# QuentinFuxa/WhisperLiveKit

Hardware: AMD Instinct MI355X
Metric: audio seconds transcribed per second (1/RTF), Whisper-base EN simul_whisper AlignAtt, 0.5 s chunks (higher is better)
Workload: dtype f32; 1 GPU; base.en simul_whisper, 1 stream(s) over 1 GPU(s) (1 per GPU), 30 s 16 kHz speech-like stream, 0.5 s chunks, beam 1, frame_threshold 25, seeded random weights, synthetic vocabulary; model=base.en, streams_total=1

## Files before the change

include/wlk_hip.h:

```cpp
#ifndef WLK_HIP_H
#define WLK_HIP_H

#include <stdint.h>

#ifdef __cplusplus
extern "C" {
#endif

#define WLK_OK 0
#define WLK_ERR_ARG (-1)
#define WLK_ERR_HIP (-2)
#define WLK_ERR_STATE (-3)
#define WLK_ERR_CAPACITY (-4)

typedef struct wlk_model wlk_model;
typedef struct wlk_session wlk_session;

typedef struct wlk_dims {
    int32_t n_mels, n_audio_ctx, n_audio_state, n_audio_head, n_audio_layer;
    int32_t n_vocab, n_text_ctx, n_text_state, n_text_head, n_text_layer;
} wlk_dims;

const char* wlk_last_error(void);
int wlk_abi_version(void);
// ... 264 lines not shown
typedef struct wlk_vad_group wlk_vad_group;
int wlk_vad_group_create(wlk_vad* m, int max_streams , int max_windows_total , wlk_vad_group** out);
int wlk_vad_group_run(wlk_vad_group* g, wlk_vad_stream* const* streams, const int32_t* n_windows, int n_streams,
                      const void* pcm_host, int sample_format, float* probs_host);
int wlk_vad_group_destroy(wlk_vad_group* g);

const char* wlk_diag_last_error(void);
int wlk_diag_env_refresh(void);
int wlk_diag_linear(const float* a, int64_t lda, int64_t a_floats, const float* w, const float* bias,
                    const float* r, int64_t ldr, int m, int n, int k, int flags, float scale, int scale_cols,
                    int force_gemv, float* c);
typedef struct wlk_nllb_dims {
    int32_t vocab, d_model, heads, ffn, enc_layers, dec_layers;
    int32_t max_src, max_tgt;
    int32_t pad_id;
    int32_t n_positions;
    float embed_scale;
} wlk_nllb_dims;
typedef struct wlk_nllb wlk_nllb;
typedef struct wlk_nllb_session wlk_nllb_session;
int wlk_nllb_arena_floats(const wlk_nllb_dims* dims, uint64_t* n_floats);
int wlk_nllb_tensor_lookup(const wlk_nllb_dims* dims, const char* packed_name, uint64_t* offset_floats, uint64_t* numel);
int wlk_nllb_tensor_name(const wlk_nllb_dims* dims, int index, const char** name);
int wlk_nllb_create(const wlk_nllb_dims* dims, int device, wlk_nllb** out);
int wlk_nllb_upload(wlk_nllb* m, const char* packed_name, const float* host, uint64_t numel);
int wlk_nllb_finalize(wlk_nllb* m);
int wlk_nllb_destroy(wlk_nllb* m);
int wlk_nllb_session_create(wlk_nllb* m, int rows, wlk_nllb_session** out);
int wlk_nllb_session_destroy(wlk_nllb_session* s);
int wlk_nllb_encode(wlk_nllb_session* s, const int64_t* src_ids, int32_t n);
int wlk_nllb_decode(wlk_nllb_session* s, const int64_t* tokens, int32_t n_rows, int32_t n_tok, int32_t first);
int wlk_nllb_step(wlk_nllb_session* s, const int64_t* tokens, int32_t n_rows, int32_t k, float* logprobs, int32_t* ids);
int wlk_nllb_kv_reorder(wlk_nllb_session* s, const int32_t* source_rows, int32_t n_rows);
int wlk_nllb_topk(wlk_nllb_session* s, int32_t k, float* logprobs, int32_t* ids);
int wlk_nllb_step_beam(wlk_nllb_session* s, const int64_t* tokens , const int32_t* source_rows ,
                       int32_t n_rows, int32_t k , float* logprobs, int32_t* ids);
int wlk_nllb_session_beam_stats(wlk_nllb_session* s, uint64_t* ancestry_steps);
int wlk_nllb_session_set_align(wlk_nllb_session* s, const int32_t* layer_head_pairs, int32_t n);
int wlk_nllb_step_align(wlk_nllb_session* s, const int64_t* tokens, int32_t n_rows, int32_t k , int32_t lo, int32_t hi,
                        int32_t limit, float* logprobs, int32_t* ids, int32_t* align_pos , float* align_prob ,
                        float* tail_mass );
enum { WLK_ALIGN_STOP_ATTENTION = 0, WLK_ALIGN_STOP_EOS = 1, WLK_ALIGN_STOP_LENGTH = 2, WLK_ALIGN_STOP_CONTEXT = 3 };
int wlk_nllb_generate_alignatt(wlk_nllb_session* s, const int64_t* prompt, int32_t n_prompt, int32_t n_accessible,
                               int32_t threshold, int32_t final, int64_t eos_id, int32_t max_new, int64_t* out_ids,
                               int32_t* out_align, int32_t* n_out, int32_t* stop_reason);
int wlk_nllb_session_align_stats(wlk_nllb_session* s, uint64_t* align_steps, uint64_t* graph_captures);
int wlk_nllb_export(wlk_nllb_session* s, const char* what, float* host, uint64_t capacity, uint64_t* n_written);
int wlk_nllb_sync(wlk_nllb_session* s);

typedef struct wlk_nllb_batch wlk_nllb_batch;
int wlk_nllb_batch_create(wlk_nllb* m, int n_slots, wlk_nllb_batch** out);
int wlk_nllb_batch_destroy(wlk_nllb_batch* b);
int wlk_nllb_batch_encode(wlk_nllb_batch* b, const int32_t* slots, const int64_t* src_ids, const int32_t* src_offsets, int32_t n);
int wlk_nllb_batch_step(wlk_nllb_batch* b, const int32_t* slots, const int64_t* tokens, int32_t n_rows, int32_t k, float* logprobs,
                        int32_t* ids);
int wlk_nllb_batch_release(wlk_nllb_batch* b, int32_t slot);
int wlk_nllb_batch_export(wlk_nllb_batch* b, int32_t slot, const char* what, float* host, uint64_t capacity, uint64_t* n_written);
int wlk_nllb_batch_cross_attention(wlk_nllb_batch* b, const int32_t* slots, int32_t n_rows, int32_t layer, const float* q_host,
                                   float* out_host);
int wlk_nllb_batch_sync(wlk_nllb_batch* b);
int wlk_nllb_batch_set_align(wlk_nllb_batch* b, const int32_t* layer_head_pairs, int32_t n);
int wlk_nllb_batch_prefill(wlk_nllb_batch* b, const int32_t* slots, const int64_t* prompt_ids, const int32_t* prompt_offsets,
                           int32_t n);
int wlk_nllb_batch_step_align(wlk_nllb_batch* b, const int32_t* slots, const int64_t* tokens, int32_t n_rows, int32_t k ,
                              const int32_t* lo , const int32_t* hi , const int32_t* limit ,
                              float* logprobs, int32_t* ids, int32_t* align_pos , float* align_prob ,
                              float* tail_mass );
int wlk_nllb_batch_align_stats(wlk_nllb_batch* b, uint64_t* align_steps, uint64_t* graph_captures);
int wlk_nllb_batch_verify(wlk_nllb_batch* b, const int32_t* slots, const int64_t* ids, const int32_t* offsets, int32_t n,
                          int32_t* accepted, int64_t* next_token);
int wlk_nllb_batch_verify_stats(wlk_nllb_batch* b, uint64_t* passes, uint64_t* draft_tokens, uint64_t* accepted_tokens);

int wlk_dtw(int device, const float* x, int32_t n_rows, int32_t n_cols, int8_t* trace);
int wlk_log_mel(wlk_session* s, const float* pcm, int64_t n_samples, int32_t padding, float* mel, uint64_t capacity_floats,
                int32_t* n_frames);
int wlk_encode_mel(wlk_session* s, const float* mel, int32_t n_frames);
int wlk_find_alignment(wlk_session* s, const int64_t* tokens, int32_t n_tokens, int32_t n_sot, int32_t eot,
                       int32_t num_frames, float qk_scale, float* cost, int8_t* trace, float* token_probs);
int wlk_head_survey(wlk_session* s, const int64_t* tokens, int32_t n_tokens, int32_t num_frames, float* peak, int32_t* frame);

int wlk_diag_linear_time(int m, int n, int k, int flags, int force_gemv, int reps, float* us_per_launch);
int wlk_diag_linear_ln(const float* a, const float* w, const float* bias, const float* gamma, const float* beta,
                       int m, int n, int k, int force_gemv, float* c);
int wlk_diag_layernorm(const float* x, const float* gamma, const float* beta, int rows, int d, float* y);
int wlk_diag_prefill_stack(wlk_session** sessions, const int64_t* tokens, const int32_t* n_tok, const int32_t* sot_index, int32_t n,
                           int32_t* taken);
int wlk_engine_prefill_stats(wlk_model* m, uint64_t* batches, uint64_t* sessions);
int wlk_diag_encoder_attention_time(int t, int d, int n_head, int reps, float* us_per_launch);
int wlk_diag_encoder_attention(const float* qkv, int t, int d, int n_head, float* out);
typedef struct wlk_diag_select_args {
    int32_t route, n_rows, n_vocab, k;
    const float* logits;
    const int32_t* adj_row;
    const int32_t* adj_ids;
    const float* adj_deltas;
    int32_t n_adj;
    int32_t n_align, ring_rows, T, single_base;
    const float* ring;
    const int32_t* prefill_rows;
    const int32_t* n_single;
    const int32_t* newest_row;
    const int32_t* content_len;
    int32_t ns_token;
    const float* ns_logits;
    float* top_logprobs;
    int32_t* top_ids;
    int32_t* frames;
    float* attn_last;
    float* z;
    float* ns_probs;
    float* logits_out;
} wlk_diag_select_args;
int wlk_diag_select(const wlk_diag_select_args* args);
int wlk_diag_topk(const float* logits, int32_t n_rows, int32_t n_vocab, int32_t k, int32_t form ,
                  float* logprobs, int32_t* ids);
int wlk_diag_nllb_align(const float* probs, int32_t n_align, int32_t rows, int32_t S, int32_t lo, int32_t hi, int32_t limit,
                        float* p_out, int32_t* pos, float* prob, float* mass);
int wlk_diag_nllb_align_rows(const float* probs, int32_t n_align, int32_t rows, int32_t stride, const int32_t* S,
                             const int32_t* lo, const int32_t* hi, const int32_t* limit, float* p_out, int32_t* pos, float* prob,
                             float* mass);
int wlk_diag_nllb_verify_pick(const float* logits, int32_t n_rows, int32_t n_vocab, const int32_t* targets, int32_t* picks,
                              int32_t* match);
enum {
    WLK_DA_S0 = 0, WLK_DA_S1 = 1, WLK_DA_S2 = 2,
    WLK_DA_C0 = 10, WLK_DA_C1 = 11, WLK_DA_C2 = 12, WLK_DA_C3 = 13, WLK_DA_C4 = 14, WLK_DA_C5 = 15,
    WLK_DA_A0 = 20, WLK_DA_G0 = 21, WLK_DA_K0 = 22, WLK_DA_K1 = 23
};
typedef struct wlk_diag_dec_attention_args {
    int32_t route, n_rows, n_tok, d, n_head, ctx_len, T;
    int32_t anc_rows, n_updates, gather_len, n_layer, n_kv, k_splits, n_align, n_beam, ring_rows;
    float scale;
    int64_t cache_floats;
    int64_t layer_off;
    int64_t scores_floats, out_floats;
    const float* qkv;
    float* kcache;
    float* vcache;
    const int32_t* offsets;
    const int32_t* row_cache;
    uint8_t* anc;
    const int32_t* ctl;
    const int32_t* upd_offsets;
    const float* q;
    const float* k;
    const float* v;
    const int32_t* row_kv;
    const float* x;
    const float* wq;
    const float* bq;
    const float* gamma;
    const float* beta;
    const float* wo;
    const float* bo;
    const float* resid;
    const int32_t* head_rank;
    const int32_t* ring_row;
    const int32_t* beam_of_row;
    float* ring;
    float* scores;
    float* out;
} wlk_diag_dec_attention_args;
int wlk_diag_dec_attention(const wlk_diag_dec_attention_args* args);
enum {
    WLK_SFK_ATTENTION = 0, WLK_SFK_CONV0 = 1, WLK_SFK_DWCONV2D = 2, WLK_SFK_GLU_DWCONV = 3, WLK_SFK_HEAD = 4, WLK_SFK_ASSEMBLE = 5
};
typedef struct wlk_diag_sf_kernel_args {
// ... 125 lines not shown
```

whisperlivekit_amd/_lib.py:

```python
from __future__ import annotations

import ctypes as C
import os
import threading
from typing import Optional


_LIB_NAME = "libwlk_hip.so"
_lock = threading.Lock()
_lib: Optional[C.CDLL] = None


class WlkError(RuntimeError):
    """Raised for every non-zero status of the C ABI (message from wlk_last_error())."""


class Dims(C.Structure):
    _fields_ = [(n, C.c_int32) for n in (
        "n_mels", "n_audio_ctx", "n_audio_state", "n_audio_head", "n_audio_layer",
        "n_vocab", "n_text_ctx", "n_text_state", "n_text_head", "n_text_layer")]


class SfDims(C.Structure):
    _fields_ = [(n, C.c_int32) for n in (
# ... 246 lines not shown
        "wlk_prof_end": (cint, [p, cint, C.POINTER(C.c_char_p), p, p, p, p, C.POINTER(i32)]),
        "wlk_melspec_create": (cint, [cint, cint, cint, cint, cint, p, p, C.c_float, C.c_float, cint, C.POINTER(p)]),
        "wlk_melspec_run": (cint, [p, p, cint, p, cint, C.POINTER(cint)]),
        "wlk_melspec_destroy": (cint, [p]),
        "wlk_sf_arena_floats": (cint, [C.POINTER(SfDims), C.POINTER(u64)]),
        "wlk_sf_tensor_lookup": (cint, [C.POINTER(SfDims), C.c_char_p, C.POINTER(u64), C.POINTER(u64)]),
        "wlk_sf_tensor_name": (cint, [C.POINTER(SfDims), cint, C.POINTER(C.c_char_p)]),
        "wlk_sf_create": (cint, [C.POINTER(SfDims), cint, C.POINTER(p)]),
        "wlk_sf_upload": (cint, [p, C.c_char_p, p, u64]),
        "wlk_sf_finalize": (cint, [p]),
        "wlk_sf_step": (cint, [p, p, cint, p, cint, p, cint, C.POINTER(cint), p, cint]),
        "wlk_sf_step_pcm": (cint, [p, p, p, cint, cint, p, cint, p, cint, C.POINTER(cint), p, cint, p, cint, C.POINTER(cint), p, cint]),
        "wlk_sf_stats": (cint, [p, C.POINTER(u64), C.POINTER(u64), C.POINTER(u64)]),
        "wlk_sf_export": (cint, [p, C.c_char_p, p, u64, C.POINTER(u64)]),
        "wlk_sf_destroy": (cint, [p]),
        "wlk_sf_session_create": (cint, [p, C.POINTER(SfCacheParams), cint, C.POINTER(p)]),
        "wlk_sf_session_destroy": (cint, [p]),
        "wlk_sf_session_step_pcm": (cint, [p, p, p, cint, cint, cint, cint, p, cint, C.POINTER(cint)]),
        "wlk_sf_session_step": (cint, [p, p, cint, cint, cint, p, cint, C.POINTER(cint)]),
        "wlk_sf_session_update": (cint, [p, p, cint, p, cint, cint, cint, p, cint, C.POINTER(cint)]),
        "wlk_sf_session_get_state": (cint, [p, C.POINTER(SfState)]),
        "wlk_sf_session_set_state": (cint, [p, C.POINTER(SfState)]),
        "wlk_nllb_arena_floats": (cint, [C.POINTER(NllbDims), C.POINTER(u64)]),
        "wlk_nllb_tensor_lookup": (cint, [C.POINTER(NllbDims), C.c_char_p, C.POINTER(u64), C.POINTER(u64)]),
        "wlk_nllb_tensor_name": (cint, [C.POINTER(NllbDims), cint, C.POINTER(C.c_char_p)]),
        "wlk_nllb_create": (cint, [C.POINTER(NllbDims), cint, C.POINTER(p)]),
        "wlk_nllb_upload": (cint, [p, C.c_char_p, p, u64]),
        "wlk_nllb_finalize": (cint, [p]),
        "wlk_nllb_destroy": (cint, [p]),
        "wlk_nllb_session_create": (cint, [p, cint, C.POINTER(p)]),
        "wlk_nllb_session_destroy": (cint, [p]),
        "wlk_nllb_encode": (cint, [p, p, i32]),
        "wlk_nllb_decode": (cint, [p, p, i32, i32, i32]),
        "wlk_nllb_step": (cint, [p, p, i32, i32, p, p]),
        "wlk_nllb_kv_reorder": (cint, [p, p, i32]),
        "wlk_nllb_step_beam": (cint, [p, p, p, i32, i32, p, p]),
        "wlk_nllb_session_beam_stats": (cint, [p, C.POINTER(u64)]),
        "wlk_nllb_topk": (cint, [p, i32, p, p]),
        "wlk_nllb_session_set_align": (cint, [p, p, i32]),
        "wlk_nllb_step_align": (cint, [p, p, i32, i32, i32, i32, i32, p, p, p, p, p]),
        "wlk_nllb_generate_alignatt": (cint, [p, p, i32, i32, i32, i32, C.c_int64, i32, p, p, C.POINTER(i32), C.POINTER(i32)]),
        "wlk_nllb_session_align_stats": (cint, [p, C.POINTER(u64), C.POINTER(u64)]),
        "wlk_nllb_export": (cint, [p, C.c_char_p, p, u64, C.POINTER(u64)]),
        "wlk_nllb_sync": (cint, [p]),
        "wlk_nllb_batch_create": (cint, [p, cint, C.POINTER(p)]),
        "wlk_nllb_batch_destroy": (cint, [p]),
        "wlk_nllb_batch_encode": (cint, [p, p, p, p, i32]),
        "wlk_nllb_batch_step": (cint, [p, p, p, i32, i32, p, p]),
        "wlk_nllb_batch_release": (cint, [p, i32]),
        "wlk_nllb_batch_export": (cint, [p, i32, C.c_char_p, p, u64, C.POINTER(u64)]),
        "wlk_nllb_batch_cross_attention": (cint, [p, p, i32, i32, p, p]),
        "wlk_nllb_batch_sync": (cint, [p]),
        "wlk_nllb_batch_set_align": (cint, [p, p, i32]),
        "wlk_nllb_batch_prefill": (cint, [p, p, p, p, i32]),
        "wlk_nllb_batch_step_align": (cint, [p, p, p, i32, i32, p, p, p, p, p, p, p, p]),
        "wlk_nllb_batch_align_stats": (cint, [p, C.POINTER(u64), C.POINTER(u64)]),
        "wlk_nllb_batch_verify": (cint, [p, p, p, p, i32, p, p]),
        "wlk_nllb_batch_verify_stats": (cint, [p, C.POINTER(u64), C.POINTER(u64), C.POINTER(u64)]),
        "wlk_vad_weights_floats": (cint, [C.POINTER(u64)]),
        "wlk_vad_tensor_lookup": (cint, [C.c_char_p, C.POINTER(u64), C.POINTER(u64)]),
        "wlk_vad_tensor_name": (cint, [cint, C.POINTER(C.c_char_p)]),
        "wlk_vad_create": (cint, [cint, p, u64, C.POINTER(p)]),
        "wlk_vad_destroy": (cint, [p]),
        "wlk_vad_stream_create": (cint, [p, cint, C.POINTER(p)]),
        "wlk_vad_stream_reset": (cint, [p]),
        "wlk_vad_stream_run": (cint, [p, p, cint, p]),
        "wlk_vad_stream_state": (cint, [p, p, p]),
        "wlk_vad_stream_destroy": (cint, [p]),
        "wlk_vad_stream_run_pcm16": (cint, [p, p, cint, p]),
        "wlk_vad_group_create": (cint, [p, cint, cint, C.POINTER(p)]),
        "wlk_vad_group_run": (cint, [p, C.POINTER(p), i32p, cint, p, cint, p]),
        "wlk_vad_group_destroy": (cint, [p]),
        "wlk_diag_last_error": (C.c_char_p, []),
        "wlk_diag_linear": (cint, [p, C.c_int64, C.c_int64, p, p, p, C.c_int64, cint, cint, cint, cint, C.c_float,
                                   cint, cint, p]),
        "wlk_dtw": (cint, [cint, C.POINTER(C.c_float), C.c_int32, C.c_int32, C.POINTER(C.c_int8)]),
        "wlk_encode_mel": (cint, [C.c_void_p, C.POINTER(C.c_float), C.c_int32]),
        "wlk_log_mel": (cint, [C.c_void_p, C.POINTER(C.c_float), C.c_int64, C.c_int32, C.POINTER(C.c_float), C.c_uint64,
                               C.POINTER(C.c_int32)]),
        "wlk_find_alignment": (cint, [C.c_void_p, C.POINTER(C.c_int64), C.c_int32, C.c_int32, C.c_int32, C.c_int32, C.c_float,
                                      C.POINTER(C.c_float), C.POINTER(C.c_int8), C.POINTER(C.c_float)]),
        "wlk_diag_linear_time": (cint, [cint, cint, cint, cint, cint, cint, C.POINTER(C.c_float)]),
        "wlk_diag_linear_ln": (cint, [p, p, p, p, p, cint, cint, cint, cint, p]),
        "wlk_diag_layernorm": (cint, [p, p, p, cint, cint, p]),
        "wlk_diag_encoder_attention_time": (cint, [cint, cint, cint, cint, C.POINTER(C.c_float)]),
        "wlk_diag_encoder_attention": (cint, [p, cint, cint, cint, p]),
        "wlk_diag_wave_ops": (cint, [p, p, p]),
        "wlk_diag_env_refresh": (cint, []),
        "wlk_diag_linear_x3": (cint, [p, p, p, cint, cint, cint, cint, C.c_float, cint, p]),
        "wlk_diag_linear_x3_time": (cint, [cint, cint, cint, cint, cint, C.POINTER(C.c_float)]),
        "wlk_diag_layernorm_x3": (cint, [p, p, p, cint, cint, p]),
        "wlk_diag_encoder_attention_x3": (cint, [p, cint, cint, cint, p]),
        "wlk_diag_encoder_attention_x3_time": (cint, [cint, cint, cint, cint, C.POINTER(C.c_float)]),
        "wlk_diag_qkv_x3_attention": (cint, [p, p, p, cint, cint, cint, C.c_float, p, p]),
        "wlk_diag_select": (cint, [C.POINTER(DiagSelectArgs)]),
        "wlk_diag_dec_attention": (cint, [C.POINTER(DiagDecAttentionArgs)]),
        "wlk_diag_topk": (cint, [p, i32, i32, i32, i32, p, p]),
        "wlk_diag_nllb_align": (cint, [p, i32, i32, i32, i32, i32, i32, p, p, p, p]),
        "wlk_diag_nllb_align_rows": (cint, [p, i32, i32, i32, p, p, p, p, p, p, p, p]),
        "wlk_diag_nllb_verify_pick": (cint, [p, i32, i32, p, p, p]),
        "wlk_diag_sf_kernel": (cint, [C.POINTER(DiagSfKernelArgs)]),
        "wlk_diag_linear_ex": (cint, [C.POINTER(DiagLinearArgs)]),
        "wlk_diag_gemv_variant": (cint, [cint, cint, cint, cint, cint, C.c_char_p, cint]),
        "wlk_diag_gemm_plan": (cint, [cint, cint, cint, cint, cint, cint, C.c_char_p, cint]),
        "wlk_diag_enc_op": (cint, [C.POINTER(DiagEncOpArgs)]),
        "wlk_diag_x3_plan": (cint, [cint, cint, cint, cint, cint, C.c_char_p, cint]),
        "wlk_diag_word_align": (cint, [C.POINTER(DiagWordAlignArgs)]),
        "wlk_diag_head_survey": (cint, [C.POINTER(DiagHeadSurveyArgs)]),
        "wlk_head_survey": (cint, [C.c_void_p, C.POINTER(C.c_int64), C.c_int32, C.c_int32, C.POINTER(C.c_float), C.POINTER(C.c_int32)]),
        "wlk_diag_nllb_cross_ragged": (cint, [C.POINTER(DiagNllbCrossRaggedArgs)]),
        "wlk_model_set_cif": (cint, [p, p, cint, C.c_float]),
        "wlk_cif_result": (cint, [p, C.POINTER(CifOut)]),
        "wlk_diag_cif": (cint, [p, cint, cint, p, C.c_float, cint, cint, p, p, p]),
    }
    for name, (res, args) in sig.items():
        try:
            fn = getattr(lib, name)
        except AttributeError:
            if "WLK_HIP_LIB" in os.environ and name.startswith("wlk_diag_"):
                continue
            raise
        fn.restype = res
        fn.argtypes = args


EXPORTED_SYMBOLS = (
    "wlk_last_error", "wlk_abi_version", "wlk_device_count", "wlk_arena_floats", "wlk_tensor_lookup",
    "wlk_tensor_name", "wlk_model_create", "wlk_model_arena", "wlk_model_upload",
    "wlk_model_set_alignment_heads", "wlk_model_finalize", "wlk_model_destroy", "wlk_session_create",
    "wlk_session_destroy", "wlk_session_set_debug", "wlk_audio_append", "wlk_audio_append_pcm16", "wlk_audio_append_zeros",
    "wlk_audio_drop_front", "wlk_audio_clear", "wlk_audio_len", "wlk_encode", "wlk_decode",
    "wlk_no_speech_prob", "wlk_rules_set", "wlk_pick_greedy", "wlk_pick_topk", "wlk_decode_ancestry", "wlk_select", "wlk_kv_reorder", "wlk_sync", "wlk_decode_until_stop", "wlk_engine_attach", "wlk_engine_detach",
    "wlk_engine_stats", "wlk_engine_encode_stats", "wlk_engine_prefill_stats", "wlk_diag_prefill_stack", "wlk_job_create",
    "wlk_job_begin_step", "wlk_job_no_speech", "wlk_job_adjustments", "wlk_job_consume", "wlk_job_result",
    "wlk_job_destroy", "wlk_export", "wlk_session_step_stats", "wlk_prof_begin",
    "wlk_decode_beam_until_stop", "wlk_session_beam_stats", "wlk_diag_beam_step", "wlk_beam_job_create",
    "wlk_beam_job_begin_step", "wlk_beam_job_no_speech", "wlk_beam_job_adjustments", "wlk_beam_job_consume",
    "wlk_beam_job_state", "wlk_beam_job_result", "wlk_beam_job_destroy",
    "wlk_prof_end", "wlk_melspec_create", "wlk_melspec_run", "wlk_melspec_destroy",
    "wlk_sf_arena_floats", "wlk_sf_tensor_lookup", "wlk_sf_tensor_name", "wlk_sf_create", "wlk_sf_upload",
    "wlk_sf_finalize", "wlk_sf_step", "wlk_sf_step_pcm", "wlk_sf_stats", "wlk_sf_export", "wlk_sf_destroy",
    "wlk_sf_session_create", "wlk_sf_session_destroy", "wlk_sf_session_step_pcm", "wlk_sf_session_step",
    "wlk_sf_session_update", "wlk_sf_session_get_state", "wlk_sf_session_set_state",
    "wlk_vad_weights_floats", "wlk_vad_tensor_lookup", "wlk_vad_tensor_name", "wlk_vad_create", "wlk_vad_destroy",
    "wlk_vad_stream_create", "wlk_vad_stream_reset", "wlk_vad_stream_run", "wlk_vad_stream_state",
    "wlk_vad_stream_destroy", "wlk_vad_stream_run_pcm16", "wlk_vad_group_create", "wlk_vad_group_run",
    "wlk_vad_group_destroy",
    "wlk_dtw", "wlk_encode_mel", "wlk_log_mel", "wlk_find_alignment", "wlk_head_survey",
    "wlk_nllb_arena_floats", "wlk_nllb_tensor_lookup", "wlk_nllb_tensor_name", "wlk_nllb_create", "wlk_nllb_upload",
    "wlk_nllb_finalize", "wlk_nllb_destroy", "wlk_nllb_session_create", "wlk_nllb_session_destroy", "wlk_nllb_encode",
    "wlk_nllb_decode", "wlk_nllb_step", "wlk_nllb_kv_reorder", "wlk_nllb_topk", "wlk_nllb_export", "wlk_nllb_sync",
    "wlk_nllb_step_beam", "wlk_nllb_session_beam_stats",
    "wlk_nllb_session_set_align", "wlk_nllb_step_align", "wlk_nllb_generate_alignatt", "wlk_nllb_session_align_stats",
    "wlk_nllb_batch_create", "wlk_nllb_batch_destroy", "wlk_nllb_batch_encode", "wlk_nllb_batch_step", "wlk_nllb_batch_release",
    "wlk_nllb_batch_export", "wlk_nllb_batch_cross_attention", "wlk_nllb_batch_sync",
    "wlk_nllb_batch_set_align", "wlk_nllb_batch_prefill", "wlk_nllb_batch_step_align", "wlk_nllb_batch_align_stats",
    "wlk_diag_last_error", "wlk_diag_linear", "wlk_diag_linear_time", "wlk_diag_linear_ln", "wlk_diag_layernorm",
    "wlk_diag_encoder_attention", "wlk_diag_encoder_attention_time", "wlk_diag_wave_ops", "wlk_diag_env_refresh",
    "wlk_diag_linear_x3", "wlk_diag_linear_x3_time", "wlk_diag_layernorm_x3",
    "wlk_diag_encoder_attention_x3", "wlk_diag_encoder_attention_x3_time", "wlk_diag_qkv_x3_attention",
    "wlk_diag_select", "wlk_diag_dec_attention", "wlk_diag_topk", "wlk_diag_sf_kernel", "wlk_diag_nllb_align",
    "wlk_diag_nllb_align_rows", "wlk_diag_linear_ex", "wlk_diag_gemv_variant", "wlk_diag_gemm_plan", "wlk_diag_enc_op",
    "wlk_diag_x3_plan", "wlk_diag_word_align", "wlk_diag_head_survey", "wlk_diag_nllb_cross_ragged",
    "wlk_model_set_cif", "wlk_cif_result", "wlk_diag_cif",
    "wlk_group_create", "wlk_group_destroy", "wlk_group_step_pick", "wlk_group_stats", "wlk_group_export_logits",
    "wlk_diag_pick_rows",
    "wlk_group_find_alignment", "wlk_group_align_fits", "wlk_diag_dtw_starts",
    "wlk_group_run_pick", "wlk_diag_pick_advance",
    "wlk_group_verify", "wlk_group_verify_fits", "wlk_diag_draft_pick",
    "wlk_nllb_batch_verify", "wlk_nllb_batch_verify_stats", "wlk_diag_nllb_verify_pick",
)


def load() -> C.CDLL:
    global _lib
    if _lib is not None:
        return _lib
    with _lock:
        if _lib is None:
            path = lib_path()
            if not os.path.exists(path):
                raise WlkError(
                    f"{path} not found: build it with `python -m whisperlivekit_amd.build` "
                    "(hipcc, gfx950). There is no CPU fallback for the HIP backend.")
            try:
                import torch
            except Exception:
                pass
            try:
                lib = C.CDLL(path, mode=C.RTLD_GLOBAL)
            except OSError as e:
                raise WlkError(f"cannot load {path}: {e}") from e
            _declare(lib)
            _lib = lib
    return _lib


def check(rc: int) -> None:
    if rc != 0:
        msg = load().wlk_last_error()
        err = WlkError(f"wlk_hip error {rc}: {msg.decode('utf-8', 'replace') if msg else '?'}")
        err.code = int(rc)
        raise err


def device_count() -> int:
    return int(load().wlk_device_count())
```

whisperlivekit_amd/csrc/api.hip:

```cpp
#include <cmath>
#include <cstdio>
#include <cstdlib>
#include <atomic>
#include <chrono>
#include <cstring>
#include <map>
#include <memory>
#include <mutex>
#include <string>
#include <vector>

#include "../../include/wlk_hip.h"
#include "common.h"
#include "internal.h"

namespace wlk {

namespace {
struct UtilStream {
    std::mutex mu;
    hipStream_t stream = nullptr;
};
UtilStream g_util[64];
UtilStream& util_of_current_device() {
// ... 333 lines not shown
        m->finalized = true;
        return WLK_OK;
    });
}

int wlk_model_destroy(wlk_model* m) {
    if (!m) return WLK_OK;
    wlk_engine_destroy_for_model(m);
    (void)hipSetDevice(m->device);
    if (m->owns_arena) (void)hipFree(m->arena);
    if (m->xkv_all_w) (void)hipFree(m->xkv_all_w);
    if (m->xkv_all_b) (void)hipFree(m->xkv_all_b);
    for (unsigned short* p : m->x3_owned) (void)hipFree(p);
    (void)hipFree(m->twiddle);
    (void)hipFree(m->filt_lo);
    (void)hipFree(m->filt_hi);
    (void)hipFree(m->head_rank);
    (void)hipFree(m->layer_heads);
    (void)hipFree(m->layer_ranks);
    (void)hipFree(m->all_ranks);
    if (m->cif_w) (void)hipFree(m->cif_w);
    delete m;
    return WLK_OK;
}

int wlk_session_create(wlk_model* m, int beam, int max_audio_samples, wlk_session** out) {
    if (!m || !out) return fail(WLK_ERR_ARG, "NULL argument");
    if (!m->finalized) return fail(WLK_ERR_STATE, "model not finalized");
    if (beam < 1 || beam > 7) return fail(WLK_ERR_ARG, "beam must be in [1, 7]");
    if (max_audio_samples < kHop) return fail(WLK_ERR_ARG, "max_audio_samples too small");
    return guarded([&]() {
        WLK_HIP(hipSetDevice(m->device));
        auto s = std::make_unique<wlk_session>();
        s->m = m;
        s->beam = beam;
        s->audio_cap = max_audio_samples;
        WLK_HIP(hipStreamCreateWithFlags(&s->stream, hipStreamNonBlocking));
        if (const char* e = std::getenv("WLK_NO_GRAPH")) s->use_graph = !(e[0] == '1');
        hipStream_t st = s->stream;
        const wlk_dims& D = m->D;
        const size_t d = D.n_audio_state, T = D.n_audio_ctx, ctx = D.n_text_ctx, V = D.n_vocab;
        s->audio[0] = dev_alloc_zero<float>(s->audio_cap, st);
        s->audio[1] = dev_alloc_zero<float>(s->audio_cap, st);
        s->frame_cap = s->audio_cap / kHop + 4;
        s->logmel = dev_alloc<float>((size_t)s->frame_cap * D.n_mels);
        s->frame_max = dev_alloc<float>(s->frame_cap);
        s->logmel_alt = dev_alloc<float>((size_t)s->frame_cap * D.n_mels);
        s->frame_max_alt = dev_alloc<float>(s->frame_cap);
        if (const char* e = std::getenv("WLK_MEL_INCREMENTAL")) s->mel_incremental = !(e[0] == '0');
        s->mel_t = dev_alloc_zero<float>((size_t)(kMelFrames + 2) * D.n_mels, st);
        s->x1p = dev_alloc_zero<float>((size_t)(kMelFrames + 1) * d, st);
        s->ex = dev_alloc<float>(T * d);
        s->eh = dev_alloc<float>(T * d);
        s->eqkv = dev_alloc<float>(T * 3 * d);
        s->eatt = dev_alloc<float>(T * d);
        s->emlp = dev_alloc<float>(T * 4 * d);
        s->enc_out = dev_alloc<float>(T * d);
        {
            bool any_x3 = m->xkv_all_w3 != nullptr, qkv_x3 = false;
            bool fc2_x3 = false;
            for (const auto& L : m->enc_layers) {
                any_x3 |= L.qkvw3 || L.fc1w3 || L.outw3;
                qkv_x3 |= L.qkvw3 != nullptr;
                fc2_x3 |= L.fc2w3 != nullptr;
            }
            if (fc2_x3) s->emlp3 = dev_alloc<unsigned short>(T * 3 * 4 * d);
            const bool attn_x3 = qkv_x3 && enc_attention_x3_enabled() && d == (size_t)D.n_audio_head * 64 && T >= 64 && (2 * d) % 128 == 0;
            if (any_x3) s->eh3 = dev_alloc<unsigned short>(T * 3 * d);
            if (attn_x3) s->eqkv3 = dev_alloc_zero<unsigned short>(x3_attn_image_elems((int)T, (int)d), st);
            if (m->xkv_all_w3) s->enc_out3 = dev_alloc<unsigned short>(T * 3 * d);
        }
        s->cross_kv = dev_alloc<float>((size_t)D.n_text_layer * T * 2 * d);

        s->max_rows = beam * (int)ctx;
        const size_t R = s->max_rows;
        s->step_in = dev_alloc<int>(3 * R + 4);
        s->tokens_dev = s->step_in;
        s->dx = dev_alloc<float>(R * d);
        s->dh = dev_alloc<float>(R * d);
        s->dqkv = dev_alloc<float>(R * 3 * d);
        s->datt = dev_alloc<float>(R * d);
        s->dq = dev_alloc<float>(R * d);
        s->dmlp = dev_alloc<float>(R * 4 * d);
        const size_t cache = (size_t)D.n_text_layer * beam * ctx * d;
        s->kcache[0] = dev_alloc<float>(cache);
        s->vcache[0] = dev_alloc<float>(cache);
        s->hsel = dev_alloc<float>((size_t)2 * beam * d);
        s->logits_last = dev_alloc<float>((size_t)2 * beam * V);
        s->logits_sot = s->logits_last + (size_t)beam * V;
        s->ring_row = s->step_in + R;
        s->beam_of_row = s->step_in + 2 * R;
        s->d_offset = s->step_in + 3 * R;
        s->ring_rows = (int)ctx + kAlignWindow;
        if (m->n_align > 0) s->ring = dev_alloc<float>((size_t)m->n_align * beam * s->ring_rows * T);
        s->xsplit = dev_alloc<float>(cross_split_scratch_floats(8, D.n_text_head, (int)T));
        s->fsplit = dev_alloc<float>(flash_split_scratch_floats(s->max_rows, D.n_text_head, wlk_session::kFlashSplitsMax));
        s->z = dev_alloc<float>((size_t)beam * std::max(m->n_align, 1) * T + (size_t)beam * 128);
        s->attn_last = dev_alloc_zero<float>((size_t)beam * T, st);
        s->adj_row = dev_alloc<int>(3 * wlk_session::kAdjCap);
        s->src_rows = dev_alloc<int>(8);
        if (beam >= 2 && beam <= 7) s->anc = dev_alloc_zero<unsigned char>((size_t)beam * ctx, st);
        s->top_vals = dev_alloc<float>((size_t)beam * 18);
        s->top_ids = reinterpret_cast<int*>(s->top_vals) + (size_t)beam * 8;
        s->frames = s->top_ids + (size_t)beam * 8;
        WLK_HIP(hipMalloc(&s->topk_scratch, topk_scratch_bytes(beam)));
        s->probs = dev_alloc<float>(beam);
        WLK_HIP(hipHostMalloc(&s->pinned, wlk_session::kPinnedBytes, hipHostMallocDefault));
        WLK_HIP(hipHostMalloc(&s->dec_stage, 65536, hipHostMallocDefault));
        WLK_HIP(hipHostMalloc(&s->audio_stage, wlk_session::kPinnedBytes, hipHostMallocDefault));
        WLK_HIP(hipEventCreateWithFlags(&s->audio_stage_ev, hipEventDisableTiming));
        WLK_HIP(hipEventCreateWithFlags(&s->dec_stage_ev, hipEventDisableTiming));
        if (beam == 1) {
            void* hp = nullptr;
            WLK_HIP(hipHostMalloc(&hp, 4096, hipHostMallocMapped | hipHostMallocCoherent));
            std::memset(hp, 0, 4096);
            s->step_host = static_cast<StepBlock*>(hp);
            s->result_host = reinterpret_cast<StepResult*>(static_cast<char*>(hp) + 2048);
            void* dp = nullptr;
            WLK_HIP(hipHostGetDevicePointer(&dp, hp, 0));
            s->step_host_dev = static_cast<StepBlock*>(dp);
            s->result_host_dev = reinterpret_cast<StepResult*>(static_cast<char*>(dp) + 2048);
            s->step_dev = reinterpret_cast<StepBlock*>(dev_alloc<int>(sizeof(StepBlock) / 4));
        }
        if (m->cif_w) wlk_cif_session_prepare(s.get());
        WLK_HIP(hipStreamSynchronize(st));
        *out = s.release();
        return WLK_OK;
    });
}

int wlk_session_destroy(wlk_session* s) {
    if (!s) return WLK_OK;
    if (s->step_count && getenv("WLK_STEP_TIMING"))
        fprintf(stderr, "[wlk] one-replay steps: %llu, mean %.1f us per step (graph launch call %.1f us)\n",
                (unsigned long long)s->step_count, s->step_ns / 1e3 / s->step_count, s->step_launch_ns / 1e3 / s->step_count);
    (void)wlk_engine_detach(s);
    (void)hipSetDevice(s->m->device);
    (void)hipStreamSynchronize(s->stream);
    float* fl[] = {s->audio[0], s->audio[1], s->logmel, s->frame_max, s->logmel_alt, s->frame_max_alt, s->mel_t, s->x1p, s->ex, s->eh, s->eqkv,
                   s->eatt, s->emlp, s->enc_out, s->cross_kv, s->dx, s->dh, s->dqkv, s->datt, s->dq, s->dmlp,
                   s->kcache[0], s->kcache[1], s->vcache[0], s->vcache[1], s->hsel, s->logits_last,
                   s->ring, s->z, s->attn_last, s->qk_debug, s->xsplit, s->fsplit, s->top_vals, s->probs};
    for (float* p : fl)
        if (p) (void)hipFree(p);
    int* il[] = {s->step_in, s->adj_row, s->src_rows};
    for (int* p : il)
        if (p) (void)hipFree(p);
    for (auto& e : s->step_exec)
        if (e) (void)hipGraphExecDestroy(e);
    for (auto& e : s->bstep_exec)
        if (e) (void)hipGraphExecDestroy(e);
    if (s->anc) (void)hipFree(s->anc);
    if (s->topk_scratch) (void)hipFree(s->topk_scratch);
    if (s->pcm16_dev) (void)hipFree(s->pcm16_dev);
    if (s->eh3) (void)hipFree(s->eh3);
    if (s->eqkv3) (void)hipFree(s->eqkv3);
    if (s->enc_out3) (void)hipFree(s->enc_out3);
    if (s->emlp3) (void)hipFree(s->emlp3);
    if (s->wa_buf) (void)hipFree(s->wa_buf);
    if (s->survey_buf) (void)hipFree(s->survey_buf);
    if (s->pinned) (void)hipHostFree(s->pinned);
    if (s->dec_stage) (void)hipHostFree(s->dec_stage);
    if (s->audio_stage) (void)hipHostFree(s->audio_stage);
    if (s->rules_mask) (void)hipFree(s->rules_mask);
    if (s->pick_out) (void)hipFree(s->pick_out);
    if (s->audio_stage_ev) (void)hipEventDestroy(s->audio_stage_ev);
    if (s->dec_stage_ev) (void)hipEventDestroy(s->dec_stage_ev);
    if (s->step_host) (void)hipHostFree(s->step_host);
    if (s->step_dev) (void)hipFree(s->step_dev);
    if (s->step_align_dev) (void)hipFree(s->step_align_dev);
    wlk_cif_session_free(s);
    for (auto& e : s->fstep_exec)
        if (e) (void)hipGraphExecDestroy(e);
    for (auto& r : s->prof.recs) {
        (void)hipEventDestroy(r.a);
        (void)hipEventDestroy(r.b);
    }
    for (auto e : s->prof.pool) (void)hipEventDestroy(e);
    (void)hipStreamDestroy(s->stream);
    delete s;
    return WLK_OK;
}

int wlk_session_set_debug(wlk_session* s, int on) {
    if (!s) return fail(WLK_ERR_ARG, "session is NULL");
    return guarded([&]() {
        WLK_HIP(hipSetDevice(s->m->device));
        s->debug = on != 0;
        if (s->debug && !s->qk_debug) {
            const wlk_dims& D = s->m->D;
            s->qk_debug = dev_alloc<float>((size_t)D.n_text_layer * s->max_rows * D.n_text_head * D.n_audio_ctx);
        }
        return WLK_OK;
    });
}

static bool drain_staging() {
    static const bool on = [] {
        const char* e = getenv("WLK_DRAIN_STAGING");
        return e && e[0] == '1';
    }();
    return on;
}

int wlk_audio_append(wlk_session* s, const float* pcm_host, int n) {
    if (!s || (n > 0 && !pcm_host) || n < 0) return fail(WLK_ERR_ARG, "bad audio chunk");
    if (s->audio_len + n > s->audio_cap)
        return fail(WLK_ERR_CAPACITY, "audio buffer capacity exceeded (" + std::to_string(s->audio_len + n) + " > " +
                                          std::to_string(s->audio_cap) + " samples)");
    if (n == 0) return WLK_OK;
    return guarded([&]() {
        WLK_HIP(hipSetDevice(s->m->device));
        float* dst = s->audio[s->audio_cur] + s->audio_len;
        size_t done = 0;
        while (done < (size_t)n) {
            const size_t chunk = std::min((size_t)n - done, wlk_session::kPinnedBytes / sizeof(float));
            if (s->audio_stage_used) WLK_HIP(hipEventSynchronize(s->audio_stage_ev));
            std::memcpy(s->audio_stage, pcm_host + done, chunk * sizeof(float));
            WLK_HIP(hipMemcpyAsync(dst + done, s->audio_stage, chunk * sizeof(float), hipMemcpyHostToDevice, s->stream));
            WLK_HIP(hipEventRecord(s->audio_stage_ev, s->stream));
            s->audio_stage_used = true;
            done += chunk;
        }
        if (drain_staging()) WLK_HIP(hipStreamSynchronize(s->stream));
        s->audio_len += n;
        s->encoded = false;
        return WLK_OK;
    });
}

// ... 7 lines not shown
        WLK_HIP(hipSetDevice(s->m->device));
        constexpr size_t kMax = wlk_session::kPinnedBytes / sizeof(int16_t);
        if (!s->pcm16_dev) WLK_HIP(hipMalloc(reinterpret_cast<void**>(&s->pcm16_dev), kMax * sizeof(int16_t)));
        float* dst = s->audio[s->audio_cur] + s->audio_len;
        const LaunchCtx c = s->ctx();
        size_t done = 0;
        while (done < (size_t)n) {
            const size_t chunk = std::min((size_t)n - done, kMax);
            if (s->audio_stage_used) WLK_HIP(hipEventSynchronize(s->audio_stage_ev));
            std::memcpy(s->audio_stage, pcm_host + done, chunk * sizeof(int16_t));
            WLK_HIP(hipMemcpyAsync(s->pcm16_dev, s->audio_stage, chunk * sizeof(int16_t), hipMemcpyHostToDevice, s->stream));
            launch_pcm16_to_float(c, s->pcm16_dev, dst + done, (int)chunk);
            WLK_HIP(hipEventRecord(s->audio_stage_ev, s->stream));
            s->audio_stage_used = true;
            done += chunk;
        }
        if (drain_staging()) WLK_HIP(hipStreamSynchronize(s->stream));
        s->audio_len += n;
        s->encoded = false;
        return WLK_OK;
    });
}

int wlk_audio_append_zeros(wlk_session* s, int n) {
    if (!s || n < 0) return fail(WLK_ERR_ARG, "bad zero run");
    if (s->audio_len + n > s->audio_cap) return fail(WLK_ERR_CAPACITY, "audio buffer capacity exceeded");
    if (n == 0) return WLK_OK;
    return guarded([&]() {
        WLK_HIP(hipSetDevice(s->m->device));
        WLK_HIP(hipMemsetAsync(s->audio[s->audio_cur] + s->audio_len, 0, (size_t)n * sizeof(float), s->stream));
        s->audio_len += n;
        s->encoded = false;
        return WLK_OK;
    });
}

int wlk_audio_drop_front(wlk_session* s, int n) {
    if (!s || n < 0 || n > s->audio_len) return fail(WLK_ERR_ARG, "bad eviction length");
    if (n == 0) return WLK_OK;
    return guarded([&]() {
        WLK_HIP(hipSetDevice(s->m->device));
        const int keep = s->audio_len - n;
        if (keep > 0)
            WLK_HIP(hipMemcpyAsync(s->audio[s->audio_cur ^ 1], s->audio[s->audio_cur] + n, (size_t)keep * sizeof(float),
                                   hipMemcpyDeviceToDevice, s->stream));
        s->audio_cur ^= 1;
        s->audio_len = keep;
        s->encoded = false;
        const int shift = n / kHop;
        if (s->mel_incremental && n % kHop == 0 && s->mel_cached_samples > n && shift < s->mel_cached_frames) {
            const int rows = s->mel_cached_frames - shift;
            const int nm = s->m->D.n_mels;
            WLK_HIP(hipMemcpyAsync(s->logmel_alt, s->logmel + (size_t)shift * nm, (size_t)rows * nm * sizeof(float),
                                   hipMemcpyDeviceToDevice, s->stream));
            WLK_HIP(hipMemcpyAsync(s->frame_max_alt, s->frame_max + shift, (size_t)rows * sizeof(float),
                                   hipMemcpyDeviceToDevice, s->stream));
            std::swap(s->logmel, s->logmel_alt);
            std::swap(s->frame_max, s->frame_max_alt);
            s->mel_cached_samples -= n;
            s->mel_cached_frames = rows;
            s->mel_dirty_head = 2;
        } else {
            s->mel_cached_samples = 0;
        }
        return WLK_OK;
    });
}

int wlk_audio_clear(wlk_session* s) {
    if (!s) return fail(WLK_ERR_ARG, "session is NULL");
    s->audio_len = 0;
    s->encoded = false;
    s->mel_cached_samples = 0;
    return WLK_OK;
}

int wlk_audio_len(wlk_session* s, int* n) {
    if (!s || !n) return fail(WLK_ERR_ARG, "NULL argument");
    *n = s->audio_len;
    return WLK_OK;
}

static void transformer_mlp(const LaunchCtx& c, const LayerW& L, float* x, float* h, float* mlp, int rows, int d,
                            const char* t_ln, const char* t_fc1, const char* t_fc2) {
    GemmArgs g;
    g.lda = d; g.W = L.fc1w; g.bias = L.fc1b; g.C = mlp; g.ldc = 4 * d; g.M = rows; g.N = 4 * d; g.K = d;
    g.flags = kGemmGelu;
    if (gemv_applicable(rows, d)) {
        g.A = x; g.ln_gamma = L.ln2w; g.ln_beta = L.ln2b;
        launch_gemv(c, g, "dec_ln2_fc1");
    } else {
        launch_layernorm(c, x, d, L.ln2w, L.ln2b, h, d, rows, d, t_ln);
        g.A = h;
        launch_gemm(c, g, t_fc1);
    }
    GemmArgs g2;
    g2.A = mlp; g2.lda = 4 * d; g2.W = L.fc2w; g2.bias = L.fc2b; g2.C = x; g2.ldc = d; g2.M = rows; g2.N = d;
    g2.K = 4 * d; g2.flags = kGemmResidual; g2.R = x; g2.ldr = d;
    launch_linear(c, g2, t_fc2);
}

extern "C++" std::string wlk_encode_precheck(const wlk_session* s, const wlk_model* m) {
    if (!s) return "encode: session is NULL";
    if (s->m != m) return "encode: the session belongs to another model";
    const int N = s->audio_len;
    const int n_total = (N + kPadSamples) / kHop;
    int n_active = N > 0 ? (N + kNFft / 2 + kHop - 1) / kHop : 0;
    if (n_active > n_total) n_active = n_total;
    if (n_active > s->frame_cap) return "audio longer than the session's frame capacity";
    return std::string();
}

extern "C++" void wlk_encode_group(const std::vector<wlk_session*>& group, const LaunchCtx& c,
                                   std::vector<int>& content_out, bool mel_given) {
    const int B = (int)group.size();
    if (B < 1 || B > kMaxBatch) throw std::invalid_argument("encode: bad group size");
    wlk_model* m = group[0]->m;
    const wlk_dims& D = m->D;
    const int d = D.n_audio_state, T = D.n_audio_ctx;
    content_out.assign(B, 0);
    for (int i = 0; i < B; ++i) {
        wlk_session* s = group[i];
        if (s->m != m) throw std::invalid_argument("encode: sessions of different models in one group");
        if (mel_given) {
            content_out[i] = D.n_audio_ctx;
            continue;
        }
        const int N = s->audio_len;
        const int n_total = (N + kPadSamples) / kHop;
        int n_active = N > 0 ? (N + kNFft / 2 + kHop - 1) / kHop : 0;
        if (n_active > n_total) n_active = n_total;
        if (n_active > s->frame_cap) throw std::length_error("audio longer than the session's frame capacity");
        content_out[i] = (n_total - kMelFrames) / 2;
        MelArgs ma;
        ma.audio = s->audio[s->audio_cur]; ma.n_samples = N;
        ma.window = m->w("mel.window"); ma.twiddle = m->twiddle; ma.filters = m->w("mel.filters");
        ma.filt_lo = m->filt_lo; ma.filt_hi = m->filt_hi; ma.n_mels = D.n_mels;
        ma.logmel = s->logmel; ma.frame_max = s->frame_max; ma.mel_t = s->mel_t;
        ma.n_active = n_active; ma.n_total = n_total;
        if (s->mel_incremental && s->mel_cached_samples > 0 && s->mel_cached_samples <= N && s->mel_cached_frames <= n_active) {
            int first = s->mel_cached_samples >= kNFft / 2 ? (s->mel_cached_samples - kNFft / 2) / kHop + 1 : 0;
            first = std::min(first, s->mel_cached_frames);
            ma.first = first;
            ma.head = std::min(s->mel_dirty_head, first);
        }
        launch_mel(c, ma);
        s->mel_cached_samples = N;
        s->mel_cached_frames = n_active;
        s->mel_dirty_head = 0;
    }
    auto table = [&](auto in, auto out, auto res) {
        PtrTable z{};
        for (int i = 0; i < B; ++i) {
            z.in[i] = in(group[i]);
            z.out[i] = out(group[i]);
            z.res[i] = res(group[i]);
        }
        return z;
    };
    auto none = [](wlk_session*) -> const float* { return nullptr; };
    auto gemm = [&](GemmArgs g, const PtrTable& z, const char* tag) {
        const bool stackable = !gemm_takes_kwave(g.M, g.N, g.K) && (long)((g.N + 63) / 64) * ((g.M + 63) / 64) >= 64;
        if (stackable) {
            g.batch = B;
            g.z = z;
            launch_gemm(c, g, tag);
        } else {
            for (int i = 0; i < B; ++i) {
                g.A = z.in[i]; g.C = z.out[i]; g.R = z.res[i];
                launch_gemm(c, g, tag);
            }
        }
    };
    {
        GemmArgs g;
        g.lda = D.n_mels; g.W = m->w("enc.conv1.w"); g.bias = m->w("enc.conv1.b");
        g.ldc = d; g.M = kMelFrames; g.N = d; g.K = 3 * D.n_mels; g.flags = kGemmGelu;
        gemm(g, table([](wlk_session* s) { return (const float*)s->mel_t; }, [&](wlk_session* s) { return s->x1p + d; }, none),
             "enc_conv1");
    }
    {
// ... 100 lines not shown
                for (int i = 0; i < B; ++i) launch_x3_pack(c, group[i]->emlp, 4 * d, group[i]->emlp3, 4 * d, T, 4 * d);
            gemm_x3(f2, L.fc2w3, z_mlp3_ex_res, "enc_fc2_x3");
        } else {
            gemm(f2, z_mlp_ex, "enc_fc2");
        }
    }
    {
        GemmArgs g;
        g.lda = d; g.W = m->xkv_all_w; g.bias = m->xkv_all_b;
        g.ldc = (long)D.n_text_layer * 2 * d; g.M = T; g.N = D.n_text_layer * 2 * d; g.K = d;
        g.flags = kGemmScaleCols; g.scale = scale; g.scale_cols = d; g.scale_period = 2 * d;
        if (m->xkv_all_w3) {
            launch_layernorm_x3_batched(c, table([](wlk_session* s) { return (const float*)s->ex; },
                                                 [](wlk_session* s) { return reinterpret_cast<float*>(s->enc_out3); }, none),
                                        B, d, m->w("enc.ln_post.w"), m->w("enc.ln_post.b"), d, T, d, "enc_ln_post");
            gemm_x3(g, m->xkv_all_w3,
                    table([](wlk_session* s) { return reinterpret_cast<const float*>(s->enc_out3); }, [](wlk_session* s) { return s->cross_kv; }, none),
                    "dec_cross_kv_x3");
        } else {
            launch_layernorm_batched(c, table([](wlk_session* s) { return (const float*)s->ex; }, [](wlk_session* s) { return s->enc_out; }, none),
                                     B, d, m->w("enc.ln_post.w"), m->w("enc.ln_post.b"), d, T, d, "enc_ln_post");
            gemm(g, table([](wlk_session* s) { return (const float*)s->enc_out; }, [](wlk_session* s) { return s->cross_kv; }, none),
                 "dec_cross_kv");
        }
        for (int i = 0; i < B; ++i) group[i]->enc_out_is_x3 = m->xkv_all_w3 != nullptr;
    }
    if (m->cif_w) wlk_cif_enqueue(group, c, content_out);
    else
        for (int i = 0; i < B; ++i) group[i]->cif_T = -1;
    for (int i = 0; i < B; ++i) {
        wlk_session* s = group[i];
        s->encoded = true;
        s->content_len = content_out[i];
        s->self_len = 0;
        s->n_steps = 0;
    }
}

int wlk_encode(wlk_session* s, int32_t* content_mel_len) {
    if (!s) return fail(WLK_ERR_ARG, "session is NULL");
    return guarded([&]() {
        WLK_HIP(hipSetDevice(s->m->device));
        int content = 0;
        struct Busy {
            wlk_session* s;
            explicit Busy(wlk_session* ss) : s(ss) { wlk_engine_loop_enter(s); }
            ~Busy() { wlk_engine_loop_exit(s); }
        } busy(s);
        if (wlk_engine_batches_encodes(s)) {
            if (int rc = wlk_engine_encode(s, &content)) return rc;
        } else {
            std::vector<int> out;
            wlk_encode_group({s}, s->ctx(), out);
            content = out[0];
        }
        if (content_mel_len) *content_mel_len = content;
        return WLK_OK;
    });
}

int wlk_session::flash_splits() {
    static const int n = [] {
        const char* e = getenv("WLK_FLASH_SPLITS");
        const int v = e ? atoi(e) : 6;
        return v < 1 ? 1 : (v > kFlashSplitsMax ? kFlashSplitsMax : v);
    }();
    return n;
}

constexpr size_t kAncStageOffset = 65536 - 64;

static void enqueue_decode(wlk_session* s, const LaunchCtx& c, int n_rows, int n_tok, bool first, int sot_index,
                           bool step_block = false, const AlignArgs* side_align = nullptr, int side_blocks = 0, int side_zf = 0,
                           bool ancestry = false) {
    wlk_model* m = s->m;
    const wlk_dims& D = m->D;
    const int ctx_len = D.n_text_ctx;
    const int R = n_rows * n_tok;
    const int d = D.n_text_state, T = D.n_audio_ctx, H = D.n_text_head, V = D.n_vocab;
    if (!step_block)
        WLK_HIP(hipMemcpyAsync(s->step_in, s->dec_stage, (size_t)(3 * s->max_rows + 1) * sizeof(int), hipMemcpyHostToDevice,
                               s->stream));
    const bool fused = gemv_applicable(R, d) && n_tok == 1;
    if (ancestry) {
        if (!fused || step_block || !s->anc) throw std::logic_error("decode: the ancestry step needs the fused beam step");
        WLK_HIP(hipMemcpyAsync(s->src_rows, static_cast<char*>(s->dec_stage) + kAncStageOffset, 8 * sizeof(int),
                               hipMemcpyHostToDevice, s->stream));
        launch_anc_update(c, s->anc, s->src_rows, s->d_offset, n_rows, ctx_len);
    }

    if (step_block)
        launch_embed_step(c, s->step_host_dev, s->step_dev, s->tokens_dev, s->ring_row, s->beam_of_row, s->d_offset,
                          m->w_tok_emb, m->w_dec_pos, s->dx, d);
    else
        launch_embed(c, s->tokens_dev, m->w_tok_emb, m->w_dec_pos, s->dx, n_rows, n_tok, s->d_offset, d);
    const float scale = std::pow((float)kHeadDim, -0.25f);
    const size_t cache_layer = (size_t)s->beam * ctx_len * d;
    bool scores_dumped = false;
    const bool raw_pass = s->align_raw_scores || s->survey;
    for (int i = 0; i < D.n_text_layer; ++i) {
        const LayerW& L = m->dec_layers[i];
        float* kc = s->kcache[s->kv_cur] + i * cache_layer;
        float* vc = s->vcache[s->kv_cur] + i * cache_layer;
        GemmArgs g;
        g.W = L.qkvw; g.bias = L.qkvb; g.C = s->dqkv; g.ldc = 3 * d; g.M = R; g.N = 3 * d;
        g.K = d; g.flags = kGemmScaleCols; g.scale = scale; g.scale_cols = 2 * d; g.lda = d;
        if (fused) {
            g.A = s->dx; g.ln_gamma = L.ln1w; g.ln_beta = L.ln1b;
            g.kcache = kc; g.vcache = vc; g.kv_pos = s->d_offset; g.kv_d = d; g.kv_ctx = ctx_len;
            launch_gemv(c, g, "dec_ln1_qkv_kv");
        } else {
            launch_layernorm(c, s->dx, d, L.ln1w, L.ln1b, s->dh, d, R, d, "dec_ln1");
            g.A = s->dh;
            if (!gemv_applicable(R, d) && gemm_takes_kwave(R, 3 * d, d)) {
                g.kcache = kc; g.vcache = vc; g.kv_pos = s->d_offset; g.kv_d = d; g.kv_ctx = ctx_len; g.kv_ntok = n_tok;
                launch_gemm(c, g, "dec_qkv");
            } else {
                launch_linear(c, g, "dec_qkv");
                launch_kv_append(c, s->dqkv, kc, vc, n_rows, n_tok, s->d_offset, d, ctx_len);
            }
        }
        if (ancestry)
            launch_decoder_self_attention_anc(c, s->dqkv, kc, vc, s->anc, s->datt, n_rows, s->d_offset, d, H, ctx_len);
        else
            launch_decoder_self_attention(c, s->dqkv, kc, vc, s->datt, n_rows, n_tok, s->d_offset, d, H, ctx_len);
        GemmArgs o;
        o.A = s->datt; o.lda = d; o.W = L.outw; o.bias = L.outb; o.C = s->dx; o.ldc = d; o.M = R; o.N = d; o.K = d;
        o.flags = kGemmResidual; o.R = s->dx; o.ldr = d;
        launch_linear(c, o, "dec_out");

        GemmArgs q;
        q.lda = d; q.W = L.xqw; q.bias = L.xqb; q.C = s->dq; q.ldc = d; q.M = R; q.N = d; q.K = d;
        q.flags = kGemmScaleCols; q.scale = scale; q.scale_cols = d;
        if (s->survey) q.C = s->survey_buf + (size_t)i * R * d;
        const bool fold_xq = fused && R == 1 && !s->debug && !raw_pass && cross_split_folds_query(d);
        if (fold_xq) {
        } else if (fused) {
            q.A = s->dx; q.ln_gamma = L.lnxw; q.ln_beta = L.lnxb;
            launch_gemv(c, q, "dec_lnx_xq");
        } else {
            launch_layernorm(c, s->dx, d, L.lnxw, L.lnxb, s->dh, d, R, d, "dec_lnx");
            q.A = s->dh;
            launch_linear(c, q, "dec_xq");
        }
        const int* ranks_l = m->n_align > 0 ? m->head_rank + (size_t)i * H : nullptr;
        bool merged_xout = false;
        GemmArgs xo_mg;
        if ((R > 8 || raw_pass) && !s->debug) {
            if (fold_xq) throw std::logic_error("decode: the folded query projection left no q for the flash kernel");
            FlashArgs fa;
            fa.q = q.C; fa.ldq = d;
            fa.k = s->cross_kv + (size_t)i * 2 * d; fa.v = fa.k + d; fa.ldkv = (long)D.n_text_layer * 2 * d;
            fa.out = s->datt; fa.ldo = d; fa.Tq = R; fa.Tk = T; fa.n_head = H;
            fa.head_rank = ranks_l; fa.ring = s->ring; fa.ring_row = s->ring_row;
            fa.beam_of_row = s->beam_of_row; fa.ring_rows = s->ring_rows; fa.n_beam = s->beam;
            if (((R + 31) / 32) * H < 256) {
                fa.k_splits = wlk_session::flash_splits();
                fa.part_o = s->fsplit;
                fa.part_m = fa.part_o + (size_t)s->max_rows * H * fa.k_splits * 64;
                fa.part_l = fa.part_m + (size_t)s->max_rows * H * fa.k_splits;
            }
            launch_prefill_cross_attention(c, fa);
            scores_dumped = true;
        } else {
            CrossAttnArgs ca;
            ca.q = s->dq;
            ca.k = s->cross_kv + (size_t)i * 2 * d;
            ca.v = ca.k + d;
            ca.ldkv = (long)D.n_text_layer * 2 * d;
            ca.out = s->datt;
            ca.rows = R; ca.d = d; ca.n_head = H; ca.T = T;
            ca.head_rank = ranks_l;
            ca.ring = s->ring;
            ca.ring_row = s->ring_row;
            ca.beam_of_row = s->beam_of_row;
            ca.ring_rows = s->ring_rows;
            ca.n_beam = s->beam;
            ca.qk_debug = s->debug ? s->qk_debug + (size_t)i * s->max_rows * H * T : nullptr;
            if (fold_xq) {
                ca.xq_x = s->dx; ca.xq_w = L.xqw; ca.xq_b = L.xqb; ca.xq_gamma = L.lnxw; ca.xq_beta = L.lnxb; ca.xq_scale = scale;
            }
            if (R <= 8 && !s->debug) {
                float* sc = s->xsplit;
                float* pm = sc + (size_t)8 * H * T;
                float* pl = pm + (size_t)8 * H * 8;
                float* po = pl + (size_t)8 * H * 8;
                merged_xout = fused && R == 1 && gemv1_folds_merge(d);
                launch_decoder_cross_attention_split(c, ca, sc, pm, pl, po, !merged_xout);
                if (merged_xout) {
                    xo_mg.mg_pm = pm; xo_mg.mg_pl = pl; xo_mg.mg_po = po; xo_mg.mg_scores = sc;
                    xo_mg.mg_head_rank = ranks_l; xo_mg.mg_ring = s->ring; xo_mg.mg_ring_row = s->ring_row;
                    xo_mg.mg_side_heads = m->layer_heads + (size_t)i * H;
                    xo_mg.mg_beam_of_row = s->beam_of_row; xo_mg.mg_heads = H; xo_mg.mg_T = T;
                    xo_mg.mg_ring_rows = s->ring_rows; xo_mg.mg_n_beam = s->beam;
                    xo_mg.mg_side_blocks = ranks_l ? m->layer_rank_count[i] : 0;
                }
            } else {
                launch_decoder_cross_attention(c, ca);
            }
        }
        GemmArgs xo = xo_mg;
        xo.A = s->datt; xo.lda = d; xo.W = L.xoutw; xo.bias = L.xoutb; xo.C = s->dx; xo.ldc = d; xo.M = R; xo.N = d;
        xo.K = d; xo.flags = kGemmResidual; xo.R = s->dx; xo.ldr = d;
        launch_linear(c, xo, "dec_xout");
        transformer_mlp(c, L, s->dx, s->dh, s->dmlp, R, d, "dec_ln2", "dec_fc1", "dec_fc2");
    }
    if (scores_dumped && m->n_align > 0 && !raw_pass)
        launch_ring_softmax(c, s->ring, s->ring_row, s->beam_of_row, m->all_ranks, m->n_align, R, s->ring_rows, s->beam, T);
    GemmArgs lg;
    lg.lda = d; lg.W = m->w_tok_emb; lg.C = s->logits_last; lg.ldc = V; lg.M = n_rows; lg.N = V; lg.K = d;
    if (side_align && !fused) throw std::logic_error("decode: side workgroups need the fused step");
    if (fused) {
        lg.A = s->dx; lg.ln_gamma = m->w_ln_w; lg.ln_beta = m->w_ln_b;
        lg.side_align = side_align; lg.side_blocks = side_blocks; lg.side_zf = side_zf;
        launch_gemv(c, lg, "dec_lnf_logits");
    } else if (first && n_rows == 1 && gemv_applicable(2, d) && getenv("WLK_NO_PREFILL_MERGE") == nullptr) {
        launch_layernorm(c, s->dx + (size_t)(n_tok - 1) * d, (long)(sot_index - (n_tok - 1)) * d, m->w_ln_w, m->w_ln_b,
                         s->hsel, d, 2, d, "dec_ln_f");
        lg.A = s->hsel; lg.M = 2;
        launch_linear(c, lg, "dec_logits");
        return;
    } else {
        launch_layernorm(c, s->dx + (size_t)(n_tok - 1) * d, (long)n_tok * d, m->w_ln_w, m->w_ln_b, s->hsel, d,
                         n_rows, d, "dec_ln_f");
        lg.A = s->hsel;
        launch_linear(c, lg, "dec_logits");
    }
    if (first) {
        float* hs = s->hsel + (size_t)n_rows * d;
        launch_layernorm(c, s->dx + (size_t)sot_index * d, (long)n_tok * d, m->w_ln_w, m->w_ln_b, hs, d, n_rows, d,
                         "dec_ln_f");
        GemmArgs ls = lg;
        ls.ln_gamma = ls.ln_beta = nullptr;
        ls.A = hs; ls.C = s->logits_sot;
        launch_linear(c, ls, "dec_logits");
    }
}

extern "C++" void wlk_prefill_ws_alloc(const wlk_model* m, wlk_prefill_ws& ws, int max_sessions, int session_rows) {
    const wlk_dims& D = m->D;
    const size_t d = D.n_text_state, V = D.n_vocab, H = D.n_text_head;
    ws.cap_session_rows = session_rows;
    ws.cap_rows = max_sessions * ((session_rows + 31) / 32 * 32);
    const size_t R = ws.cap_rows;
    ws.dx = dev_alloc<float>(R * d);
    ws.dh = dev_alloc<float>(R * d);
    ws.dqkv = dev_alloc<float>(R * 3 * d);
    ws.datt = dev_alloc<float>(R * d);
    ws.dq = dev_alloc<float>(R * d);
    ws.dmlp = dev_alloc<float>(R * 4 * d);
    ws.hsel = dev_alloc<float>((size_t)2 * max_sessions * d);
    ws.logits = dev_alloc<float>((size_t)8 * V);
    ws.part = dev_alloc<float>(flash_split_scratch_floats((int)R, (int)H, wlk_session::kFlashSplitsMax));
    ws.rows_dev = reinterpret_cast<StepRow*>(dev_alloc<char>(R * sizeof(StepRow)));
    ws.tiles_dev = reinterpret_cast<StepRow*>(dev_alloc<char>(R / 32 * sizeof(StepRow)));
    ws.ring_row_dev = dev_alloc<int>(R);
    ws.zeros_dev = dev_alloc<int>(R);
    memset_sync(ws.zeros_dev, 0, R * sizeof(int));
    ws.pinned_bytes = R * sizeof(StepRow) + R / 32 * sizeof(StepRow) + R * sizeof(int);
    WLK_HIP(hipHostMalloc(reinterpret_cast<void**>(&ws.pinned), ws.pinned_bytes, hipHostMallocDefault));
}

extern "C++" void wlk_prefill_ws_free(wlk_prefill_ws& ws) {
    void* dev[] = {ws.dx, ws.dh, ws.dqkv, ws.datt, ws.dq, ws.dmlp, ws.hsel, ws.logits, ws.part, ws.rows_dev, ws.tiles_dev,
                   ws.ring_row_dev, ws.zeros_dev};
    for (void* p : dev)
        if (p) (void)hipFree(p);
    if (ws.pinned) (void)hipHostFree(ws.pinned);
    ws = wlk_prefill_ws{};
}

extern "C++" std::string wlk_prefill_precheck(const wlk_prefill_item& it, const wlk_prefill_ws& ws) {
    const wlk_session* s = it.s;
    if (!s || !it.tokens) return "prefill: NULL argument";
    const wlk_dims& D = s->m->D;
    const int P = it.n_tok, d = D.n_text_state;
    if (!s->encoded) return "wlk_decode before wlk_encode";
    if (s->beam != 1 || s->debug || s->prof_on || s->align_raw_scores || s->survey) return "not a plain beam-1 session";
    if (it.sot_index < 0 || it.sot_index >= P) return "sot_index out of range";
    if (P > D.n_text_ctx) return "text context exceeded";
    for (int i = 0; i < P; ++i)
        if (it.tokens[i] < 0 || it.tokens[i] >= D.n_vocab) return "token id out of range";
    const std::string shape = wlk_prefill_shape_check(s->m, P, ws.cap_session_rows);
    if (!shape.empty()) return shape;
    if (!gemv_applicable(8, d)) return "model too wide for the stacked vocabulary projection";
    return std::string();
}

extern "C++" std::string wlk_prefill_shape_check(const wlk_model* m, int P, int cap_session_rows) {
    const wlk_dims& D = m->D;
    const int d = D.n_text_state;
    if (P <= 8 || P > cap_session_rows) return "prompt length outside the stacked range";
    if (!gemm_takes_kwave(P, 3 * d, d) || !gemm_takes_kwave(P, d, d) || !gemm_takes_kwave(P, 4 * d, d) ||
        !gemm_takes_kwave(P, d, 4 * d))
        return "prompt too long for the k-wave GEMMs";
    if (((P + 31) / 32) * D.n_text_head >= 256) return "prompt too long for the key-split cross-attention";
    return std::string();
}

extern "C++" void wlk_prefill_chain(const std::vector<wlk_prefill_item*>& items, const LaunchCtx& c, wlk_prefill_ws& ws,
                                    std::vector<int>& row0) {
    wlk_model* m = items[0]->s->m;
    const wlk_dims& D = m->D;
    const int d = D.n_text_state, T = D.n_audio_ctx, H = D.n_text_head, L = D.n_text_layer;
    const int B = (int)items.size();
    StepRow* rows_h = reinterpret_cast<StepRow*>(ws.pinned);
    std::vector<int> padded(B);
    row0.assign(B, 0);
    int R = 0;
    for (int i = 0; i < B; ++i) {
        row0[i] = R;
        padded[i] = (items[i]->n_tok + 31) / 32 * 32;
        R += padded[i];
    }
    if (R > ws.cap_rows) throw std::length_error("stacked prefill: more rows than the workspace holds");
    StepRow* tiles_h = rows_h + R;
    int* ring_row_h = reinterpret_cast<int*>(tiles_h + R / 32);
    for (int i = 0; i < B; ++i) {
        wlk_session* s = items[i]->s;
        for (int p = 0; p < padded[i]; ++p) {
            const int src = p < items[i]->n_tok ? p : 0;
            StepRow r{};
            r.kcache = s->kcache[s->kv_cur];
            r.vcache = s->vcache[s->kv_cur];
            r.cross_kv = s->cross_kv;
            r.ring = s->ring;
            r.token = (int)items[i]->tokens[src];
            r.offset = src;
            r.ring_row = src;
            rows_h[row0[i] + p] = r;
            ring_row_h[row0[i] + p] = src;
            if (p % 32 == 0) tiles_h[(row0[i] + p) / 32] = r;
        }
    }
    WLK_HIP(hipMemcpyAsync(ws.rows_dev, rows_h, (size_t)R * sizeof(StepRow), hipMemcpyHostToDevice, c.stream));
    WLK_HIP(hipMemcpyAsync(ws.tiles_dev, tiles_h, (size_t)(R / 32) * sizeof(StepRow), hipMemcpyHostToDevice, c.stream));
    WLK_HIP(hipMemcpyAsync(ws.ring_row_dev, ring_row_h, (size_t)R * sizeof(int), hipMemcpyHostToDevice, c.stream));

    launch_embed_rows(c, ws.rows_dev, m->w_tok_emb, m->w_dec_pos, ws.dx, R, d);
    const float scale = std::pow((float)kHeadDim, -0.25f);
    const size_t cache_layer = (size_t)D.n_text_ctx * d;
    auto linear = [&](const float* A, long lda, const float* W, const float* bias, float* C, long ldc, int N, int K, int flags,
                      const float* Rs, float sc, int sc_cols, const char* tag) {
        GemmArgs g;
        g.A = A; g.lda = lda; g.W = W; g.bias = bias; g.C = C; g.ldc = ldc; g.M = R; g.N = N; g.K = K;
        g.flags = flags; g.R = Rs; g.ldr = ldc; g.scale = sc; g.scale_cols = sc_cols;
        g.force_kwave = true;
        launch_gemm(c, g, tag);
    };
    auto ln_linear = [&](const float* gamma, const float* beta, const float* W, const float* bias, float* C, long ldc, int N,
                         int flags, float sc, int sc_cols, const char* t_ln, const char* tag) {
        launch_layernorm(c, ws.dx, d, gamma, beta, ws.dh, d, R, d, t_ln);
        linear(ws.dh, d, W, bias, C, ldc, N, d, flags, nullptr, sc, sc_cols, tag);
    };
    for (int i = 0; i < L; ++i) {
        const LayerW& W = m->dec_layers[i];
        ln_linear(W.ln1w, W.ln1b, W.qkvw, W.qkvb, ws.dqkv, 3 * d, 3 * d, kGemmScaleCols, scale, 2 * d, "dec_ln1", "dec_qkv");
        launch_kv_append_rows(c, ws.dqkv, ws.rows_dev, (long)(i * cache_layer), R, d);
        launch_decoder_self_attention_rows(c, ws.dqkv, ws.rows_dev, (long)(i * cache_layer), ws.datt, R, d, H, D.n_text_ctx);
        linear(ws.datt, d, W.outw, W.outb, ws.dx, d, d, d, kGemmResidual, ws.dx, 1.f, 0, "dec_out");
        ln_linear(W.lnxw, W.lnxb, W.xqw, W.xqb, ws.dq, d, d, kGemmScaleCols, scale, d, "dec_lnx", "dec_xq");
        FlashArgs fa;
        fa.q = ws.dq; fa.ldq = d;
        fa.k = nullptr; fa.v = nullptr; fa.ldkv = (long)L * 2 * d;
        fa.tile_rows = ws.tiles_dev; fa.tile_kv_off = (long)i * 2 * d; fa.tile_v_off = d;
        fa.out = ws.datt; fa.ldo = d; fa.Tq = R; fa.Tk = T; fa.n_head = H;
        fa.head_rank = m->n_align > 0 ? m->head_rank + (size_t)i * H : nullptr;
        fa.ring = nullptr; fa.ring_row = ws.ring_row_dev; fa.beam_of_row = ws.zeros_dev;
        fa.ring_rows = items[0]->s->ring_rows; fa.n_beam = 1;
        fa.k_splits = wlk_session::flash_splits();
        fa.part_o = ws.part;
        fa.part_m = fa.part_o + (size_t)R * H * fa.k_splits * 64;
        fa.part_l = fa.part_m + (size_t)R * H * fa.k_splits;
        launch_prefill_cross_attention(c, fa);
        linear(ws.datt, d, W.xoutw, W.xoutb, ws.dx, d, d, d, kGemmResidual, ws.dx, 1.f, 0, "dec_xout");
        ln_linear(W.ln2w, W.ln2b, W.fc1w, W.fc1b, ws.dmlp, 4 * d, 4 * d, kGemmGelu, 1.f, 0, "dec_ln2", "dec_fc1");
        linear(ws.dmlp, 4 * d, W.fc2w, W.fc2b, ws.dx, d, d, 4 * d, kGemmResidual, ws.dx, 1.f, 0, "dec_fc2");
    }
}

extern "C++" void wlk_prefill_group(const std::vector<wlk_prefill_item*>& items, const LaunchCtx& c, wlk_prefill_ws& ws) {
    if (items.empty()) return;
    wlk_model* m = items[0]->s->m;
    const wlk_dims& D = m->D;
    const int d = D.n_text_state, T = D.n_audio_ctx, V = D.n_vocab;
    const int B = (int)items.size();
    std::vector<int> row0;
    wlk_prefill_chain(items, c, ws, row0);
    for (int i = 0; i < B; ++i) {
        wlk_session* s = items[i]->s;
        const int P = items[i]->n_tok;
        if (m->n_align > 0)
            launch_ring_softmax(c, s->ring, ws.ring_row_dev + row0[i], ws.zeros_dev, m->all_ranks, m->n_align, P, s->ring_rows, 1, T);
        launch_layernorm(c, ws.dx + (size_t)(row0[i] + P - 1) * d, (long)(items[i]->sot_index - (P - 1)) * d, m->w_ln_w, m->w_ln_b,
                         ws.hsel + (size_t)2 * i * d, d, 2, d, "dec_ln_f");
    }
    for (int lo = 0; lo < B; lo += 4) {
        const int nb = std::min(4, B - lo);
        GemmArgs lg;
        lg.A = ws.hsel + (size_t)2 * lo * d; lg.lda = d; lg.W = m->w_tok_emb; lg.C = ws.logits; lg.ldc = V; lg.M = 2 * nb; lg.N = V;
        lg.K = d;
        launch_gemv(c, lg, "dec_logits");
        for (int i = 0; i < nb; ++i)
            WLK_HIP(hipMemcpyAsync(items[lo + i]->s->logits_last, ws.logits + (size_t)2 * i * V, (size_t)2 * V * sizeof(float),
                                   hipMemcpyDeviceToDevice, c.stream));
    }
    for (int i = 0; i < B; ++i) {
        wlk_session* s = items[i]->s;
        s->self_len = items[i]->n_tok;
        s->n_steps = 1;
        s->have_sot = true;
        s->prefill_rows = items[i]->n_tok;
        s->last_rows = 1;
        s->last_ntok = items[i]->n_tok;
    }
}

int wlk_decode(wlk_session* s, const int64_t* tokens, int n_rows, int n_tok, int first, int sot_index) {
    if (!s || !tokens) return fail(WLK_ERR_ARG, "NULL argument");
    if (!s->encoded) return fail(WLK_ERR_STATE, "wlk_decode before wlk_encode");
    if (n_rows != s->beam) return fail(WLK_ERR_ARG, "n_rows must equal the session's beam size");
    if (n_tok < 1) return fail(WLK_ERR_ARG, "n_tok must be >= 1");
    if (!first && n_tok != 1) return fail(WLK_ERR_ARG, "only one token per row may be fed after the first call");
    if (!first && s->n_steps == 0) return fail(WLK_ERR_STATE, "first decode of an infer must set first=1");
    if (!first && s->anc_live)
        return fail(WLK_ERR_STATE, "wlk_decode(first=0) after an ancestry beam step: the cache rows are not the hypotheses");
    if (first && (sot_index < 0 || sot_index >= n_tok)) return fail(WLK_ERR_ARG, "sot_index out of range");
    return guarded([&]() {
        wlk_model* m = s->m;
        const wlk_dims& D = m->D;
        WLK_HIP(hipSetDevice(m->device));
        const LaunchCtx c = s->ctx();
        if (first) {
            s->self_len = 0;
// ... 634 lines not shown
```

whisperlivekit_amd/csrc/common.h:

```cpp
#pragma once
#include <hip/hip_runtime.h>

#include <cstdint>
#include <stdexcept>
#include <mutex>
#include <string>

namespace wlk {

constexpr int kNFft = 400;
constexpr int kHop = 160;
constexpr int kNFreq = 201;
constexpr int kMelFrames = 3000;
constexpr int kPadSamples = 480000;
constexpr int kHeadDim = 64;
constexpr int kAlignWindow = 16;

struct HipError : std::runtime_error {
    using std::runtime_error::runtime_error;
};

inline void hip_check(hipError_t e, const char* what, const char* file, int line) {
    if (e != hipSuccess) {
        throw HipError(std::string(what) + " failed: " + hipGetErrorString(e) + " (" + file + ":" +
// ... 66 lines not shown
    r.newest_row = n_text_ctx + ((after - 2) % kAlignWindow);
    r.content_len = content_len;
    r.pad = 0;
}

constexpr int kStepMaxAdj = 160;
struct StepBlock {
    StepRow row;
    int n_adj;
    unsigned seq;
    int pad[2];
    int adj_row[kStepMaxAdj];
    int adj_ids[kStepMaxAdj];
    float adj_deltas[kStepMaxAdj];
};
struct StepResult {
    float top_vals[2];
    int top_ids[2];
    int frame;
    unsigned flag_topk, flag_align;
    int pad;
};
struct StepHostOut {
    StepResult* result = nullptr;
    const int* n_adj = nullptr;
    const unsigned* seq = nullptr;
};
constexpr int kEngineFusedAdj = 1024;
struct EngineBlock {
    int n_adj;
    unsigned seq;
    int pad[2];
    StepRow rows[8];
    int adj_row[kEngineFusedAdj];
    int adj_ids[kEngineFusedAdj];
    float adj_deltas[kEngineFusedAdj];
};
void launch_embed_rows_step(const LaunchCtx& ctx, const EngineBlock* host_block, EngineBlock* dev_block, const float* tok_emb,
                            const float* pos_emb, float* x, int n_rows, int d);
void launch_embed_step(const LaunchCtx& ctx, const StepBlock* host_block, StepBlock* dev_block, int* tokens_dev,
                       int* ring_row, int* beam_of_row, int* d_offset, const float* tok_emb, const float* pos_emb, float* x,
                       int d);

constexpr int kMaxBatch = 8;
struct PtrTable {
    const float* in[kMaxBatch];
    float* out[kMaxBatch];
    const float* res[kMaxBatch];
};
template <typename T>
__device__ __forceinline__ T table_at(T const (&t)[kMaxBatch], unsigned z) {
    T v = t[0];
#pragma unroll
    for (int i = 1; i < kMaxBatch; ++i) v = (z == (unsigned)i) ? t[i] : v;
    return v;
}

enum GemmFlags : int {
    kGemmGelu = 1,
    kGemmResidual = 2,
    kGemmScaleCols = 4,
    kGemmRelu = 8,
    kGemmSwish = 16,
};
struct AlignArgs;
struct GemmArgs {
    const float* A = nullptr;
    long lda = 0;
    const float* W = nullptr;
    const float* bias = nullptr;
    float* C = nullptr;
    long ldc = 0;
    const float* R = nullptr;
    long ldr = 0;
    int M = 0, N = 0, K = 0;
    int flags = 0;
    float scale = 1.f;
    int scale_cols = 0;
    int scale_period = 0;
    int batch = 0;
    long long* dbg_clock = nullptr;
    const float* ln_gamma = nullptr;
    const float* ln_beta = nullptr;
    float* kcache = nullptr;
    float* vcache = nullptr;
    const int* kv_pos = nullptr;
    int kv_d = 0, kv_ctx = 0;
    int kv_ntok = 1;
    const StepRow* kv_rows = nullptr;
    long kv_layer_off = 0;
    const float* mg_pm = nullptr;
    const float* mg_pl = nullptr;
    const float* mg_po = nullptr;
    const float* mg_scores = nullptr;
    const int* mg_head_rank = nullptr;
    const int* mg_side_heads = nullptr;
    float* mg_ring = nullptr;
    const int* mg_ring_row = nullptr;
    const int* mg_beam_of_row = nullptr;
    int mg_heads = 0, mg_T = 0, mg_ring_rows = 0, mg_n_beam = 1, mg_side_blocks = 0;
    PtrTable z;
    const AlignArgs* side_align = nullptr;
    int side_blocks = 0, side_zf = 0;
    bool force_kwave = false;
    int force_kernel = 0;
    bool gemm_plain_loop = false;
};
#define WLK_PIN_S(x) asm volatile("" ::"s"(x))
#define WLK_PIN_GEMM_ARGS(g)                                                                                                \
    do {                                                                                                                    \
        asm volatile("" ::"s"((g).A), "s"((g).lda), "s"((g).W), "s"((g).bias), "s"((g).C), "s"((g).ldc), "s"((g).R),        \
                     "s"((g).ldr), "s"((g).M), "s"((g).N), "s"((g).K), "s"((g).flags), "s"((g).scale), "s"((g).scale_cols), \
                     "s"((g).scale_period), "s"((g).batch), "s"((g).dbg_clock));                                            \
        __builtin_amdgcn_sched_barrier(0);     \
    } while (0)
void launch_gemm(const LaunchCtx& ctx, const GemmArgs& g, const char* tag);
void launch_gemm_kp(const LaunchCtx& ctx, const GemmArgs& g, const char* tag);
bool gemm_kp_takes_kpipe(int M, int N, int K);
bool gemm_kpipe_has_tile(int tm, int tn);
struct GemmPlan {
    enum Kernel {
        kRefused,
        kTiled64, kTiled32,
        kKwave, kKwave16,
        kKpipe,
        kKpKwave2, kKpKwave1, kKpKwave16
    };
    Kernel kernel = kRefused;
    int tm = 0, tn = 0;
    const char* refusal = nullptr;
};
GemmPlan gemm_plan(const GemmArgs& g, bool kp_family);
bool gemm_takes_kwave(int M, int N, int K);
bool gemm_takes_ksplit(int M, int N, int K);
void launch_gemv(const LaunchCtx& ctx, const GemmArgs& g, const char* tag);
inline int gemv_row_bucket(int M) { return M <= 1 ? 1 : M <= 2 ? 2 : M <= 4 ? 4 : 8; }
inline bool gemv_applicable(int M, int K) {
    return M <= 8 && (long)gemv_row_bucket(M) * K * 4 <= 64 * 1024 && K % 4 == 0;
}
struct GemvPlan {
    enum Kernel { kRefused, kStaged, kSingleRow, kSingleRowMergeLds };
    Kernel kernel = kRefused;
    int width = 0;
    int rpw = 0;
    bool ln = false, mg = false, full = false;
    const char* refusal = nullptr;
};
GemvPlan gemv_plan(const GemmArgs& g);
bool gemv1_folds_merge(int K);
void refresh_env_switches();
inline void launch_linear(const LaunchCtx& ctx, const GemmArgs& g, const char* tag) {
    if (gemv_applicable(g.M, g.K)) launch_gemv(ctx, g, tag);
    else launch_gemm(ctx, g, tag);
}

struct X3GemmArgs {
    const unsigned short* A3 = nullptr;
    long lda = 0;
    const unsigned short* W3 = nullptr;
    const float* bias = nullptr;
    float* C = nullptr;
    long ldc = 0;
    const float* R = nullptr;
    long ldr = 0;
    int M = 0, N = 0, K = 0;
    int flags = 0;
    float scale = 1.f;
    int scale_cols = 0;
    int scale_period = 0;
    int batch = 0;
    int walk_banded = 0;
    int walk_colmajor = 0;
    int walk_slots = 0;
    unsigned short* C3 = nullptr;
    long ldc3 = 0;
    int vt_col0 = 0;
    long vt_off = 0;
    long vt_ld = 0;
    bool x3_out = false;
    PtrTable z;
};
bool gemm_x3_wide_applicable(int M, int N, int K, long lda);
void launch_gemm_x3(const LaunchCtx& ctx, const X3GemmArgs& g, const char* tag);
void x3_gemm_check(const X3GemmArgs& g);
struct X3GemmPlan {
    int bm = 96;
    int tiles_m = 0, tiles_n = 0;
    int banded = 0, colmajor = 0, persist = 1;
    int slots = 0;
    int blocks = 0;
};
X3GemmPlan x3_gemm_plan(int M, int N, int batch, int cus);
size_t x3_w_elems(int n, int k);
void launch_x3_pack_w(const LaunchCtx& ctx, const float* src, long ld_src, unsigned short* dst, int n, int k);
void launch_x3_pack(const LaunchCtx& ctx, const float* src, long ld_src, unsigned short* dst, long ld_dst, int rows, int cols);
void x3_pack_check(long ld_src, long ld_dst, int cols);
void launch_x3_unpack(const LaunchCtx& ctx, const unsigned short* src, long ld_src, float* dst, long ld_dst, int rows, int cols);

inline long x3_attn_vt_ld(int T) { return ((long)T + 31) / 32 * 32; }
inline long x3_attn_vt_off(int T, int d) { return (long)T * 3 * 2 * d; }
inline size_t x3_attn_image_elems(int T, int d) { return (size_t)x3_attn_vt_off(T, d) + (size_t)d * 3 * x3_attn_vt_ld(T); }
bool enc_attention_x3_enabled();
void launch_encoder_attention_x3(const LaunchCtx& ctx, const unsigned short* qk3, long ldqk, long vt_off, long vt_ld, float* out,
                                 long ldo, int T, int d, int n_head, const PtrTable* z, int batch, bool x3_out = false);
void enc_attention_x3_check(long ldqk, long vt_ld, long ldo, int T, int d, int n_head, bool x3_out);
void launch_x3_pack_qkv(const LaunchCtx& ctx, const float* qkv, unsigned short* out, int T, int d, long vt_off, long vt_ld);

struct HeadSurveyArgs {
    const float* q = nullptr;
    long ldq = 0, q_layer = 0;
    const float* k = nullptr;
    long ldkv = 0, k_layer = 0;
    float* peak = nullptr;
    int* frame = nullptr;
    long out_layer = 0, out_head = 0;
    float* part = nullptr;
    int n_layer = 0, n_head = 0, P = 0, F = 0;
    int k_splits = 0;
};
void head_survey_check(const HeadSurveyArgs& a);
int head_survey_splits(const HeadSurveyArgs& a);
size_t head_survey_scratch_floats(const HeadSurveyArgs& a);
void launch_head_survey(const LaunchCtx& ctx, const HeadSurveyArgs& a);
enum WordAlignStage { kWaSoftmax = 0, kWaZscore = 1, kWaCost = 2, kWaDtw = 3 };
struct WordAlignArgs {
    const float* logits = nullptr;
    long ld = 0;
    int n_cols = 0;
    const int* target = nullptr;
    float* probs = nullptr;
    const float* ring = nullptr;
    int ring_rows = 0, T = 0, n_align = 0, P = 0, F = 0, n_sot = 0;
    float qk_scale = 1.f;
// ... 37 lines not shown
struct MelArgs {
    const float* audio;
    int n_samples;
    const float* window;
    const double* twiddle;
    const float* filters;
    const int* filt_lo;
    const int* filt_hi;
    int n_mels;
    float* logmel;
    float* frame_max;
    float* mel_t;
    int n_active;
    int n_total;
    int head = 0;
    int first = 0;
    int n_padded = 0x7fffffff;
};
void launch_mel(const LaunchCtx& ctx, const MelArgs& a);
void launch_mel_full(const LaunchCtx& ctx, const MelArgs& a, float* max_scratch, float* out);
void launch_pcm16_to_float(const LaunchCtx& ctx, const short* in, float* out, int n);

struct MelSpecArgs {
    const float* audio;
    int n_samples;
    const float* window;
    const double* twiddle;
    const float* filters;
    const int* filt_lo;
    const int* filt_hi;
    float* out;
    int n_fft, win_length, hop, n_mels;
    float preemph, log_guard;
};
void launch_melspec(const LaunchCtx& ctx, const MelSpecArgs& a, int n_frames);
}
struct wlk_melspec {
    int device = 0, n_fft = 0, win_length = 0, hop = 0, n_mels = 0, cap = 0;
    float preemph = 0.f, log_guard = 0.f;
    float *window = nullptr, *filters = nullptr, *audio = nullptr, *out = nullptr;
    double* twiddle = nullptr;
    int *lo = nullptr, *hi = nullptr;
    hipStream_t stream = nullptr;
    std::mutex mu;
};
namespace wlk {

struct FlashArgs {
    const float* q = nullptr; long ldq = 0;
    const float* k = nullptr; const float* v = nullptr; long ldkv = 0;
    float* out = nullptr; long ldo = 0;
    int Tq = 0, Tk = 0, n_head = 0;
    int batch = 0;
    long z_k_off = 0, z_v_off = 0;
    int k_splits = 1;
    int ring_rows = 0;
    const StepRow* tile_rows = nullptr;
    long tile_kv_off = 0, tile_v_off = 0;
    const int* head_rank = nullptr;
    float* ring = nullptr;
    const int* ring_row = nullptr;
    const int* beam_of_row = nullptr;
    int n_beam = 1;
    float* part_o = nullptr;
    float* part_m = nullptr;
    float* part_l = nullptr;
    PtrTable z;
};
#define WLK_PIN_FLASH_ARGS(a)                                                                                              \
    do {                                                                                                                   \
        asm volatile("" ::"s"((a).q), "s"((a).ldq), "s"((a).k), "s"((a).v), "s"((a).ldkv), "s"((a).out), "s"((a).ldo),      \
                     "s"((a).Tq), "s"((a).Tk), "s"((a).n_head), "s"((a).batch), "s"((a).z_k_off), "s"((a).z_v_off),         \
                     "s"((a).k_splits), "s"((a).ring_rows), "s"((a).tile_rows));                                            \
        __builtin_amdgcn_sched_barrier(0);                                                                                 \
    } while (0)
size_t flash_split_scratch_floats(int rows, int n_head, int k_splits);
void launch_encoder_attention(const LaunchCtx& ctx, const float* qkv, float* out, int T, int d, int n_head);
void launch_encoder_attention_batched(const LaunchCtx& ctx, const PtrTable& z, int batch, int T, int d, int n_head);
void launch_prefill_cross_attention(const LaunchCtx& ctx, const FlashArgs& a);
void launch_ring_softmax(const LaunchCtx& ctx, float* ring, const int* ring_row, const int* beam_of_row,
                         const int* ranks_dev, int n_ranks, int rows, int ring_rows, int n_beam, int T);

void launch_embed(const LaunchCtx& ctx, const int* tokens, const float* tok_emb, const float* pos_emb,
                  float* x, int n_rows, int n_tok, const int* offset_dev, int d);
void launch_embed_rows(const LaunchCtx& ctx, const StepRow* rows, const float* tok_emb, const float* pos_emb, float* x,
                       int n_rows, int d);
void launch_decoder_self_attention_rows(const LaunchCtx& ctx, const float* qkv, const StepRow* rows, long layer_off,
                                        float* out, int n_rows, int d, int n_head, int ctx_len);
void launch_kv_append(const LaunchCtx& ctx, const float* qkv, float* kc, float* vc, int n_rows, int n_tok,
                      const int* offset_dev, int d, int ctx_len);
void launch_kv_append_rows(const LaunchCtx& ctx, const float* qkv, const StepRow* rows, long layer_off, int n_rows, int d);
void launch_decoder_self_attention_anc(const LaunchCtx& ctx, const float* qkv, const float* kc, const float* vc,
                                       const unsigned char* anc, float* out, int n_rows, const int* offset, int d,
                                       int n_head, int ctx_len);
void launch_anc_update(const LaunchCtx& ctx, unsigned char* anc, const int* ctl, const int* offset, int n_rows, int ctx_len);
void launch_anc_update_block(const LaunchCtx& ctx, unsigned char* anc, const int* block, int n_rows, int ctx_len);
void launch_decoder_self_attention(const LaunchCtx& ctx, const float* qkv, const float* kc, const float* vc,
                                   float* out, int n_rows, int n_tok, const int* offset_dev, int d, int n_head,
                                   int ctx_len);
struct CrossAttnArgs {
    const float* q;
    const float* k;
    const float* v;
    long ldkv;
    float* out;
    int rows, d, n_head, T;
    const int* head_rank;
    float* ring;
    const int* ring_row;
    const int* beam_of_row;
    int ring_rows, n_beam;
    float* qk_debug;
    const StepRow* step_rows = nullptr;
    long kv_off = 0;
    const float* xq_x = nullptr;
    const float* xq_w = nullptr;
    const float* xq_b = nullptr;
    const float* xq_gamma = nullptr;
    const float* xq_beta = nullptr;
    float xq_scale = 1.f;
};
void launch_decoder_cross_attention(const LaunchCtx& ctx, const CrossAttnArgs& a);
bool cross_split_folds_query(int d);
void launch_decoder_cross_attention_split(const LaunchCtx& ctx, const CrossAttnArgs& a, float* scores, float* pm,
                                          float* pl, float* po, bool merge = true);
constexpr int kCrossSplitWays = 8;
size_t cross_split_scratch_floats(int rows, int n_head, int T);
void launch_kv_gather(const LaunchCtx& ctx, const float* src, float* dst, const int* source_rows, int n_rows,
                      int len, int d, int ctx_len, int n_layer);

inline int sf_sub_len(int n) { return (n - 1) / 2 + 1; }
void launch_sf_scale_copy(const LaunchCtx& ctx, const float* src, float* dst, long n, float scale);
constexpr int kSfMaxSegments = 8;
struct SfSegments {
    int n = 0;
    int start[kSfMaxSegments] = {0}, len[kSfMaxSegments] = {0};
};
struct SfConvSegs {
    int n = 0, in_total = 0, out_total = 0;
    int in_start[kSfMaxSegments] = {0}, in_len[kSfMaxSegments] = {0}, out_start[kSfMaxSegments] = {0};
};
SfConvSegs sf_conv_segs_next(const SfConvSegs& prev);
void launch_sf_conv0(const LaunchCtx& ctx, const float* in, const float* w, const float* b, float* out, const SfConvSegs& sg, int F,
                     int C);
void launch_sf_dwconv2d(const LaunchCtx& ctx, const float* in, const float* w, const float* b, float* out, const SfConvSegs& sg,
                        int Fi, int C);
void launch_sf_assemble(const LaunchCtx& ctx, const float* ctx_rows, const float* chunk_rows, float* x, const SfSegments& rows,
                        const SfSegments& chunks, int d, float scale);
struct SfAttnArgs {
    const float* q = nullptr; const float* k = nullptr; const float* v = nullptr;
    long ldq = 0, ldk = 0, ldv = 0;
    float* out = nullptr; long ldo = 0;
    int T = 0, n_head = 0, dh = 0;
    float scale = 1.f;
    const float* pos = nullptr; long ldp = 0; int pos_row0 = 0;
    const float* bias_u = nullptr; const float* bias_v = nullptr;
    int n_seg = 0;
    int seg_start[kSfMaxSegments] = {0}, seg_T[kSfMaxSegments] = {0};
};
constexpr int kSfMaxFrames = 512;
void launch_sf_attention(const LaunchCtx& ctx, const SfAttnArgs& a, int form = 0);
void launch_sf_glu_dwconv(const LaunchCtx& ctx, const float* in, const float* w, const float* b, const float* bn_mean,
                          const float* bn_invstd, const float* bn_w, const float* bn_b, float* out, const SfSegments& rows, int d,
                          int taps);
void launch_sf_head(const LaunchCtx& ctx, const float* x, const float* w1t, const float* b1, const float* w2,
                    const float* b2, float* out, int T, int d, int n_spk);
void launch_sf_transpose(const LaunchCtx& ctx, const float* src, float* dst, int rows, int cols);

constexpr int kSfStateMaxKeys = 4096;
// ... 96 lines not shown
```

whisperlivekit_amd/csrc/decoder.hip:

```cpp
#include <cstddef>

#include <cstdlib>

#include "common.h"
#include "wave_ops.h"

namespace wlk {

__global__ __launch_bounds__(128) void embed_kernel(const int* __restrict__ tokens,
                                                    const float* __restrict__ tok_emb,
                                                    const float* __restrict__ pos_emb, float* __restrict__ x,
                                                    int n_tok, const int* __restrict__ offset_p, int d) {
    const int row = blockIdx.x;
    const int p = row % n_tok;
    const int offset = *offset_p;
    const float* e = tok_emb + (long)tokens[row] * d;
    const float* pe = pos_emb + (long)(offset + p) * d;
    for (int c = threadIdx.x; c < d; c += 128) x[(long)row * d + c] = e[c] + pe[c];
}

void launch_embed(const LaunchCtx& ctx, const int* tokens, const float* tok_emb, const float* pos_emb,
                  float* x, int n_rows, int n_tok, const int* offset, int d) {
    KernelScope ks(ctx, "dec_embed");
    hipLaunchKernelGGL(embed_kernel, dim3(n_rows * n_tok), dim3(128), 0, ctx.stream, tokens, tok_emb, pos_emb, x,
                       n_tok, offset, d);
    WLK_HIP(hipGetLastError());
}

__global__ __launch_bounds__(128) void embed_rows_kernel(const StepRow* __restrict__ rows, const float* __restrict__ tok_emb,
                                                         const float* __restrict__ pos_emb, float* __restrict__ x, int d) {
    const int row = blockIdx.x;
    const StepRow sr = rows[row];
    const float* e = tok_emb + (long)sr.token * d;
    const float* pe = pos_emb + (long)sr.offset * d;
    for (int c = threadIdx.x; c < d; c += 128) x[(long)row * d + c] = e[c] + pe[c];
}

void launch_embed_rows(const LaunchCtx& ctx, const StepRow* rows, const float* tok_emb, const float* pos_emb, float* x,
                       int n_rows, int d) {
    KernelScope ks(ctx, "dec_embed");
    hipLaunchKernelGGL(embed_rows_kernel, dim3(n_rows), dim3(128), 0, ctx.stream, rows, tok_emb, pos_emb, x, d);
    WLK_HIP(hipGetLastError());
}

__global__ __launch_bounds__(256) void embed_step_kernel(const StepBlock* __restrict__ host_block, StepBlock* __restrict__ dev_block,
                                                         int* __restrict__ tokens_dev, int* __restrict__ ring_row,
                                                         int* __restrict__ beam_of_row, int* __restrict__ d_offset,
                                                         const float* __restrict__ tok_emb, const float* __restrict__ pos_emb,
                                                         float* __restrict__ x, int d) {
    constexpr int kWords = sizeof(StepBlock) / 4, kHead = sizeof(StepRow) / 4;
    static_assert(kWords <= 512 && sizeof(StepBlock) <= 2048, "two words of the step block per thread");
    __shared__ unsigned head[kHead];
    const int tid = threadIdx.x;
    const unsigned* src = reinterpret_cast<const unsigned*>(host_block);
    unsigned w0 = 0, w1 = 0;
    if (tid < kWords) w0 = __hip_atomic_load(src + tid, __ATOMIC_RELAXED, __HIP_MEMORY_SCOPE_SYSTEM);
    if (tid + 256 < kWords) w1 = __hip_atomic_load(src + tid + 256, __ATOMIC_RELAXED, __HIP_MEMORY_SCOPE_SYSTEM);
    if (tid < kWords) reinterpret_cast<unsigned*>(dev_block)[tid] = w0;
    if (tid + 256 < kWords) reinterpret_cast<unsigned*>(dev_block)[tid + 256] = w1;
    if (tid < kHead) head[tid] = w0;
    __syncthreads();
    const StepRow* row = reinterpret_cast<const StepRow*>(head);
    const int token = row->token, offset = row->offset;
    if (tid == 0) {
        tokens_dev[0] = token;
        ring_row[0] = row->ring_row;
        beam_of_row[0] = 0;
        d_offset[0] = offset;
    }
    const float* e = tok_emb + (long)token * d;
    const float* pe = pos_emb + (long)offset * d;
    for (int c = tid; c < d; c += 256) x[c] = e[c] + pe[c];
}

void launch_embed_step(const LaunchCtx& ctx, const StepBlock* host_block, StepBlock* dev_block, int* tokens_dev,
                       int* ring_row, int* beam_of_row, int* d_offset, const float* tok_emb, const float* pos_emb, float* x,
                       int d) {
    KernelScope ks(ctx, "dec_embed");
    hipLaunchKernelGGL(embed_step_kernel, dim3(1), dim3(256), 0, ctx.stream, host_block, dev_block, tokens_dev, ring_row,
                       beam_of_row, d_offset, tok_emb, pos_emb, x, d);
    WLK_HIP(hipGetLastError());
}

__global__ __launch_bounds__(256) void embed_rows_step_kernel(const EngineBlock* __restrict__ host_block,
                                                              EngineBlock* __restrict__ dev_block,
                                                              const float* __restrict__ tok_emb,
                                                              const float* __restrict__ pos_emb, float* __restrict__ x, int d) {
    constexpr int kWords = sizeof(EngineBlock) / 4, kRowWords = sizeof(StepRow) / 4;
    constexpr int kRow0 = offsetof(EngineBlock, rows) / 4;
    __shared__ unsigned mine[kRowWords];
    const int tid = threadIdx.x, row = blockIdx.x, n_blocks = gridDim.x;
    const unsigned* src = reinterpret_cast<const unsigned*>(host_block);
    unsigned* dst = reinterpret_cast<unsigned*>(dev_block);
    if (tid < kRowWords) mine[tid] = __hip_atomic_load(src + kRow0 + row * kRowWords + tid, __ATOMIC_RELAXED, __HIP_MEMORY_SCOPE_SYSTEM);
    for (int w = row * 256 + tid; w < kWords; w += n_blocks * 256)
        dst[w] = __hip_atomic_load(src + w, __ATOMIC_RELAXED, __HIP_MEMORY_SCOPE_SYSTEM);
    __syncthreads();
    const StepRow* sr = reinterpret_cast<const StepRow*>(mine);
    const float* e = tok_emb + (long)sr->token * d;
    const float* pe = pos_emb + (long)sr->offset * d;
    for (int c = tid; c < d; c += 256) x[(long)row * d + c] = e[c] + pe[c];
}

void launch_embed_rows_step(const LaunchCtx& ctx, const EngineBlock* host_block, EngineBlock* dev_block, const float* tok_emb,
                            const float* pos_emb, float* x, int n_rows, int d) {
    KernelScope ks(ctx, "dec_embed");
    hipLaunchKernelGGL(embed_rows_step_kernel, dim3(n_rows), dim3(256), 0, ctx.stream, host_block, dev_block, tok_emb,
                       pos_emb, x, d);
    WLK_HIP(hipGetLastError());
}

__global__ __launch_bounds__(256) void kv_append_kernel(const float* __restrict__ qkv, float* __restrict__ kc,
                                                        float* __restrict__ vc, int n_tok,
                                                        const int* __restrict__ offset_p, int d, int ctx_len) {
    const int offset = *offset_p;
    const int row = blockIdx.x;
    const int b = row / n_tok, p = row - b * n_tok;
    const float* src = qkv + (long)row * 3 * d;
    const long dst = ((long)b * ctx_len + offset + p) * d;
    for (int c = threadIdx.x; c < d; c += 256) {
        kc[dst + c] = src[d + c];
        vc[dst + c] = src[2 * d + c];
    }
}
// ... 653 lines not shown
```

whisperlivekit_amd/csrc/diag.hip:

```cpp
#include <cstdio>
#include <cmath>
#include <cstdlib>
#include <cstring>
#include <stdexcept>
#include <string>
#include <vector>

#include "../../include/wlk_hip.h"
#include "common.h"
#include "internal.h"
#include "nllb_internal.h"
#include "wave_ops.h"

using namespace wlk;

namespace {
thread_local std::string g_diag_error;
struct DevBuf {
    float* p = nullptr;
    explicit DevBuf(size_t n, const float* host = nullptr) {
        WLK_HIP(hipMalloc(reinterpret_cast<void**>(&p), std::max<size_t>(n, 1) * sizeof(float)));
        if (host) WLK_HIP(hipMemcpy(p, host, n * sizeof(float), hipMemcpyHostToDevice));
    }
    ~DevBuf() { (void)hipFree(p); }
// ... 81 lines not shown
        WLK_HIP(hipDeviceSynchronize());
        WLK_HIP(hipMemcpy(c, Cc.p, (size_t)m * n * sizeof(float), hipMemcpyDeviceToHost));
    });
}

int wlk_diag_linear_time(int m, int n, int k, int flags, int force, int reps, float* us_per_launch) {
    return run([&]() {
        std::vector<float> ha((size_t)m * k), hw((size_t)n * k);
        unsigned seed = 12345u;
        auto rnd = [&]() { seed = seed * 1664525u + 1013904223u; return ((seed >> 8) & 0xffff) / 65536.0f - 0.5f; };
        for (auto& v : ha) v = rnd();
        for (auto& v : hw) v = rnd() * 0.05f;
        DevBuf A((size_t)m * k, ha.data()), W((size_t)n * k, hw.data()), B(n), R((size_t)m * n), Cc((size_t)m * n);
        WLK_HIP(hipMemset(B.p, 0, n * sizeof(float)));
        WLK_HIP(hipMemset(R.p, 0, (size_t)m * n * sizeof(float)));
        GemmArgs g;
        g.A = A.p; g.lda = k; g.W = W.p; g.bias = B.p; g.C = Cc.p; g.ldc = n; g.R = (flags & kGemmResidual) ? R.p : nullptr;
        g.ldr = n; g.M = m; g.N = n; g.K = k; g.flags = flags; g.scale = 0.5f; g.scale_cols = n / 2;
        g.force_kwave = force == 2;
        g.force_kernel = (force >= 2 && force <= 4) || (force >= 6 && force <= 8) || force >= 500 ? force : 0;
        long long* dbg = nullptr;
        const bool want_clock = getenv("WLK_GEMM_CLOCKS") != nullptr;
        if (want_clock) {
            WLK_HIP(hipMalloc(reinterpret_cast<void**>(&dbg), 4 * 8192 * sizeof(long long)));
            WLK_HIP(hipMemset(dbg, 0, 4 * 8192 * sizeof(long long)));
            g.dbg_clock = dbg;
        }
        hipStream_t st;
        WLK_HIP(hipStreamCreateWithFlags(&st, hipStreamNonBlocking));
        LaunchCtx ctx{st, nullptr};
        auto go = [&]() {
            if (force == 1) launch_gemv(ctx, g, "diag");
            else if ((force >= 5 && force <= 8) || force >= 500) launch_gemm_kp(ctx, g, "diag");
            else launch_gemm(ctx, g, "diag");
        };
        go();
        WLK_HIP(hipStreamSynchronize(st));
        hipEvent_t e0, e1;
        WLK_HIP(hipEventCreate(&e0));
        WLK_HIP(hipEventCreate(&e1));
        WLK_HIP(hipEventRecord(e0, st));
        for (int i = 0; i < reps; ++i) go();
        WLK_HIP(hipEventRecord(e1, st));
        WLK_HIP(hipStreamSynchronize(st));
        float ms = 0.f;
        WLK_HIP(hipEventElapsedTime(&ms, e0, e1));
        *us_per_launch = 1e3f * ms / (float)reps;
        if (want_clock) {
            std::vector<long long> h(4 * 8192);
            WLK_HIP(hipMemcpy(h.data(), dbg, h.size() * sizeof(long long), hipMemcpyDeviceToHost));
            long long t0 = 0, t1 = 0;
            double pro = 0, loop = 0, epi = 0;
            int n = 0;
            for (int i = 0; i < 8192; ++i) {
                if (!h[4 * i + 3]) continue;
                if (!n || h[4 * i] < t0) t0 = h[4 * i];
                if (!n || h[4 * i + 3] > t1) t1 = h[4 * i + 3];
                pro += h[4 * i + 1] - h[4 * i]; loop += h[4 * i + 2] - h[4 * i + 1]; epi += h[4 * i + 3] - h[4 * i + 2];
                ++n;
            }
            if (n) fprintf(stderr, "[clocks] %d workgroups: prologue %.0f, loop %.0f, fold+epilogue %.0f ticks (mean); first start -> last end %lld ticks\n",
                           n, pro / n, loop / n, epi / n, t1 - t0);
            (void)hipFree(dbg);
        }
        (void)hipEventDestroy(e0);
        (void)hipEventDestroy(e1);
        (void)hipStreamDestroy(st);
    });
}

int wlk_diag_linear_ln(const float* a, const float* w, const float* bias, const float* gamma, const float* beta, int m,
                       int n, int k, int force_gemv, float* c) {
    return run([&]() {
        DevBuf A((size_t)m * k, a), W((size_t)n * k, w), B(n, bias), G(k, gamma), Bt(k, beta), Cc((size_t)m * n);
        GemmArgs g;
        g.A = A.p; g.lda = k; g.W = W.p; g.bias = B.p; g.C = Cc.p; g.ldc = n; g.M = m; g.N = n; g.K = k;
        g.ln_gamma = G.p; g.ln_beta = Bt.p;
        LaunchCtx ctx;
        (void)force_gemv;
        if (m <= 8) launch_gemv(ctx, g, "diag_gemv_ln");
        else launch_gemm(ctx, g, "diag_gemm_ln");
        WLK_HIP(hipDeviceSynchronize());
        WLK_HIP(hipMemcpy(c, Cc.p, (size_t)m * n * sizeof(float), hipMemcpyDeviceToHost));
    });
}

int wlk_diag_layernorm(const float* x, const float* gamma, const float* beta, int rows, int d, float* y) {
    return run([&]() {
        DevBuf X((size_t)rows * d, x), G(d, gamma), Bt(d, beta), Y((size_t)rows * d);
        LaunchCtx ctx;
        launch_layernorm(ctx, X.p, d, G.p, Bt.p, Y.p, d, rows, d, "diag_ln");
        WLK_HIP(hipDeviceSynchronize());
        WLK_HIP(hipMemcpy(y, Y.p, (size_t)rows * d * sizeof(float), hipMemcpyDeviceToHost));
    });
}

int wlk_diag_prefill_stack(wlk_session** sessions, const int64_t* tokens, const int32_t* n_tok, const int32_t* sot_index, int32_t n,
                           int32_t* taken) {
    if (!sessions || !tokens || !n_tok || !sot_index || !taken || n < 1 || n > kMaxBatch) {
        set_last_error("prefill_stack: bad arguments");
        return WLK_ERR_ARG;
    }
    return run([&]() {
        wlk_model* m = sessions[0]->m;
        WLK_HIP(hipSetDevice(m->device));
        wlk_prefill_ws ws;
        wlk_prefill_ws_alloc(m, ws, kMaxBatch, std::min(256, (int)m->D.n_text_ctx));
        hipStream_t st = nullptr;
        try {
            WLK_HIP(hipStreamCreateWithFlags(&st, hipStreamNonBlocking));
            std::vector<wlk_prefill_item> items(n);
            std::vector<wlk_prefill_item*> stack;
            const int64_t* t = tokens;
            for (int i = 0; i < n; ++i) {
                items[i].s = sessions[i];
                items[i].tokens = t;
                items[i].n_tok = n_tok[i];
                items[i].sot_index = sot_index[i];
                t += n_tok[i];
                WLK_HIP(hipStreamSynchronize(sessions[i]->stream));
                taken[i] = sessions[i]->m == m && wlk_prefill_precheck(items[i], ws).empty() ? 1 : 0;
                if (taken[i]) stack.push_back(&items[i]);
            }
            wlk_prefill_group(stack, LaunchCtx{st, nullptr}, ws);
            WLK_HIP(hipStreamSynchronize(st));
        } catch (...) {
            if (st) (void)hipStreamDestroy(st);
            wlk_prefill_ws_free(ws);
            throw;
        }
        (void)hipStreamDestroy(st);
        wlk_prefill_ws_free(ws);
    });
}

int wlk_diag_encoder_attention_time(int t, int d, int n_head, int reps, float* us_per_launch) {
    return run([&]() {
        std::vector<float> h((size_t)t * 3 * d);
        unsigned seed = 777u;
        for (auto& v : h) { seed = seed * 1664525u + 1013904223u; v = (((seed >> 8) & 0xffff) / 65536.0f - 0.5f) * 1.5f; }
        DevBuf Q((size_t)t * 3 * d, h.data()), O((size_t)t * d);

        hipStream_t st;
        WLK_HIP(hipStreamCreateWithFlags(&st, hipStreamNonBlocking));
        LaunchCtx ctx{st, nullptr};
        auto go = [&]() { launch_encoder_attention(ctx, Q.p, O.p, t, d, n_head); };
        go();
        WLK_HIP(hipStreamSynchronize(st));
        hipEvent_t e0, e1;
        WLK_HIP(hipEventCreate(&e0));
        WLK_HIP(hipEventCreate(&e1));
        WLK_HIP(hipEventRecord(e0, st));
        for (int i = 0; i < reps; ++i) go();
        WLK_HIP(hipEventRecord(e1, st));
        WLK_HIP(hipStreamSynchronize(st));
        float ms = 0.f;
        WLK_HIP(hipEventElapsedTime(&ms, e0, e1));
        *us_per_launch = 1e3f * ms / (float)reps;
        (void)hipEventDestroy(e0);
        (void)hipEventDestroy(e1);
        (void)hipStreamDestroy(st);
    });
}

int wlk_diag_encoder_attention(const float* qkv, int t, int d, int n_head, float* out) {
    return run([&]() {
// ... 1432 lines not shown
```

whisperlivekit_amd/csrc/gemm_f32.hip:

```cpp
#include <algorithm>
#include <atomic>
#include <cstdlib>
#include <type_traits>

#include "common.h"
#include "wave_ops.h"
#include "align_body.h"

namespace wlk {

typedef float f32x16 __attribute__((ext_vector_type(16)));
typedef float f32x4 __attribute__((ext_vector_type(4)));
typedef unsigned int u32x4 __attribute__((ext_vector_type(4)));

constexpr int BK = 32, LDS_LD = BK + 4;

__device__ __forceinline__ float gelu_erf(float x) {
    return 0.5f * x * (1.0f + erff(x * 0.70710678118654752440f));
}

template <int NA, int NW>
struct Stage {
    float4 a[NA], w[NW];
};
// ... 207 lines not shown
    const int frag = (KP ? wave * 8 : wave * SUB) + (lane & 31) * LDS_LD + (lane >> 5) * 4;
    auto mma = [&](int buf) {
#pragma unroll
        for (int s = 0; s < 4; ++s) {
            const float4 a4 = *reinterpret_cast<const float4*>(&As[buf][frag + s * (KP ? SUB : 8)]);
            const float4 b4 = *reinterpret_cast<const float4*>(&Ws[buf][frag + s * (KP ? SUB : 8)]);
            acc = __builtin_amdgcn_mfma_f32_32x32x2f32(a4.x, b4.x, acc, 0, 0, 0);
            acc = __builtin_amdgcn_mfma_f32_32x32x2f32(a4.y, b4.y, acc, 0, 0, 0);
            acc = __builtin_amdgcn_mfma_f32_32x32x2f32(a4.z, b4.z, acc, 0, 0, 0);
            acc = __builtin_amdgcn_mfma_f32_32x32x2f32(a4.w, b4.w, acc, 0, 0, 0);
        }
    };
    const int ns = (g.K + SLAB - 1) / SLAB, ns2 = (ns + 1) & ~1;
    Slab s0, s1;
    fetch(s0, 0);
    fetch(s1, 1);
    stash(s0, 0);
    __syncthreads();
    for (int ks = 0; ks < ns2; ks += 2) {
        fetch(s0, ks + 2);
        __builtin_amdgcn_sched_barrier(0);
        mma(0);
        if constexpr (NBUF == 1) __syncthreads();
        stash(s1, NBUF - 1);
        __syncthreads();
        fetch(s1, ks + 3);
        __builtin_amdgcn_sched_barrier(0);
        mma(NBUF - 1);
        if constexpr (NBUF == 1) __syncthreads();
        stash(s0, 0);
        __syncthreads();
    }
    float* red = &As[0][0];
    if (wave > 0) {
#pragma unroll
        for (int r = 0; r < 16; ++r) red[((wave - 1) * 16 + r) * 64 + lane] = acc[r];
    }
    __syncthreads();
    if (wave > 0) return;
#pragma unroll
    for (int w = 0; w < KW - 1; ++w)
#pragma unroll
        for (int r = 0; r < 16; ++r) acc[r] += red[(w * 16 + r) * 64 + lane];

    const int col = n0 + (lane & 31);
    if (col >= g.N) return;
    const float b = g.bias ? g.bias[col] : 0.f;
    const bool do_scale = (g.flags & kGemmScaleCols) && (g.scale_period ? col % g.scale_period : col) < g.scale_cols;
    const int row_base = m0 + 4 * (lane >> 5);
    float* kv_dst = nullptr;
    int kv_col = 0, kv_off = 0;
    if (g.kcache && col >= g.kv_d) {
        kv_dst = col < 2 * g.kv_d ? g.kcache : g.vcache;
        kv_col = col < 2 * g.kv_d ? col - g.kv_d : col - 2 * g.kv_d;
        kv_off = *g.kv_pos;
    }
    float res[16];
    if (g.flags & kGemmResidual) {
#pragma unroll
        for (int r = 0; r < 16; ++r) res[r] = g.R[(long)min(row_base + (r & 3) + 8 * (r >> 2), g.M - 1) * g.ldr + col];
    } else {
#pragma unroll
        for (int r = 0; r < 16; ++r) res[r] = 0.f;
    }
#pragma unroll
    for (int r = 0; r < 16; ++r) {
        const int row = row_base + (r & 3) + 8 * (r >> 2);
        float v = acc[r] + b;
        if (do_scale) v *= g.scale;
        if (g.flags & kGemmGelu) v = gelu_erf(v);
        if (g.flags & kGemmRelu) v = fmaxf(v, 0.f);
        if (g.flags & kGemmSwish) v = v / (1.0f + expf(-v));
        v += res[r];
        if (row < g.M) {
            g.C[(long)row * g.ldc + col] = v;
            if (kv_dst) {
                const int bm = row / g.kv_ntok, t = row - bm * g.kv_ntok;
                kv_dst[((long)bm * g.kv_ctx + kv_off + t) * g.kv_d + kv_col] = v;
            }
        }
    }
}

template <bool KP = false>
__global__ __launch_bounds__(256) void gemm_nt_f32_kwave16_kernel(GemmArgs g) {
    WLK_PIN_GEMM_ARGS(g);
    constexpr int KW = 4, SLAB = BK * KW, SUB = 16 * LDS_LD;
    __shared__ __attribute__((aligned(16))) float As[2][KW * SUB];
    __shared__ __attribute__((aligned(16))) float Ws[2][KW * SUB];
    const int tid = threadIdx.x, lane = tid & 63, wave = tid >> 6;
    const int tiles_n = (g.N + 15) / 16;
    const int tile_m = blockIdx.x / tiles_n, tile_n = blockIdx.x - tile_m * tiles_n;
    const int m0 = tile_m * 16, n0 = tile_n * 16;

    constexpr unsigned kOob = 0x80000000u;
    const __amdgpu_buffer_rsrc_t rsrc_a = __builtin_amdgcn_make_buffer_rsrc(
        const_cast<float*>(g.A), 0, (int)((((long)g.M - 1) * g.lda + g.K) * 4), 0x00020000);
    const __amdgpu_buffer_rsrc_t rsrc_w = __builtin_amdgcn_make_buffer_rsrc(
        const_cast<float*>(g.W), 0, (int)((long)g.N * g.K * 4), 0x00020000);
    unsigned a_byte[2], w_byte[2];
    int lds_at[2];
    const int c4 = tid & 31, kcol = c4 * 4;
#pragma unroll
    for (int i = 0; i < 2; ++i) {
        const int row = (tid >> 5) + 8 * i;
        a_byte[i] = (m0 + row) < g.M ? (unsigned)(((long)(m0 + row) * g.lda + kcol) * 4) : kOob;
        w_byte[i] = (n0 + row) < g.N ? (unsigned)(((long)(n0 + row) * g.K + kcol) * 4) : kOob;
        lds_at[i] = (c4 >> 3) * SUB + row * LDS_LD + (c4 & 7) * 4;
    }
    struct Slab {
        float4 a[2], w[2];
    };
    auto fetch = [&](Slab& st, int ks) {
        const int k0 = ks * SLAB;
        const bool in = (k0 + kcol) < g.K;
#pragma unroll
        for (int i = 0; i < 2; ++i) {
            const u32x4 v = __builtin_amdgcn_raw_buffer_load_b128(rsrc_a, (int)(in ? a_byte[i] + (unsigned)k0 * 4u : kOob), 0, 0);
            st.a[i] = make_float4(__uint_as_float(v.x), __uint_as_float(v.y), __uint_as_float(v.z), __uint_as_float(v.w));
        }
#pragma unroll
        for (int i = 0; i < 2; ++i) {
            const u32x4 v = __builtin_amdgcn_raw_buffer_load_b128(rsrc_w, (int)(in ? w_byte[i] + (unsigned)k0 * 4u : kOob), 0, 0);
            st.w[i] = make_float4(__uint_as_float(v.x), __uint_as_float(v.y), __uint_as_float(v.z), __uint_as_float(v.w));
        }
    };
    auto stash = [&](const Slab& st, int buf) {
#pragma unroll
        for (int i = 0; i < 2; ++i) *reinterpret_cast<float4*>(&As[buf][lds_at[i]]) = st.a[i];
#pragma unroll
        for (int i = 0; i < 2; ++i) *reinterpret_cast<float4*>(&Ws[buf][lds_at[i]]) = st.w[i];
    };
    f32x4 acc = {0.f, 0.f, 0.f, 0.f};
    const int g4 = lane >> 4;
    const int frag = (KP ? wave * 8 : wave * SUB) + (lane & 15) * LDS_LD + (g4 & 1) * 4;
    const bool odd = (g4 >> 1) != 0;
    auto mma = [&](int buf) {
#pragma unroll
        for (int s = 0; s < 4; ++s) {
            const float4 a4 = *reinterpret_cast<const float4*>(&As[buf][frag + s * (KP ? SUB : 8)]);
            const float4 b4 = *reinterpret_cast<const float4*>(&Ws[buf][frag + s * (KP ? SUB : 8)]);
            acc = __builtin_amdgcn_mfma_f32_16x16x4f32(odd ? a4.y : a4.x, odd ? b4.y : b4.x, acc, 0, 0, 0);
            acc = __builtin_amdgcn_mfma_f32_16x16x4f32(odd ? a4.w : a4.z, odd ? b4.w : b4.z, acc, 0, 0, 0);
        }
    };
    const int ns = (g.K + SLAB - 1) / SLAB, ns2 = (ns + 1) & ~1;
    Slab s0, s1;
    fetch(s0, 0);
    fetch(s1, 1);
    const int col = n0 + (lane & 15);
    const int colc = min(col, g.N - 1);
    const int row_base = m0 + 4 * g4;
    const bool has_res = (g.flags & kGemmResidual) != 0;
    float b = (g.bias ? g.bias + colc : g.W)[0];
    float res[4];
#pragma unroll
    for (int r = 0; r < 4; ++r) res[r] = (has_res ? g.R + (long)min(row_base + r, g.M - 1) * g.ldr + colc : g.W)[0];
    int kv_off = (g.kcache ? g.kv_pos : reinterpret_cast<const int*>(g.W))[0];
    pin_loaded(b);
#pragma unroll
    for (int r = 0; r < 4; ++r) pin_loaded(res[r]);
    asm volatile("" : "+v"(kv_off));
    stash(s0, 0);
    __syncthreads();
    for (int ks = 0; ks < ns2; ks += 2) {
        fetch(s0, ks + 2);
        __builtin_amdgcn_sched_barrier(0);
        mma(0);
        stash(s1, 1);
        __syncthreads();
        fetch(s1, ks + 3);
        __builtin_amdgcn_sched_barrier(0);
        mma(1);
        stash(s0, 0);
        __syncthreads();
    }
    float* red = &As[0][0];
    if (wave > 0) {
#pragma unroll
        for (int r = 0; r < 4; ++r) red[((wave - 1) * 4 + r) * 64 + lane] = acc[r];
    }
    __syncthreads();
    if (wave > 0) return;
#pragma unroll
    for (int w = 0; w < KW - 1; ++w)
#pragma unroll
        for (int r = 0; r < 4; ++r) acc[r] += red[(w * 4 + r) * 64 + lane];

    if (col >= g.N) return;
    if (!g.bias) b = 0.f;
    const bool do_scale = (g.flags & kGemmScaleCols) && (g.scale_period ? col % g.scale_period : col) < g.scale_cols;
    float* kv_dst = nullptr;
    int kv_col = 0;
    if (g.kcache && col >= g.kv_d) {
        kv_dst = col < 2 * g.kv_d ? g.kcache : g.vcache;
        kv_col = col < 2 * g.kv_d ? col - g.kv_d : col - 2 * g.kv_d;
    }
#pragma unroll
    for (int r = 0; r < 4; ++r)
        if (!has_res) res[r] = 0.f;
#pragma unroll
    for (int r = 0; r < 4; ++r) {
        const int row = row_base + r;
        float v = acc[r] + b;
        if (do_scale) v *= g.scale;
        if (g.flags & kGemmGelu) v = gelu_erf(v);
        if (g.flags & kGemmRelu) v = fmaxf(v, 0.f);
        if (g.flags & kGemmSwish) v = v / (1.0f + expf(-v));
        v += res[r];
        if (row < g.M) {
            g.C[(long)row * g.ldc + col] = v;
            if (kv_dst) {
                const int bm = row / g.kv_ntok, t = row - bm * g.kv_ntok;
                kv_dst[((long)bm * g.kv_ctx + kv_off + t) * g.kv_d + kv_col] = v;
            }
        }
    }
}

template <int N, int I = 0, typename F>
__device__ __forceinline__ void static_for(F&& f) {
    if constexpr (I < N) {
        f(std::integral_constant<int, I>{});
        static_for<N, I + 1>(f);
    }
}

__device__ __forceinline__ void lds_barrier() {
    asm volatile("s_waitcnt lgkmcnt(0)" ::: "memory");
    __builtin_amdgcn_s_barrier();
    asm volatile("" ::: "memory");
}

template <int TM, int TN>
struct EpilogueOperands {
    float res[TM * TN][4];
    float bias[TN], mul[TN];
};

template <int TM, int TN>
__device__ __forceinline__ void ksplit_fetch_epilogue(const GemmArgs& g, EpilogueOperands<TM, TN>& eo, int wave, int lane, int m0,
                                                      int n0, const float* gR) {
    const bool has_res = (g.flags & kGemmResidual) != 0, scaled = (g.flags & kGemmScaleCols) != 0;
#pragma unroll
    for (int j = 0; j < TN; ++j) {
        const int col = n0 + 32 * j + (lane & 31);
        eo.bias[j] = g.bias && col < g.N ? g.bias[col] : 0.f;
        eo.mul[j] = scaled && (g.scale_period ? col % g.scale_period : col) < g.scale_cols ? g.scale : 1.0f;
    }
#pragma unroll
    for (int q = 0; q < TM * TN; ++q) {
        const int i = q / TN, j = q % TN;
        const int col = min(n0 + 32 * j + (lane & 31), g.N - 1);
        const int row0 = m0 + 32 * i + 8 * wave + 4 * (lane >> 5);
#pragma unroll
        for (int e = 0; e < 4; ++e) eo.res[q][e] = has_res ? gR[(long)min(row0 + e, g.M - 1) * g.ldr + col] : 0.f;
    }
}

template <int TM, int TN, int LDS_FLOATS>
__device__ __forceinline__ void ksplit_fold_store(const GemmArgs& g, f32x16 (&acc)[TM][TN], const EpilogueOperands<TM, TN>& eo,
                                                  float* lds, int wave, int lane, int m0, int n0, float* gC) {
    constexpr int NT = TM * TN;
    constexpr int RES_FLOATS = NT * 1024, COL_FLOATS = 512;
    constexpr int P_FIT = (LDS_FLOATS - RES_FLOATS - COL_FLOATS) / 4096;
    static_assert(P_FIT >= 1, "no room for the fold");
    constexpr int P = P_FIT < NT ? P_FIT : NT;
    constexpr int PASSES = (NT + P - 1) / P;
    float* resbuf = lds;
    float* colbuf = lds + RES_FLOATS;
    float* red = colbuf + COL_FLOATS;
    const bool gelu = (g.flags & kGemmGelu) != 0, relu = (g.flags & kGemmRelu) != 0, swish = (g.flags & kGemmSwish) != 0;
    static_for<NT>([&](auto Q) {
        constexpr int q = decltype(Q)::value;
        *reinterpret_cast<float4*>(resbuf + (q * 4 + wave) * 256 + lane * 4) =
            make_float4(eo.res[q][0], eo.res[q][1], eo.res[q][2], eo.res[q][3]);
    });
    if (wave == 0 && lane < 32) {
        static_for<TN>([&](auto J) {
            constexpr int j = decltype(J)::value;
            colbuf[j * 32 + lane] = eo.bias[j];
            colbuf[128 + j * 32 + lane] = eo.mul[j];
        });
    }
    static_for<PASSES>([&](auto PP) {
        constexpr int pass = decltype(PP)::value, q_lo = pass * P, q_hi = (q_lo + P < NT ? q_lo + P : NT);
        if constexpr (pass > 0) lds_barrier();
        static_for<q_hi - q_lo>([&](auto T) {
            constexpr int t = decltype(T)::value, q = q_lo + t, i = q / TN, j = q % TN;
            float* dst = red + (t * 4 + wave) * 1024 + lane * 4;
            static_for<4>([&](auto V) {
                constexpr int v = decltype(V)::value;
                *reinterpret_cast<float4*>(dst + v * 256) =
                    make_float4(acc[i][j][4 * v], acc[i][j][4 * v + 1], acc[i][j][4 * v + 2], acc[i][j][4 * v + 3]);
            });
        });
        lds_barrier();
#pragma unroll 1
// ... 188 lines not shown
    const int ntrip = nslab;
    int tt = 0;
    for (; tt + 1 < ntrip; tt += 2) {
        trip(f0, f1, tt);
        trip(f1, f0, tt + 1);
    }
    if (tt < ntrip) trip(f0, f1, tt);
    wait_vmcnt<0>();
    __syncthreads();
    const long long t_fold = g.dbg_clock ? (long long)__builtin_readcyclecounter() : 0;

    ksplit_fold_store<TM, TN, Cfg::LDS_FLOATS>(g, acc, eo, lds, wave, lane, m0, n0, gC);
    if (g.dbg_clock && threadIdx.x == 0) {
        long long* d = g.dbg_clock + 4 * ((long)blockIdx.y * gridDim.x + blockIdx.x);
        d[0] = t_start; d[1] = t_loop; d[2] = t_fold; d[3] = (long long)__builtin_readcyclecounter();
    }
}

template <int TM, int TN>
static void launch_kpipe(const LaunchCtx& ctx, const GemmArgs& g) {
    using Cfg = KPipeCfg<TM, TN>;
    static_assert(Cfg::LDS_BYTES <= 160 * 1024, "ring does not fit the 160 KiB LDS");
    static std::atomic<uint64_t> configured{0};
    int dev = 0;
    WLK_HIP(hipGetDevice(&dev));
    if (!(configured.load(std::memory_order_acquire) >> (dev & 63) & 1)) {
        WLK_HIP(hipFuncSetAttribute(reinterpret_cast<const void*>(&gemm_nt_f32_kpipe_kernel<TM, TN>),
                                    hipFuncAttributeMaxDynamicSharedMemorySize, (int)Cfg::LDS_BYTES));
        configured.fetch_or(1ull << (dev & 63), std::memory_order_release);
    }
    const int tiles_m = (g.M + Cfg::BM - 1) / Cfg::BM, tiles_n = (g.N + Cfg::BN - 1) / Cfg::BN;
    const int blocks = tiles_m >= 8 ? 8 * ((tiles_m + 3) / 4) * ((tiles_n + 1) / 2) : tiles_m * tiles_n;
    hipLaunchKernelGGL((gemm_nt_f32_kpipe_kernel<TM, TN>), dim3(blocks, std::max(g.batch, 1)), dim3(256), Cfg::LDS_BYTES,
                       ctx.stream, g);
}

#define WLK_KPIPE_TILES(X) X(3, 4) X(3, 3) X(3, 2) X(3, 1) X(2, 4) X(2, 2) X(2, 1) X(4, 2)
bool gemm_kpipe_has_tile(int tm, int tn) {
#define WLK_KP(a, b) if (tm == a && tn == b) return true;
    WLK_KPIPE_TILES(WLK_KP)
#undef WLK_KP
    return false;
}
static bool dispatch_kpipe(const LaunchCtx& ctx, const GemmArgs& g, int tm, int tn) {
#define WLK_KP(a, b) if (tm == a && tn == b) { launch_kpipe<a, b>(ctx, g); return true; }
    WLK_KPIPE_TILES(WLK_KP)
#undef WLK_KP
    return false;
}

struct KSplitTile { int tm, tn; };
static KSplitTile ksplit_tile(int M, int N, int K, bool forced = false) {
    if (K % 64 != 0 || K < 256 || M < 512) return {0, 0};
    if (!forced && (N > 1536 || K < 512)) return {0, 0};
#define WLK_KP(a, b) {a, b},
    static const KSplitTile cand[] = {WLK_KPIPE_TILES(WLK_KP)};
#undef WLK_KP
    KSplitTile best{0, 0};
    double best_cost = 0.0;
    for (const KSplitTile& c : cand) {
        const long tiles = (long)((M + 32 * c.tm - 1) / (32 * c.tm)) * ((N + 32 * c.tn - 1) / (32 * c.tn));
        const double cost = ((tiles + 255) / 256) * (c.tm * c.tn * (K / 8.0) + 48.0 + 2.0 * (c.tm + c.tn) * (K / 64.0));
        if (best.tm == 0 || cost < best_cost) { best = c; best_cost = cost; }
    }
    return best;
}

static long kwave_max_tiles() {
    static const long v = [] {
        const char* e = getenv("WLK_KWAVE_MAX_TILES");
        return e ? atol(e) : 416L;
    }();
    return v;
}

bool gemm_takes_kwave(int M, int N, int K) {
    const long tiles32 = (long)((N + 31) / 32) * ((M + 31) / 32);
    return K >= 256 && tiles32 <= kwave_max_tiles();
}

bool gemm_takes_ksplit(int M, int N, int K) { return ksplit_tile(M, N, K).tm != 0; }

void x3_refresh_env_switches();
void refresh_env_switches() { x3_refresh_env_switches(); }

static GemmPlan gemm_plan_tiled(const GemmArgs& g) {
    GemmPlan p;
    auto refuse = [&](const char* why) {
        p = GemmPlan{};
        p.refusal = why;
        return p;
    };
    if (g.K % 4 != 0 || g.lda % 4 != 0) return refuse("gemm: K and lda must be multiples of 4");
    if ((((long)g.M - 1) * g.lda + g.K) * 4 >= (1L << 31) || (long)g.N * g.K * 4 >= (1L << 31))
        return refuse("gemm: operand larger than 2 GiB");
    if (g.ln_gamma) return refuse("gemm: only the GEMV kernels (rows <= 8) take the LayerNorm; launch it separately");
    if (g.batch > kMaxBatch) return refuse("gemm: batch too large");
    const bool want_kwave = g.force_kwave || g.force_kernel == 2;
    const KSplitTile kt = (want_kwave || g.kcache || g.force_kernel == 3) ? KSplitTile{0, 0} : ksplit_tile(g.M, g.N, g.K, g.force_kernel == 4);
    if (g.force_kernel == 4 && !kt.tm) return refuse("gemm: the k-pipe kernel does not take this shape");
    if (kt.tm) {
        p.kernel = GemmPlan::kKpipe;
        p.tm = kt.tm;
        p.tn = kt.tn;
        return p;
    }
    const long tiles64 = (long)((g.N + 63) / 64) * ((g.M + 63) / 64);
    if (g.batch > 0 && (gemm_takes_kwave(g.M, g.N, g.K) || want_kwave || tiles64 < 64))
        return refuse("gemm: batched launches are only available on the tiled paths");
    if (g.kcache && !(gemm_takes_kwave(g.M, g.N, g.K) || want_kwave))
        return refuse("gemm: fused KV-cache append is only available on the k-wave path");
    if ((gemm_takes_kwave(g.M, g.N, g.K) && g.force_kernel != 3) || (want_kwave && g.K >= 256))
        p.kernel = g.M <= 128 && g.force_kernel != 2 ? GemmPlan::kKwave16 : GemmPlan::kKwave;
    else
        p.kernel = tiles64 >= 64 ? GemmPlan::kTiled64 : GemmPlan::kTiled32;
    return p;
}

static void launch_gemm_plan(const LaunchCtx& ctx, const GemmArgs& g, const GemmPlan& p, const char* tag) {
    if (p.kernel == GemmPlan::kRefused) throw std::invalid_argument(p.refusal);
    const double nb = std::max(g.batch, 1);
    KernelScope ks(ctx, tag, nb * 2.0 * g.M * g.N * g.K,
                   4.0 * (nb * (double)g.M * g.K + (double)g.N * g.K + nb * (double)g.M * g.N));
    const int tiles_n = (g.N + 63) / 64;
    const long tiles32 = (long)((g.N + 31) / 32) * ((g.M + 31) / 32);
    const long tiles16 = (long)((g.N + 15) / 16) * ((g.M + 15) / 16);
    switch (p.kernel) {
    case GemmPlan::kKpipe:
        if (!dispatch_kpipe(ctx, g, p.tm, p.tn)) throw std::logic_error("gemm: k-pipe tile without an instantiation");
        break;
    case GemmPlan::kKwave16:
        hipLaunchKernelGGL(gemm_nt_f32_kwave16_kernel<>, dim3((unsigned)tiles16), dim3(256), 0, ctx.stream, g);
        break;
    case GemmPlan::kKwave:
        hipLaunchKernelGGL(gemm_nt_f32_kwave_kernel<false>, dim3((unsigned)tiles32), dim3(256), 0, ctx.stream, g);
        break;
    case GemmPlan::kTiled64: {
        const int tiles_m = (g.M + 63) / 64;
        const int blocks = tiles_m >= 8 ? 8 * ((tiles_m + 3) / 4) * ((tiles_n + 1) / 2) : tiles_m * tiles_n;
        hipLaunchKernelGGL((gemm_nt_f32_kernel<64, 64>), dim3(blocks, std::max(g.batch, 1)), dim3(256), 0, ctx.stream, g);
        break;
    }
    case GemmPlan::kTiled32: {
        const int tiles_m = (g.M + 31) / 32;
        const int blocks = tiles_m >= 8 ? 8 * ((tiles_m + 3) / 4) * ((tiles_n + 1) / 2) : tiles_m * tiles_n;
        hipLaunchKernelGGL((gemm_nt_f32_kernel<32, 64>), dim3(blocks), dim3(128), 0, ctx.stream, g);
        break;
    }
    case GemmPlan::kKpKwave16:
        hipLaunchKernelGGL((gemm_nt_f32_kwave16_kernel<true>), dim3((unsigned)tiles16), dim3(256), 0, ctx.stream, g);
        break;
    case GemmPlan::kKpKwave1:
        hipLaunchKernelGGL((gemm_nt_f32_kwave_kernel<true, 1>), dim3((unsigned)tiles32), dim3(256), 0, ctx.stream, g);
        break;
    case GemmPlan::kKpKwave2:
        hipLaunchKernelGGL(gemm_nt_f32_kwave_kernel<true>, dim3((unsigned)tiles32), dim3(256), 0, ctx.stream, g);
        break;
    case GemmPlan::kRefused:
        break;
    }
    WLK_HIP(hipGetLastError());
}

void launch_gemm(const LaunchCtx& ctx, const GemmArgs& g, const char* tag) {
    if (g.M <= 0 || g.N <= 0) return;
    launch_gemm_plan(ctx, g, gemm_plan(g, false), tag);
}

static bool kp16_rule(int M, int N, int K, long tiles16) {
    if (N <= 512 && K <= 1024) return true;
    if (K > 1024) return M <= 320;
    if (N == 1024) return M <= 320;
    return tiles16 <= 1300;
}
static KSplitTile kp_tile(int M, int N, int K) {
    const int band = M < 900 ? 0 : M < 1800 ? 1 : M < 2800 ? 2 : 3;
    struct Row { int n, k; int t[4][2]; };
    static const Row rows[] = {
        {2048, 512, {{3, 2}, {2, 1}, {2, 2}, {2, 1}}},
        {512, 2048, {{2, 1}, {3, 1}, {3, 2}, {2, 4}}},
        {1536, 512, {{3, 2}, {2, 2}, {2, 2}, {2, 2}}},
        {512, 512, {{2, 1}, {3, 1}, {3, 2}, {2, 4}}},
        {1024, 512, {{3, 1}, {3, 2}, {2, 1}, {2, 1}}},
        {192, 768, {{2, 1}, {2, 1}, {2, 1}, {3, 1}}},
        {192, 512, {{2, 1}, {2, 1}, {2, 1}, {3, 1}}},
    };
    for (const Row& r : rows)
        if (r.n == N && r.k == K) return KSplitTile{r.t[band][0], r.t[band][1]};
    if (N == 256 && K == 256) return M < 4000 ? KSplitTile{2, 1} : M < 9000 ? KSplitTile{2, 2} : KSplitTile{2, 1};
    return ksplit_tile(M, N, K, true);
}
static bool kp_takes_16(int M, int N, int K, int force) {
    if (force == 6) return true;
    if (force == 7 || force == 8) return false;
    const long tiles16 = (long)((N + 15) / 16) * ((M + 15) / 16);
    return kp16_rule(M, N, K, tiles16);
}
bool gemm_kp_takes_kpipe(int M, int N, int K) { return K % 128 == 0 && K >= 256 && M >= 512 && ksplit_tile(M, N, K, true).tm != 0; }
static GemmPlan gemm_plan_kp(const GemmArgs& g) {
    GemmPlan p;
    auto refuse = [&](const char* why) {
        p = GemmPlan{};
        p.refusal = why;
        return p;
    };
    if (g.K % 4 != 0 || g.lda % 4 != 0) return refuse("gemm: K and lda must be multiples of 4");
    if (g.batch > 0 || g.kcache) return refuse("gemm (kp family): plain projections only");
    if (g.ln_gamma) return refuse("gemm (kp family): the LayerNorm is a launch of its own");
    const bool short_k_kwave = g.K % 32 == 0 && g.K >= 128 && g.K < 256;
    if (!short_k_kwave && (g.K % 128 != 0 || g.K < 256)) {
        GemmArgs t = g;
        t.force_kernel = 3;
        return gemm_plan_tiled(t);
    }
    if ((((long)g.M - 1) * g.lda + g.K) * 4 >= (1L << 31) || (long)g.N * g.K * 4 >= (1L << 31))
        return refuse("gemm: operand larger than 2 GiB");
    if (!short_k_kwave && gemm_kp_takes_kpipe(g.M, g.N, g.K)) {
        KSplitTile kt = kp_tile(g.M, g.N, g.K);
        if (g.force_kernel >= 500) kt = KSplitTile{(g.force_kernel - 500) / 10, (g.force_kernel - 500) % 10};
        p.kernel = GemmPlan::kKpipe;
        p.tm = kt.tm;
        p.tn = kt.tn;
    } else if ((!short_k_kwave || g.M < 512) && kp_takes_16(g.M, g.N, g.K, g.force_kernel)) {
        p.kernel = GemmPlan::kKpKwave16;
    } else {
        const long tiles32 = (long)((g.N + 31) / 32) * ((g.M + 31) / 32);
        const bool one_buf = g.force_kernel == 8 || (g.force_kernel != 7 && tiles32 > 512);
        p.kernel = one_buf ? GemmPlan::kKpKwave1 : GemmPlan::kKpKwave2;
    }
    return p;
}

GemmPlan gemm_plan(const GemmArgs& g, bool kp_family) { return kp_family ? gemm_plan_kp(g) : gemm_plan_tiled(g); }

void launch_gemm_kp(const LaunchCtx& ctx, const GemmArgs& g, const char* tag) {
    if (g.M <= 0 || g.N <= 0) return;
    launch_gemm_plan(ctx, g, gemm_plan(g, true), tag);
}

template <int MR, int RPW>
__global__ __launch_bounds__(256) void gemv_f32_kernel(GemmArgs g) {
    WLK_PIN_GEMM_ARGS(g);
    extern __shared__ __attribute__((aligned(16))) float xs[];
    const int side = g.side_blocks;
    if ((int)blockIdx.x < side) {
        const AlignArgs a = *g.side_align;
        const int fblock = (int)blockIdx.x % g.side_zf, rest = (int)blockIdx.x / g.side_zf;
        align_zscore_body(a, fblock, rest % a.n_align, rest / a.n_align);
        return;
    }
    const int blk = (int)blockIdx.x - side, n_blk = (int)gridDim.x - side;
    const int tid = threadIdx.x;
    const int lane = tid & 63;
    const int wave = tid >> 6;
    const int K4 = g.K >> 2;
    const int n_groups = (g.N + RPW - 1) / RPW;
    const int grp0 = blk * 4 + wave;
    float4 wpre[RPW];
#pragma unroll
    for (int r = 0; r < RPW; ++r) {
        const int n = min(grp0 * RPW + r, g.N - 1);
        const bool ok = grp0 < n_groups && lane < K4;
        const float4 t = *reinterpret_cast<const float4*>(g.W + (long)(ok ? n : 0) * g.K + (ok ? lane : 0) * 4);
        wpre[r] = t;
    }
    constexpr int kLnKeep = 8;
    [[maybe_unused]] float gq[kLnKeep], bq[kLnKeep];
    {
        const float* gp = g.ln_gamma ? g.ln_gamma : g.W;
        const float* bp = g.ln_gamma ? g.ln_beta : g.W;
#pragma unroll
        for (int i = 0; i < kLnKeep; ++i) {
            const int c = lane + 64 * i;
            gq[i] = gp[c < g.K ? c : 0];
            bq[i] = bp[c < g.K ? c : 0];
        }
    }
    const int ep_r = lane / MR, ep_m = lane - ep_r * MR;
    const int ep_n0 = min(grp0 * RPW + (ep_r < RPW ? ep_r : 0), g.N - 1);
    const int ep_mm = ep_m < g.M ? ep_m : 0;
    const float bias0 = (g.bias ? g.bias + ep_n0 : g.W)[0];
    const float res0 = ((g.flags & kGemmResidual) ? g.R + (long)ep_mm * g.ldr + ep_n0 : g.W)[0];
    static_assert(sizeof(StepRow) == 64, "the dummy StepRow read below stays inside the first weight row");
    const StepRow kv_row0 = (g.kv_rows ? g.kv_rows + ep_mm : reinterpret_cast<const StepRow*>(g.W))[0];
    const int kv_pos0 = (g.kcache ? g.kv_pos : reinterpret_cast<const int*>(g.W))[0];
    for (int i = tid; i < MR * K4; i += 256) {
        const int m = i / K4, c = i - m * K4;
        float4 v = make_float4(0.f, 0.f, 0.f, 0.f);
        if (m < g.M) v = *reinterpret_cast<const float4*>(g.A + (long)m * g.lda + c * 4);
        reinterpret_cast<float4*>(xs)[i] = v;
    }
// ... 355 lines not shown
            pmv[j][s] = mg.pm[base + s];
            plv[j][s] = mg.pl[base + s];
            pov[j][s] = *reinterpret_cast<const float4*>(mg.po + (base + s) * 64 + dd);
        }
    }
    float bias_v = bias[n];
    float res_v = R[n];
    const int kv_pos = *t.kv_pos;
    WLK_PIN_S(t.C); WLK_PIN_S(t.kcache); WLK_PIN_S(t.vcache); WLK_PIN_S(t.flags); WLK_PIN_S(t.scale);
    WLK_PIN_S(t.scale_cols); WLK_PIN_S(t.kv_d); WLK_PIN_S(kv_pos);
    __builtin_amdgcn_sched_barrier(0);

#pragma unroll
    for (int j = 0; j < NCH; ++j) {
        float M = pmv[j][0];
#pragma unroll
        for (int s = 1; s < kCrossSplitWays; ++s) M = fmaxf(M, pmv[j][s]);
        float L = 0.f;
        float f[kCrossSplitWays];
#pragma unroll
        for (int s = 0; s < kCrossSplitWays; ++s) {
            f[s] = expf(pmv[j][s] - M);
            L += plv[j][s] * f[s];
        }
        float4 acc = make_float4(0.f, 0.f, 0.f, 0.f);
#pragma unroll
        for (int s = 0; s < kCrossSplitWays; ++s) {
            const float4 o = pov[j][s];
            acc.x += o.x * f[s]; acc.y += o.y * f[s]; acc.z += o.z * f[s]; acc.w += o.w * f[s];
        }
        const int c = (int)threadIdx.x + 256 * j;
        if (c < K4) reinterpret_cast<float4*>(xs)[c] = make_float4(acc.x / L, acc.y / L, acc.z / L, acc.w / L);
    }
    __syncthreads();
    float acc = 0.f;
#pragma unroll
    for (int u = 0; u < UB; ++u) {
        const float4 x = reinterpret_cast<const float4*>(xs)[lane + 64 * u];
        acc = fmaf(w[u].x, x.x, acc);
        acc = fmaf(w[u].y, x.y, acc);
        acc = fmaf(w[u].z, x.z, acc);
        acc = fmaf(w[u].w, x.w, acc);
    }
    acc = wave_sum(acc);
    asm volatile("" ::"v"(bias_v), "v"(res_v));
    if (lane == 0 && (int)blockIdx.x * 4 + wave < N) {
        float o = acc;
        if (bias != W) o += bias_v;
        if ((t.flags & kGemmScaleCols) && n < t.scale_cols) o *= t.scale;
        if (t.flags & kGemmGelu) o = gelu_erf(o);
        if (t.flags & kGemmRelu) o = fmaxf(o, 0.f);
        if (t.flags & kGemmSwish) o = o / (1.0f + expf(-o));
        if (t.flags & kGemmResidual) o += res_v;
        t.C[n] = o;
    }
}

static bool gemv1_enabled() {
    static const bool on = getenv("WLK_NO_GEMV1") == nullptr;
    return on;
}

static bool gemv1_merge_through_lds(int K) {
    const char* e = getenv("WLK_MERGE_FOLD_LDS");
    const char* w = getenv("WLK_MERGE_FOLD");
    return K > 512 && K <= 2048 && K % 256 == 0 && !(e && e[0] == '0') && !(w && w[0] == '1');
}
bool gemv1_folds_merge(int K) {
    if (getenv("WLK_NO_MERGE_FOLD") != nullptr || !gemv1_enabled() || K > 2048 || K % 64 != 0) return false;
    const char* e = getenv("WLK_MERGE_FOLD");
    return (e && e[0] == '1') || K <= 512 || gemv1_merge_through_lds(K);
}

GemvPlan gemv_plan(const GemmArgs& g) {
    GemvPlan p;
    auto refuse = [&](const char* why) {
        p = GemvPlan{};
        p.refusal = why;
        return p;
    };
    if (!gemv_applicable(g.M, g.K) || g.lda % 4 != 0) return refuse("gemv: unsupported shape");
    if (g.scale_period > 0) return refuse("gemv: scale_period is a GEMM operand (the GEMV kernels scale columns below scale_cols only)");
    if (g.batch > 0) return refuse("gemv: batched operand tables are a GEMM operand");
    p.rpw = g.N >= 16384 ? 4 : (g.N >= 2048 ? 2 : 1);
    p.ln = g.ln_gamma != nullptr;
    p.mg = g.mg_pm != nullptr;
    if (p.mg && !(g.M == 1 && g.K <= 2048 && p.rpw <= 2 && gemv1_enabled() && !p.ln))
        return refuse("gemv: the merged cross-attention operand needs the single-row kernel");
    const bool plain1 = p.rpw == 1 && !p.ln && !p.mg;
    if (g.side_blocks > 0 && (!g.side_align || g.side_zf <= 0 || p.rpw != 4))
        return refuse("gemv: side workgroups ride only in the vocabulary projection's launch");
    if (g.M == 1 && (g.K <= 2048 || (plain1 && g.K <= 5120)) && p.rpw <= 2 && gemv1_enabled() && !g.kv_rows) {
        const int ub = (g.K / 4 + 63) / 64;
        if (p.mg && g.mg_side_blocks > 0 && !g.mg_side_heads)
            return refuse("gemv: the merged operand's side blocks need the layer's alignment head list");
        if (p.mg && p.rpw == 1 && !g.kcache && gemv1_merge_through_lds(g.K)) {
            if (!(ub == 3 || ub == 4 || ub == 5 || ub == 6 || ub == 8))
                return refuse("gemv: no workgroup-merge instantiation for this width");
            p.kernel = GemvPlan::kSingleRowMergeLds;
            p.width = ub;
            p.full = true;
            return p;
        }
        p.kernel = GemvPlan::kSingleRow;
        if (ub <= 2) p.width = 2;
        else if (ub <= 8) p.width = p.mg ? (ub <= 4 ? 4 : 8) : (ub == 7 ? 8 : ub);
        else p.width = ub <= 12 ? 12 : ub <= 16 ? 16 : 20;
        p.full = g.K == 256 * p.width;
        return p;
    }
    p.kernel = GemvPlan::kStaged;
    p.width = gemv_row_bucket(g.M);
    p.mg = false;
    p.full = false;
    return p;
}

void launch_gemv(const LaunchCtx& ctx, const GemmArgs& g, const char* tag) {
    if (g.M <= 0 || g.N <= 0) return;
    const GemvPlan p = gemv_plan(g);
    if (p.kernel == GemvPlan::kRefused) throw std::invalid_argument(p.refusal);
    const int n_groups = (g.N + p.rpw - 1) / p.rpw;
    int blocks = (n_groups + 3) / 4;
    if (blocks > 2048) blocks = 2048;
    KernelScope ks(ctx, tag, 2.0 * g.M * g.N * g.K, 4.0 * ((double)g.M * g.K + (double)g.N * g.K + (double)g.M * g.N));
    if (p.kernel != GemvPlan::kStaged) {
        blocks += g.mg_pm ? g.mg_side_blocks : 0;
        const float* bias = g.bias ? g.bias : g.W;
        const float* res = (g.flags & kGemmResidual) ? g.R : g.W;
        Gemv1Tail t{g.C, g.kcache, g.vcache, g.kcache ? g.kv_pos : reinterpret_cast<const int*>(g.W), g.flags, g.scale,
                    g.scale_cols, g.kv_d};
        Gemv1Merge mg{g.mg_pm, g.mg_pl, g.mg_po, g.mg_scores, g.mg_head_rank, g.mg_side_heads, g.mg_ring, g.mg_ring_row,
                      g.mg_beam_of_row, g.mg_T, g.mg_ring_rows, g.mg_n_beam, g.mg_side_blocks};
        if (p.kernel == GemvPlan::kSingleRowMergeLds) {
#define WLK_GEMV1_MGL(UBv)                                                                                             \
    hipLaunchKernelGGL((gemv1_mgl_f32_kernel<UBv>), dim3(blocks), dim3(256), 0, ctx.stream, g.W, g.K, g.N, bias, res, t, mg)
            switch (p.width) {
                case 3: WLK_GEMV1_MGL(3); break;
                case 4: WLK_GEMV1_MGL(4); break;
                case 5: WLK_GEMV1_MGL(5); break;
                case 6: WLK_GEMV1_MGL(6); break;
                case 8: WLK_GEMV1_MGL(8); break;
                default: throw std::logic_error("gemv: workgroup-merge plan without an instantiation");
            }
#undef WLK_GEMV1_MGL
            WLK_HIP(hipGetLastError());
            return;
        }
#define WLK_GEMV1_F(UBv, RPWv, LNv, MGv, FULLv)                                                                         \
    hipLaunchKernelGGL((gemv1_f32_kernel<UBv, RPWv, LNv, MGv, FULLv>), dim3(blocks), dim3(256), 0, ctx.stream, g.W, g.A, \
                       g.K, g.N, g.ln_gamma, g.ln_beta, bias, res, t, mg)
#define WLK_GEMV1_I(UBv, RPWv, LNv, MGv)                       \
    do {                                                       \
        if (p.full) WLK_GEMV1_F(UBv, RPWv, LNv, MGv, true);    \
        else WLK_GEMV1_F(UBv, RPWv, LNv, MGv, false);          \
    } while (0)
#define WLK_GEMV1_R(UBv, LNv, MGv)                   \
    do {                                             \
        if (p.rpw == 2) WLK_GEMV1_I(UBv, 2, LNv, MGv); \
        else WLK_GEMV1_I(UBv, 1, LNv, MGv);          \
    } while (0)
#define WLK_GEMV1_NOMG(UBv)                                    \
    do {                                                       \
        if (p.ln) WLK_GEMV1_R(UBv, true, false);               \
        else WLK_GEMV1_R(UBv, false, false);                   \
    } while (0)
// ... 49 lines not shown
```

whisperlivekit_amd/csrc/internal.h:

```cpp
#pragma once
#include <algorithm>
#include <map>
#include <memory>
#include <chrono>
#include <cstdlib>
#include <thread>
#include <mutex>
#include <stdexcept>
#include <string>
#include <vector>

#include "../../include/wlk_hip.h"
#include "common.h"

namespace wlk {

const std::string& get_last_error();

template <typename F>
inline int guarded(F&& f) {
    try {
        return f();
    } catch (const HipError& e) {
        set_last_error(e.what());
// ... 21 lines not shown
        hipEvent_t a, b;
        double flops, bytes;
    };
    std::vector<Rec> recs;
    std::vector<hipEvent_t> pool;
    hipEvent_t pending = nullptr;
    const char* pending_name = nullptr;
    double pending_flops = 0.0, pending_bytes = 0.0;
    hipEvent_t get() {
        if (!pool.empty()) {
            hipEvent_t e = pool.back();
            pool.pop_back();
            return e;
        }
        hipEvent_t e;
        WLK_HIP(hipEventCreate(&e));
        return e;
    }
};

struct TensorSlot {
    std::string name;
    uint64_t offset, numel;
};


struct LayerW {
    const float *ln1w, *ln1b, *qkvw, *qkvb, *outw, *outb, *ln2w, *ln2b, *fc1w, *fc1b, *fc2w, *fc2b;
    const float *lnxw = nullptr, *lnxb = nullptr, *xqw = nullptr, *xqb = nullptr, *xkvw = nullptr, *xkvb = nullptr,
                *xoutw = nullptr, *xoutb = nullptr;
    const unsigned short *qkvw3 = nullptr, *fc1w3 = nullptr;
    const unsigned short *outw3 = nullptr, *fc2w3 = nullptr;
};

template <typename T>
inline T* dev_alloc(size_t n) {
    T* p = nullptr;
    WLK_HIP(hipMalloc(reinterpret_cast<void**>(&p), n * sizeof(T)));
    return p;
}
template <typename T>
inline T* dev_alloc_zero(size_t n, hipStream_t s) {
    T* p = dev_alloc<T>(n);
    WLK_HIP(hipMemsetAsync(p, 0, n * sizeof(T), s));
    return p;
}

struct DevBytes {
    char* p = nullptr;
    size_t bytes = 0;
    void* host = nullptr;
    DevBytes() = default;
    explicit DevBytes(size_t n, const void* from = nullptr) { alloc(n, from); }
    DevBytes(const DevBytes&) = delete;
    DevBytes& operator=(const DevBytes&) = delete;
    ~DevBytes() { (void)hipFree(p); }
    void alloc(size_t n, const void* from = nullptr) {
        bytes = n;
        WLK_HIP(hipMalloc(reinterpret_cast<void**>(&p), std::max<size_t>(n, 64)));
        if (from && n) WLK_HIP(hipMemcpy(p, from, n, hipMemcpyHostToDevice));
    }
    void mirror(const void* h, size_t n) {
        alloc(n, h);
        host = const_cast<void*>(h);
    }
    void back() const { if (host) back(host); }
    void back(void* to) const { if (bytes) WLK_HIP(hipMemcpy(to, p, bytes, hipMemcpyDeviceToHost)); }
    template <typename T> T* as() const { return reinterpret_cast<T*>(p); }
    float* f() const { return as<float>(); }
    int* i() const { return as<int>(); }
};

}

struct wlk_engine;
struct wlk_session;
struct wlk_model;

struct wlk_prefill_ws {
    int cap_rows = 0;
    int cap_session_rows = 0;
    float *dx = nullptr, *dh = nullptr, *dqkv = nullptr, *datt = nullptr, *dq = nullptr, *dmlp = nullptr, *hsel = nullptr,
          *logits = nullptr, *part = nullptr;
    wlk::StepRow *rows_dev = nullptr, *tiles_dev = nullptr;
    int *ring_row_dev = nullptr, *zeros_dev = nullptr;
    char* pinned = nullptr;
    size_t pinned_bytes = 0;
};
struct wlk_prefill_item {
    wlk_session* s = nullptr;
    const int64_t* tokens = nullptr;
    int n_tok = 0, sot_index = 0;
    int rc = 0;
    std::string err;
};

struct wlk_model {
    wlk_dims D{};
    int device = 0;
    float* arena = nullptr;
    bool owns_arena = false;
    uint64_t arena_floats = 0;
    std::vector<wlk::TensorSlot> slots;
    std::map<std::string, const wlk::TensorSlot*> by_name;
    double* twiddle = nullptr;
    float* xkv_all_w = nullptr;
    float* xkv_all_b = nullptr;
    unsigned short* xkv_all_w3 = nullptr;
    std::vector<unsigned short*> x3_owned;
    int* filt_lo = nullptr;
    int* filt_hi = nullptr;
    int* head_rank = nullptr;
    int* layer_ranks = nullptr;
    int* layer_heads = nullptr;
    int* all_ranks = nullptr;
    std::vector<int> layer_rank_count;
    std::vector<int> align_pairs;
    int n_align = 0;
    bool finalized = false;
    std::vector<wlk::LayerW> enc_layers, dec_layers;
    const float *w_tok_emb = nullptr, *w_dec_pos = nullptr, *w_ln_w = nullptr, *w_ln_b = nullptr;
    wlk_engine* engine = nullptr;
    std::mutex engine_mu;
    float* cif_w = nullptr;
    float cif_b = 0.f;

    const float* w(const std::string& name) const {
        auto it = by_name.find(name);
        if (it == by_name.end()) throw std::invalid_argument("unknown tensor " + name);
        return arena + it->second->offset;
    }
};


struct wlk_session {
    wlk_model* m = nullptr;
    int beam = 1;
    int audio_cap = 0;
    hipStream_t stream = nullptr;
    wlk::Profiler prof;
    bool prof_on = false;
    bool debug = false;
    bool use_graph = true;
    hipGraphExec_t step_exec[2] = {nullptr, nullptr};
    short* pcm16_dev = nullptr;

    float* audio[2] = {nullptr, nullptr};
    int audio_cur = 0;
    int audio_len = 0;

    float *logmel = nullptr, *frame_max = nullptr, *mel_t = nullptr;
    float *logmel_alt = nullptr, *frame_max_alt = nullptr;
    int mel_cached_samples = 0, mel_cached_frames = 0, mel_dirty_head = 0;
    bool mel_incremental = true;
    int frame_cap = 0;
    float *x1p = nullptr, *ex = nullptr, *eh = nullptr, *eqkv = nullptr, *eatt = nullptr, *emlp = nullptr,
          *enc_out = nullptr, *cross_kv = nullptr;
    unsigned short *eh3 = nullptr, *enc_out3 = nullptr;
    unsigned short* emlp3 = nullptr;
    bool enc_out_is_x3 = false;
    unsigned short* eqkv3 = nullptr;
    bool encoded = false;
    int content_len = 0;

    int max_rows = 0;
    int* tokens_dev = nullptr;
    float *dx = nullptr, *dh = nullptr, *dqkv = nullptr, *datt = nullptr, *dq = nullptr, *dmlp = nullptr;
    float* kcache[2] = {nullptr, nullptr};
    float* vcache[2] = {nullptr, nullptr};
    int kv_cur = 0;
    int self_len = 0;
    int n_steps = 0;
    int prefill_rows = 0;
    int last_rows = 0, last_ntok = 0;
    float *hsel = nullptr, *logits_last = nullptr, *logits_sot = nullptr;
    bool have_sot = false;
    int* step_in = nullptr;
    int *ring_row = nullptr, *beam_of_row = nullptr, *d_offset = nullptr;
    float* ring = nullptr;
    int ring_rows = 0;
    float *z = nullptr, *attn_last = nullptr;
    float* qk_debug = nullptr;
    float* xsplit = nullptr;
    float* fsplit = nullptr;
    static constexpr int kFlashSplitsMax = 16;
    static int flash_splits();

    int *adj_row = nullptr, *src_rows = nullptr;
    float* top_vals = nullptr;
    void* topk_scratch = nullptr;
    int *top_ids = nullptr, *frames = nullptr;
    float* probs = nullptr;
    static constexpr int kAdjCap = 4096;
    void* pinned = nullptr;
    static constexpr size_t kPinnedBytes = 1 << 20;
    void* dec_stage = nullptr;
    hipEvent_t dec_stage_ev = nullptr;
    bool dec_stage_used = false;
    void* audio_stage = nullptr;
    hipEvent_t audio_stage_ev = nullptr;
    unsigned char* rules_mask = nullptr;
    int* pick_out = nullptr;
    bool audio_stage_used = false;
    wlk::StepBlock *step_host = nullptr, *step_host_dev = nullptr, *step_dev = nullptr;
    wlk::StepResult *result_host = nullptr, *result_host_dev = nullptr;
    hipGraphExec_t fstep_exec[2] = {nullptr, nullptr};
    wlk::AlignArgs* step_align_dev = nullptr;
    unsigned step_seq = 0;
    uint64_t step_ns = 0, step_launch_ns = 0, step_count = 0;

    unsigned char* anc = nullptr;
    hipGraphExec_t bstep_exec[2] = {nullptr, nullptr};
    bool anc_live = false;
    uint64_t anc_steps = 0;

    wlk::LaunchCtx ctx() { return wlk::LaunchCtx{stream, prof_on ? &prof : nullptr}; }
    bool align_raw_scores = false;
    float* wa_buf = nullptr;
    size_t wa_cap = 0;
    bool survey = false;
    float* survey_buf = nullptr;
    size_t survey_cap = 0;
    wlk_engine* engine = nullptr;
    float* cif_alpha = nullptr;
    wlk_cif_out *cif_host = nullptr, *cif_host_dev = nullptr;
    unsigned cif_seq = 0;
    int cif_T = -1;
    hipStream_t cif_stream = nullptr;
};


inline wlk::StepRow next_step_row(const wlk_session* s, int token, int content_len) {
    wlk::StepRow r;
    r.kcache = s->kcache[s->kv_cur];
    r.vcache = s->vcache[s->kv_cur];
    r.cross_kv = s->cross_kv;
    r.ring = s->ring;
    wlk::step_row_scalars(r, s->n_steps, s->self_len, s->prefill_rows, s->m->D.n_text_ctx, token, content_len);
    return r;
}

inline void wlk_wait_step_flags(hipStream_t stream, const wlk::StepResult* res, int n, unsigned seq) {
    static const long spin_us = [] {
        const char* e = getenv("WLK_STEP_SPIN_US");
        return e ? atol(e) : 400L;
    }();
    const auto t_start = std::chrono::steady_clock::now();
    auto all_set = [&]() {
        for (int i = 0; i < n; ++i)
            if (__atomic_load_n(&res[i].flag_topk, __ATOMIC_ACQUIRE) != seq || __atomic_load_n(&res[i].flag_align, __ATOMIC_ACQUIRE) != seq)
// ... 75 lines not shown
```

whisperlivekit_amd/csrc/wave_ops.h:

```cpp
#pragma once
#include <hip/hip_runtime.h>

namespace wlk {

typedef const __attribute__((address_space(1))) float* gcf_ptr;
typedef float wlk_v4f __attribute__((ext_vector_type(4)));
typedef const __attribute__((address_space(1))) wlk_v4f* gcf4_ptr;
__device__ __forceinline__ gcf_ptr to_global(const float* p) { return (gcf_ptr)p; }
__device__ __forceinline__ float4 ldg4(gcf_ptr p) {
    const wlk_v4f t = *(gcf4_ptr)p;
    return make_float4(t.x, t.y, t.z, t.w);
}

__device__ __forceinline__ void pin_loaded(float4& a) { asm volatile("" : "+v"(a.x), "+v"(a.y), "+v"(a.z), "+v"(a.w)); }
__device__ __forceinline__ void pin_loaded(float& a) { asm volatile("" : "+v"(a)); }

template <int CTRL>
__device__ __forceinline__ float dpp_f32(float v) {
    return __builtin_bit_cast(float, __builtin_amdgcn_update_dpp(0, __builtin_bit_cast(int, v), CTRL, 0xf, 0xf, true));
}
template <int CTRL>
__device__ __forceinline__ int dpp_i32(int v) {
    return __builtin_amdgcn_update_dpp(0, v, CTRL, 0xf, 0xf, true);
}

__device__ __forceinline__ void swap32(float v, float& a, float& b) {
    a = v;
    b = v;
    asm volatile("s_nop 1\n\tv_permlane32_swap_b32 %0, %1" : "+v"(a), "+v"(b));
}
__device__ __forceinline__ void swap16(float v, float& a, float& b) {
    a = v;
    b = v;
    asm volatile("s_nop 1\n\tv_permlane16_swap_b32 %0, %1" : "+v"(a), "+v"(b));
}

template <int OFF>
__device__ __forceinline__ float wave_xor(float v) {
    static_assert(OFF == 1 || OFF == 2 || OFF == 4 || OFF == 8 || OFF == 16 || OFF == 32, "butterfly offsets only");
    if constexpr (OFF == 32) {
        float a, b;
        swap32(v, a, b);
        return (__lane_id() & 32) ? a : b;
    } else if constexpr (OFF == 16) {
        float a, b;
        swap16(v, a, b);
        return (__lane_id() & 16) ? a : b;
    } else if constexpr (OFF == 8) {
        return dpp_f32<0x128>(v);
    } else if constexpr (OFF == 4) {
        return dpp_f32<0x1B>(dpp_f32<0x141>(v));
    } else if constexpr (OFF == 2) {
        return dpp_f32<0x4E>(v);
    } else {
        return dpp_f32<0xB1>(v);
    }
}
template <int OFF>
__device__ __forceinline__ int wave_xor(int v) {
    return __builtin_bit_cast(int, wave_xor<OFF>(__builtin_bit_cast(float, v)));
}

__device__ __forceinline__ float wave_sum(float v) {
    float a, b;
    swap32(v, a, b);
    v = a + b;
    swap16(v, a, b);
    v = a + b;
    v += dpp_f32<0x128>(v);
    v += dpp_f32<0x1B>(dpp_f32<0x141>(v));
    v += dpp_f32<0x4E>(v);
    v += dpp_f32<0xB1>(v);
    return v;
}

__device__ __forceinline__ float wave_max(float v) {
    float a, b;
    swap32(v, a, b);
    v = fmaxf(a, b);
    swap16(v, a, b);
    v = fmaxf(a, b);
    v = fmaxf(v, dpp_f32<0x128>(v));
    v = fmaxf(v, dpp_f32<0x1B>(dpp_f32<0x141>(v)));
    v = fmaxf(v, dpp_f32<0x4E>(v));
    v = fmaxf(v, dpp_f32<0xB1>(v));
    return v;
}

__device__ __forceinline__ float row16_sum_1248(float v) {
    v += dpp_f32<0xB1>(v);
    v += dpp_f32<0x4E>(v);
    v += dpp_f32<0x1B>(dpp_f32<0x141>(v));
    v += dpp_f32<0x128>(v);
    return v;
}

__device__ __forceinline__ void wave_argmax(float& bv, int& bi) {
#define WLK_ARGMAX_LEVEL(OFF)                                              \
    {                                                                      \
        const float ov = wave_xor<OFF>(bv);                                \
        const int oi = wave_xor<OFF>(bi);                                  \
        if (ov > bv || (ov == bv && oi < bi)) { bv = ov; bi = oi; }        \
    }
    WLK_ARGMAX_LEVEL(32)
    WLK_ARGMAX_LEVEL(16)
    WLK_ARGMAX_LEVEL(8)
    WLK_ARGMAX_LEVEL(4)
    WLK_ARGMAX_LEVEL(2)
    WLK_ARGMAX_LEVEL(1)
#undef WLK_ARGMAX_LEVEL
}

}
```

Before: 204.5 audio_s/s.

## Fuse decoder prefill LayerNorms into GEMM loads via per-16-column row statistics

The residual-epilogue GEMMs and the embedding kernels now write per-16-column mean and M2 partials for each row. The next k-wave GEMM combines these partials into a row mean and rstd and applies LayerNorm as it loads A. This drops the separate LayerNorm launches and the dh round-trip in multi-row decoder prefill, both for a single session and for stacked sessions. The route is gated by an env switch and shape checks (rows > 8, d % 16 == 0), forces the 16x16 k-wave kernel, and adds register pressure plus a small stats buffer.

After: 204.0 audio_s/s (median of 2 runs). Within noise of the previous version (-0.2%).

```diff
diff --git a/include/wlk_hip.h b/include/wlk_hip.h
--- a/include/wlk_hip.h
+++ b/include/wlk_hip.h
@@ -370,6 +370,9 @@
 int wlk_diag_linear_time(int m, int n, int k, int flags, int force_gemv, int reps, float* us_per_launch);
 int wlk_diag_linear_ln(const float* a, const float* w, const float* bias, const float* gamma, const float* beta,
                        int m, int n, int k, int force_gemv, float* c);
+int wlk_diag_linear_ln_stats(const float* x0, const float* w1, const float* bias1, const float* res, const float* gamma,
+                             const float* beta, const float* w2, const float* bias2, int m, int d, int k1, int n2, int two_launch,
+                             int stats_rows, float* stats, float* y1, float* y2);
 int wlk_diag_layernorm(const float* x, const float* gamma, const float* beta, int rows, int d, float* y);
 int wlk_diag_prefill_stack(wlk_session** sessions, const int64_t* tokens, const int32_t* n_tok, const int32_t* sot_index, int32_t n,
                            int32_t* taken);
diff --git a/whisperlivekit_amd/_lib.py b/whisperlivekit_amd/_lib.py
--- a/whisperlivekit_amd/_lib.py
+++ b/whisperlivekit_amd/_lib.py
@@ -352,6 +352,7 @@
                                       C.POINTER(C.c_float), C.POINTER(C.c_int8), C.POINTER(C.c_float)]),
         "wlk_diag_linear_time": (cint, [cint, cint, cint, cint, cint, cint, C.POINTER(C.c_float)]),
         "wlk_diag_linear_ln": (cint, [p, p, p, p, p, cint, cint, cint, cint, p]),
+        "wlk_diag_linear_ln_stats": (cint, [p, p, p, p, p, p, p, p, cint, cint, cint, cint, cint, cint, p, p, p]),
         "wlk_diag_layernorm": (cint, [p, p, p, cint, cint, p]),
         "wlk_diag_encoder_attention_time": (cint, [cint, cint, cint, cint, C.POINTER(C.c_float)]),
         "wlk_diag_encoder_attention": (cint, [p, cint, cint, cint, p]),
@@ -425,7 +426,7 @@
     "wlk_nllb_batch_create", "wlk_nllb_batch_destroy", "wlk_nllb_batch_encode", "wlk_nllb_batch_step", "wlk_nllb_batch_release",
     "wlk_nllb_batch_export", "wlk_nllb_batch_cross_attention", "wlk_nllb_batch_sync",
     "wlk_nllb_batch_set_align", "wlk_nllb_batch_prefill", "wlk_nllb_batch_step_align", "wlk_nllb_batch_align_stats",
-    "wlk_diag_last_error", "wlk_diag_linear", "wlk_diag_linear_time", "wlk_diag_linear_ln", "wlk_diag_layernorm",
+    "wlk_diag_last_error", "wlk_diag_linear", "wlk_diag_linear_time", "wlk_diag_linear_ln", "wlk_diag_linear_ln_stats", "wlk_diag_layernorm",
     "wlk_diag_encoder_attention", "wlk_diag_encoder_attention_time", "wlk_diag_wave_ops", "wlk_diag_env_refresh",
     "wlk_diag_linear_x3", "wlk_diag_linear_x3_time", "wlk_diag_layernorm_x3",
     "wlk_diag_encoder_attention_x3", "wlk_diag_encoder_attention_x3_time", "wlk_diag_qkv_x3_attention",
diff --git a/whisperlivekit_amd/csrc/api.hip b/whisperlivekit_amd/csrc/api.hip
--- a/whisperlivekit_amd/csrc/api.hip
+++ b/whisperlivekit_amd/csrc/api.hip
@@ -439,6 +439,7 @@
         s->datt = dev_alloc<float>(R * d);
         s->dq = dev_alloc<float>(R * d);
         s->dmlp = dev_alloc<float>(R * 4 * d);
+        s->ln_part = dev_alloc<float2>(R * ((d + 15) / 16));
         const size_t cache = (size_t)D.n_text_layer * beam * ctx * d;
         s->kcache[0] = dev_alloc<float>(cache);
         s->vcache[0] = dev_alloc<float>(cache);
@@ -503,6 +504,7 @@
     int* il[] = {s->step_in, s->adj_row, s->src_rows};
     for (int* p : il)
         if (p) (void)hipFree(p);
+    if (s->ln_part) (void)hipFree(s->ln_part);
     for (auto& e : s->step_exec)
         if (e) (void)hipGraphExecDestroy(e);
     for (auto& e : s->bstep_exec)
@@ -676,11 +678,14 @@
 }
 
 static void transformer_mlp(const LaunchCtx& c, const LayerW& L, float* x, float* h, float* mlp, int rows, int d,
-                            const char* t_ln, const char* t_fc1, const char* t_fc2) {
+                            const char* t_ln, const char* t_fc1, const char* t_fc2, float2* ln_part = nullptr) {
     GemmArgs g;
     g.lda = d; g.W = L.fc1w; g.bias = L.fc1b; g.C = mlp; g.ldc = 4 * d; g.M = rows; g.N = 4 * d; g.K = d;
     g.flags = kGemmGelu;
-    if (gemv_applicable(rows, d)) {
+    if (ln_part) {
+        g.A = x; g.ln_gamma = L.ln2w; g.ln_beta = L.ln2b; g.ln_stats = ln_part;
+        launch_gemm(c, g, t_fc1);
+    } else if (gemv_applicable(rows, d)) {
         g.A = x; g.ln_gamma = L.ln2w; g.ln_beta = L.ln2b;
         launch_gemv(c, g, "dec_ln2_fc1");
     } else {
@@ -691,6 +696,7 @@
     GemmArgs g2;
     g2.A = mlp; g2.lda = 4 * d; g2.W = L.fc2w; g2.bias = L.fc2b; g2.C = x; g2.ldc = d; g2.M = rows; g2.N = d;
     g2.K = 4 * d; g2.flags = kGemmResidual; g2.R = x; g2.ldr = d;
+    g2.stats_out = ln_part;
     launch_linear(c, g2, t_fc2);
 }
 
@@ -957,6 +963,7 @@
         WLK_HIP(hipMemcpyAsync(s->step_in, s->dec_stage, (size_t)(3 * s->max_rows + 1) * sizeof(int), hipMemcpyHostToDevice,
                                s->stream));
     const bool fused = gemv_applicable(R, d) && n_tok == 1;
+    float2* const ln_part = !fused && !step_block && prefill_ln_stats_applicable(R, d) ? s->ln_part : nullptr;
     if (ancestry) {
         if (!fused || step_block || !s->anc) throw std::logic_error("decode: the ancestry step needs the fused beam step");
         WLK_HIP(hipMemcpyAsync(s->src_rows, static_cast<char*>(s->dec_stage) + kAncStageOffset, 8 * sizeof(int),
@@ -968,7 +975,7 @@
         launch_embed_step(c, s->step_host_dev, s->step_dev, s->tokens_dev, s->ring_row, s->beam_of_row, s->d_offset,
                           m->w_tok_emb, m->w_dec_pos, s->dx, d);
     else
-        launch_embed(c, s->tokens_dev, m->w_tok_emb, m->w_dec_pos, s->dx, n_rows, n_tok, s->d_offset, d);
+        launch_embed(c, s->tokens_dev, m->w_tok_emb, m->w_dec_pos, s->dx, n_rows, n_tok, s->d_offset, d, ln_part);
     const float scale = std::pow((float)kHeadDim, -0.25f);
     const size_t cache_layer = (size_t)s->beam * ctx_len * d;
     bool scores_dumped = false;
@@ -985,8 +992,12 @@
             g.kcache = kc; g.vcache = vc; g.kv_pos = s->d_offset; g.kv_d = d; g.kv_ctx = ctx_len;
             launch_gemv(c, g, "dec_ln1_qkv_kv");
         } else {
-            launch_layernorm(c, s->dx, d, L.ln1w, L.ln1b, s->dh, d, R, d, "dec_ln1");
-            g.A = s->dh;
+            if (ln_part) {
+                g.A = s->dx; g.ln_gamma = L.ln1w; g.ln_beta = L.ln1b; g.ln_stats = ln_part;
+            } else {
+                launch_layernorm(c, s->dx, d, L.ln1w, L.ln1b, s->dh, d, R, d, "dec_ln1");
+                g.A = s->dh;
+            }
             if (!gemv_applicable(R, d) && gemm_takes_kwave(R, 3 * d, d)) {
                 g.kcache = kc; g.vcache = vc; g.kv_pos = s->d_offset; g.kv_d = d; g.kv_ctx = ctx_len; g.kv_ntok = n_tok;
                 launch_gemm(c, g, "dec_qkv");
@@ -1002,6 +1013,7 @@
         GemmArgs o;
         o.A = s->datt; o.lda = d; o.W = L.outw; o.bias = L.outb; o.C = s->dx; o.ldc = d; o.M = R; o.N = d; o.K = d;
         o.flags = kGemmResidual; o.R = s->dx; o.ldr = d;
+        o.stats_out = ln_part;
         launch_linear(c, o, "dec_out");
 
         GemmArgs q;
@@ -1013,6 +1025,9 @@
         } else if (fused) {
             q.A = s->dx; q.ln_gamma = L.lnxw; q.ln_beta = L.lnxb;
             launch_gemv(c, q, "dec_lnx_xq");
+        } else if (ln_part) {
+            q.A = s->dx; q.ln_gamma = L.lnxw; q.ln_beta = L.lnxb; q.ln_stats = ln_part;
+            launch_gemm(c, q, "dec_xq");
         } else {
             launch_layernorm(c, s->dx, d, L.lnxw, L.lnxb, s->dh, d, R, d, "dec_lnx");
             q.A = s->dh;
@@ -1077,8 +1092,9 @@
         GemmArgs xo = xo_mg;
         xo.A = s->datt; xo.lda = d; xo.W = L.xoutw; xo.bias = L.xoutb; xo.C = s->dx; xo.ldc = d; xo.M = R; xo.N = d;
         xo.K = d; xo.flags = kGemmResidual; xo.R = s->dx; xo.ldr = d;
+        xo.stats_out = ln_part;
         launch_linear(c, xo, "dec_xout");
-        transformer_mlp(c, L, s->dx, s->dh, s->dmlp, R, d, "dec_ln2", "dec_fc1", "dec_fc2");
+        transformer_mlp(c, L, s->dx, s->dh, s->dmlp, R, d, "dec_ln2", "dec_fc1", "dec_fc2", ln_part);
     }
     if (scores_dumped && m->n_align > 0 && !raw_pass)
         launch_ring_softmax(c, s->ring, s->ring_row, s->beam_of_row, m->all_ranks, m->n_align, R, s->ring_rows, s->beam, T);
@@ -1124,6 +1140,7 @@
     ws.datt = dev_alloc<float>(R * d);
     ws.dq = dev_alloc<float>(R * d);
     ws.dmlp = dev_alloc<float>(R * 4 * d);
+    ws.ln_part = dev_alloc<float2>(R * ((d + 15) / 16));
     ws.hsel = dev_alloc<float>((size_t)2 * max_sessions * d);
     ws.logits = dev_alloc<float>((size_t)8 * V);
     ws.part = dev_alloc<float>(flash_split_scratch_floats((int)R, (int)H, wlk_session::kFlashSplitsMax));
@@ -1138,7 +1155,7 @@
 
 extern "C++" void wlk_prefill_ws_free(wlk_prefill_ws& ws) {
     void* dev[] = {ws.dx, ws.dh, ws.dqkv, ws.datt, ws.dq, ws.dmlp, ws.hsel, ws.logits, ws.part, ws.rows_dev, ws.tiles_dev,
-                   ws.ring_row_dev, ws.zeros_dev};
+                   ws.ring_row_dev, ws.zeros_dev, ws.ln_part};
     for (void* p : dev)
         if (p) (void)hipFree(p);
     if (ws.pinned) (void)hipHostFree(ws.pinned);
@@ -1212,7 +1229,12 @@
     WLK_HIP(hipMemcpyAsync(ws.tiles_dev, tiles_h, (size_t)(R / 32) * sizeof(StepRow), hipMemcpyHostToDevice, c.stream));
     WLK_HIP(hipMemcpyAsync(ws.ring_row_dev, ring_row_h, (size_t)R * sizeof(int), hipMemcpyHostToDevice, c.stream));
 
-    launch_embed_rows(c, ws.rows_dev, m->w_tok_emb, m->w_dec_pos, ws.dx, R, d);
+    const bool ln_stats = prefill_ln_stats_applicable(items[0]->n_tok, d);
+    for (int i = 1; i < B; ++i)
+        if (prefill_ln_stats_applicable(items[i]->n_tok, d) != ln_stats)
+            throw std::logic_error("stacked prefill: the sessions' own prefills take different LayerNorm routes");
+    float2* const ln_part = ln_stats ? ws.ln_part : nullptr;
+    launch_embed_rows(c, ws.rows_dev, m->w_tok_emb, m->w_dec_pos, ws.dx, R, d, ln_part);
     const float scale = std::pow((float)kHeadDim, -0.25f);
     const size_t cache_layer = (size_t)D.n_text_ctx * d;
     auto linear = [&](const float* A, long lda, const float* W, const float* bias, float* C, long ldc, int N, int K, int flags,
@@ -1221,10 +1243,19 @@
         g.A = A; g.lda = lda; g.W = W; g.bias = bias; g.C = C; g.ldc = ldc; g.M = R; g.N = N; g.K = K;
         g.flags = flags; g.R = Rs; g.ldr = ldc; g.scale = sc; g.scale_cols = sc_cols;
         g.force_kwave = true;
+        if (flags & kGemmResidual) g.stats_out = ln_part;
         launch_gemm(c, g, tag);
     };
     auto ln_linear = [&](const float* gamma, const float* beta, const float* W, const float* bias, float* C, long ldc, int N,
                          int flags, float sc, int sc_cols, const char* t_ln, const char* tag) {
+        if (ln_part) {
+            GemmArgs g;
+            g.A = ws.dx; g.lda = d; g.W = W; g.bias = bias; g.C = C; g.ldc = ldc; g.M = R; g.N = N; g.K = d;
+            g.flags = flags; g.scale = sc; g.scale_cols = sc_cols;
+            g.ln_gamma = gamma; g.ln_beta = beta; g.ln_stats = ln_part;
+            launch_gemm(c, g, tag);
+            return;
+        }
         launch_layernorm(c, ws.dx, d, gamma, beta, ws.dh, d, R, d, t_ln);
         linear(ws.dh, d, W, bias, C, ldc, N, d, flags, nullptr, sc, sc_cols, tag);
     };
diff --git a/whisperlivekit_amd/csrc/common.h b/whisperlivekit_amd/csrc/common.h
--- a/whisperlivekit_amd/csrc/common.h
+++ b/whisperlivekit_amd/csrc/common.h
@@ -172,6 +172,8 @@
     long long* dbg_clock = nullptr;
     const float* ln_gamma = nullptr;
     const float* ln_beta = nullptr;
+    float2* stats_out = nullptr;
+    const float2* ln_stats = nullptr;
     float* kcache = nullptr;
     float* vcache = nullptr;
     const int* kv_pos = nullptr;
@@ -239,6 +241,9 @@
 GemvPlan gemv_plan(const GemmArgs& g);
 bool gemv1_folds_merge(int K);
 void refresh_env_switches();
+constexpr int kLnStatsMaxK = 1536;
+bool prefill_ln_stats_enabled();
+bool prefill_ln_stats_applicable(int rows, int d);
 inline void launch_linear(const LaunchCtx& ctx, const GemmArgs& g, const char* tag) {
     if (gemv_applicable(g.M, g.K)) launch_gemv(ctx, g, tag);
     else launch_gemm(ctx, g, tag);
@@ -442,9 +447,9 @@
                          const int* ranks_dev, int n_ranks, int rows, int ring_rows, int n_beam, int T);
 
 void launch_embed(const LaunchCtx& ctx, const int* tokens, const float* tok_emb, const float* pos_emb,
-                  float* x, int n_rows, int n_tok, const int* offset_dev, int d);
+                  float* x, int n_rows, int n_tok, const int* offset_dev, int d, float2* stats = nullptr);
 void launch_embed_rows(const LaunchCtx& ctx, const StepRow* rows, const float* tok_emb, const float* pos_emb, float* x,
-                       int n_rows, int d);
+                       int n_rows, int d, float2* stats = nullptr);
 void launch_decoder_self_attention_rows(const LaunchCtx& ctx, const float* qkv, const StepRow* rows, long layer_off,
                                         float* out, int n_rows, int d, int n_head, int ctx_len);
 void launch_kv_append(const LaunchCtx& ctx, const float* qkv, float* kc, float* vc, int n_rows, int n_tok,
diff --git a/whisperlivekit_amd/csrc/decoder.hip b/whisperlivekit_amd/csrc/decoder.hip
--- a/whisperlivekit_amd/csrc/decoder.hip
+++ b/whisperlivekit_amd/csrc/decoder.hip
@@ -6,40 +6,52 @@
 #include "wave_ops.h"
 
 namespace wlk {
+
+__device__ __forceinline__ void embed_store(float* __restrict__ x, float2* __restrict__ stats, int row, int c, int d, float v) {
+    x[(long)row * d + c] = v;
+    if (stats) {
+        const float2 st = row16_stats(v);
+        if ((c & 15) == 0) stats[(long)row * (d >> 4) + (c >> 4)] = st;
+    }
+}
 
 __global__ __launch_bounds__(128) void embed_kernel(const int* __restrict__ tokens,
                                                     const float* __restrict__ tok_emb,
                                                     const float* __restrict__ pos_emb, float* __restrict__ x,
-                                                    int n_tok, const int* __restrict__ offset_p, int d) {
+                                                    int n_tok, const int* __restrict__ offset_p, int d,
+                                                    float2* __restrict__ stats) {
     const int row = blockIdx.x;
     const int p = row % n_tok;
     const int offset = *offset_p;
     const float* e = tok_emb + (long)tokens[row] * d;
     const float* pe = pos_emb + (long)(offset + p) * d;
-    for (int c = threadIdx.x; c < d; c += 128) x[(long)row * d + c] = e[c] + pe[c];
+    for (int c = threadIdx.x; c < d; c += 128) embed_store(x, stats, row, c, d, e[c] + pe[c]);
 }
 
 void launch_embed(const LaunchCtx& ctx, const int* tokens, const float* tok_emb, const float* pos_emb,
-                  float* x, int n_rows, int n_tok, const int* offset, int d) {
+                  float* x, int n_rows, int n_tok, const int* offset, int d, float2* stats) {
+    if (stats && d % 16 != 0) throw std::invalid_argument("embed: row statistics need d % 16 == 0");
     KernelScope ks(ctx, "dec_embed");
     hipLaunchKernelGGL(embed_kernel, dim3(n_rows * n_tok), dim3(128), 0, ctx.stream, tokens, tok_emb, pos_emb, x,
-                       n_tok, offset, d);
+                       n_tok, offset, d, stats);
     WLK_HIP(hipGetLastError());
 }
 
 __global__ __launch_bounds__(128) void embed_rows_kernel(const StepRow* __restrict__ rows, const float* __restrict__ tok_emb,
-                                                         const float* __restrict__ pos_emb, float* __restrict__ x, int d) {
+                                                         const float* __restrict__ pos_emb, float* __restrict__ x, int d,
+                                                         float2* __restrict__ stats) {
     const int row = blockIdx.x;
     const StepRow sr = rows[row];
     const float* e = tok_emb + (long)sr.token * d;
     const float* pe = pos_emb + (long)sr.offset * d;
-    for (int c = threadIdx.x; c < d; c += 128) x[(long)row * d + c] = e[c] + pe[c];
+    for (int c = threadIdx.x; c < d; c += 128) embed_store(x, stats, row, c, d, e[c] + pe[c]);
 }
 
 void launch_embed_rows(const LaunchCtx& ctx, const StepRow* rows, const float* tok_emb, const float* pos_emb, float* x,
-                       int n_rows, int d) {
+                       int n_rows, int d, float2* stats) {
+    if (stats && d % 16 != 0) throw std::invalid_argument("embed: row statistics need d % 16 == 0");
     KernelScope ks(ctx, "dec_embed");
-    hipLaunchKernelGGL(embed_rows_kernel, dim3(n_rows), dim3(128), 0, ctx.stream, rows, tok_emb, pos_emb, x, d);
+    hipLaunchKernelGGL(embed_rows_kernel, dim3(n_rows), dim3(128), 0, ctx.stream, rows, tok_emb, pos_emb, x, d, stats);
     WLK_HIP(hipGetLastError());
 }
 
diff --git a/whisperlivekit_amd/csrc/diag.hip b/whisperlivekit_amd/csrc/diag.hip
--- a/whisperlivekit_amd/csrc/diag.hip
+++ b/whisperlivekit_amd/csrc/diag.hip
@@ -187,6 +187,42 @@
         else launch_gemm(ctx, g, "diag_gemm_ln");
         WLK_HIP(hipDeviceSynchronize());
         WLK_HIP(hipMemcpy(c, Cc.p, (size_t)m * n * sizeof(float), hipMemcpyDeviceToHost));
+    });
+}
+
+int wlk_diag_linear_ln_stats(const float* x0, const float* w1, const float* bias1, const float* res, const float* gamma,
+                             const float* beta, const float* w2, const float* bias2, int m, int d, int k1, int n2, int two_launch,
+                             int stats_rows, float* stats, float* y1, float* y2) {
+    if (!x0 || !w1 || !bias1 || !res || !gamma || !beta || !w2 || !bias2 || !y1 || !y2 || m < 1 || d < 16 || d % 16 != 0 ||
+        k1 < 4 || n2 < 1 || (stats && stats_rows < m)) {
+        set_diag_error("linear_ln_stats: bad arguments");
+        return WLK_ERR_ARG;
+    }
+    return run([&]() {
+        const size_t np = (size_t)d / 16;
+        DevBuf X0((size_t)m * k1, x0), W1((size_t)d * k1, w1), B1(d, bias1), Rs((size_t)m * d, res), G(d, gamma), Bt(d, beta),
+            W2((size_t)n2 * d, w2), B2(n2, bias2), Y1((size_t)m * d), H((size_t)m * d), Y2((size_t)m * n2),
+            St((size_t)std::max(stats_rows, m) * np * 2, stats);
+        LaunchCtx ctx;
+        GemmArgs a;
+        a.A = X0.p; a.lda = k1; a.W = W1.p; a.bias = B1.p; a.C = Y1.p; a.ldc = d; a.M = m; a.N = d; a.K = k1;
+        a.flags = kGemmResidual; a.R = Rs.p; a.ldr = d;
+        GemmArgs b;
+        b.lda = d; b.W = W2.p; b.bias = B2.p; b.C = Y2.p; b.ldc = n2; b.M = m; b.N = n2; b.K = d;
+        if (two_launch) {
+            launch_gemm(ctx, a, "diag_ln_stats_producer");
+            launch_layernorm(ctx, Y1.p, d, G.p, Bt.p, H.p, d, m, d, "diag_ln_stats_ln");
+            b.A = H.p;
+        } else {
+            a.stats_out = reinterpret_cast<float2*>(St.p);
+            launch_gemm(ctx, a, "diag_ln_stats_producer");
+            b.A = Y1.p; b.ln_gamma = G.p; b.ln_beta = Bt.p; b.ln_stats = reinterpret_cast<const float2*>(St.p);
+        }
+        launch_gemm(ctx, b, "diag_ln_stats_consumer");
+        WLK_HIP(hipDeviceSynchronize());
+        WLK_HIP(hipMemcpy(y1, Y1.p, (size_t)m * d * sizeof(float), hipMemcpyDeviceToHost));
+        WLK_HIP(hipMemcpy(y2, Y2.p, (size_t)m * n2 * sizeof(float), hipMemcpyDeviceToHost));
+        if (stats) WLK_HIP(hipMemcpy(stats, St.p, (size_t)stats_rows * np * 2 * sizeof(float), hipMemcpyDeviceToHost));
     });
 }
 
diff --git a/whisperlivekit_amd/csrc/gemm_f32.hip b/whisperlivekit_amd/csrc/gemm_f32.hip
--- a/whisperlivekit_amd/csrc/gemm_f32.hip
+++ b/whisperlivekit_amd/csrc/gemm_f32.hip
@@ -313,9 +313,11 @@
     }
 }
 
-template <bool KP = false>
+template <bool KP = false, bool LN = false>
 __global__ __launch_bounds__(256) void gemm_nt_f32_kwave16_kernel(GemmArgs g) {
     WLK_PIN_GEMM_ARGS(g);
+    WLK_PIN_S(g.stats_out);
+    if constexpr (LN) asm volatile("" ::"s"(g.ln_gamma), "s"(g.ln_beta), "s"(g.ln_stats));
     constexpr int KW = 4, SLAB = BK * KW, SUB = 16 * LDS_LD;
     __shared__ __attribute__((aligned(16))) float As[2][KW * SUB];
     __shared__ __attribute__((aligned(16))) float Ws[2][KW * SUB];
@@ -339,12 +341,22 @@
         w_byte[i] = (n0 + row) < g.N ? (unsigned)(((long)(n0 + row) * g.K + kcol) * 4) : kOob;
         lds_at[i] = (c4 >> 3) * SUB + row * LDS_LD + (c4 & 7) * 4;
     }
-    struct Slab {
+    struct SlabPlain {
         float4 a[2], w[2];
     };
+    struct SlabLn {
+        float4 a[2], w[2], gm, bt;
+    };
+    using Slab = std::conditional_t<LN, SlabLn, SlabPlain>;
+    float2 stat[2] = {};
     auto fetch = [&](Slab& st, int ks) {
         const int k0 = ks * SLAB;
         const bool in = (k0 + kcol) < g.K;
+        if constexpr (LN) {
+            const int kc = min(k0 + kcol, g.K - 4);
+            st.gm = ldg4(to_global(g.ln_gamma) + kc);
+            st.bt = ldg4(to_global(g.ln_beta) + kc);
+        }
 #pragma unroll
         for (int i = 0; i < 2; ++i) {
             const u32x4 v = __builtin_amdgcn_raw_buffer_load_b128(rsrc_a, (int)(in ? a_byte[i] + (unsigned)k0 * 4u : kOob), 0, 0);
@@ -358,7 +370,17 @@
     };
     auto stash = [&](const Slab& st, int buf) {
 #pragma unroll
-        for (int i = 0; i < 2; ++i) *reinterpret_cast<float4*>(&As[buf][lds_at[i]]) = st.a[i];
+        for (int i = 0; i < 2; ++i) {
+            float4 a = st.a[i];
+            if constexpr (LN) {
+                const float mean = stat[i].x, rstd = stat[i].y;
+                a.x = (a.x - mean) * rstd * st.gm.x + st.bt.x;
+                a.y = (a.y - mean) * rstd * st.gm.y + st.bt.y;
+                a.z = (a.z - mean) * rstd * st.gm.z + st.bt.z;
+                a.w = (a.w - mean) * rstd * st.gm.w + st.bt.w;
+            }
+            *reinterpret_cast<float4*>(&As[buf][lds_at[i]]) = a;
+        }
 #pragma unroll
         for (int i = 0; i < 2; ++i) *reinterpret_cast<float4*>(&Ws[buf][lds_at[i]]) = st.w[i];
     };
@@ -388,10 +410,30 @@
 #pragma unroll
     for (int r = 0; r < 4; ++r) res[r] = (has_res ? g.R + (long)min(row_base + r, g.M - 1) * g.ldr + colc : g.W)[0];
     int kv_off = (g.kcache ? g.kv_pos : reinterpret_cast<const int*>(g.W))[0];
+    float2 part[2][3];
+    const int n_part = g.K >> 4;
+    if constexpr (LN) {
+#pragma unroll
+        for (int i = 0; i < 2; ++i) {
+            const float2* pr = g.ln_stats + (long)min(m0 + (tid >> 5) + 8 * i, g.M - 1) * n_part;
+#pragma unroll
+            for (int j = 0; j < 3; ++j) part[i][j] = pr[min(c4 + 32 * j, n_part - 1)];
+        }
+    }
     pin_loaded(b);
 #pragma unroll
     for (int r = 0; r < 4; ++r) pin_loaded(res[r]);
     asm volatile("" : "+v"(kv_off));
+    if constexpr (LN) {
+#pragma unroll
+        for (int i = 0; i < 2; ++i)
+#pragma unroll
+            for (int j = 0; j < 3; ++j) { pin_loaded(part[i][j].x); pin_loaded(part[i][j].y); }
+        __builtin_amdgcn_sched_barrier(0);
+        const int n_mine = c4 >= n_part ? 0 : (n_part - c4 + 31) >> 5;
+#pragma unroll
+        for (int i = 0; i < 2; ++i) stat[i] = ln_stats_combine(part[i], n_mine, n_part);
+    }
     stash(s0, 0);
     __syncthreads();
     for (int ks = 0; ks < ns2; ks += 2) {
@@ -445,6 +487,10 @@
                 const int bm = row / g.kv_ntok, t = row - bm * g.kv_ntok;
                 kv_dst[((long)bm * g.kv_ctx + kv_off + t) * g.kv_d + kv_col] = v;
             }
+        }
+        if (g.stats_out) {
+            const float2 st = row16_stats(v);
+            if (row < g.M && (lane & 15) == 0) g.stats_out[(long)row * tiles_n + tile_n] = st;
         }
     }
 }
@@ -799,7 +845,27 @@
 bool gemm_takes_ksplit(int M, int N, int K) { return ksplit_tile(M, N, K).tm != 0; }
 
 void x3_refresh_env_switches();
-void refresh_env_switches() { x3_refresh_env_switches(); }
+static std::atomic<int> g_prefill_ln_stats{-1};
+void refresh_env_switches() {
+    x3_refresh_env_switches();
+    g_prefill_ln_stats.store(-1, std::memory_order_relaxed);
+}
+
+bool prefill_ln_stats_enabled() {
+    int v = g_prefill_ln_stats.load(std::memory_order_relaxed);
+    if (v < 0) {
+        const char* e = getenv("WLK_PREFILL_LN_STATS");
+        v = !(e && e[0] == '0');
+        g_prefill_ln_stats.store(v, std::memory_order_relaxed);
+    }
+    return v != 0;
+}
+
+bool prefill_ln_stats_applicable(int rows, int d) {
+    return prefill_ln_stats_enabled() && rows > 8 && d % 16 == 0 && d >= 256 && d <= kLnStatsMaxK &&
+           gemm_takes_kwave(rows, 3 * d, d) && gemm_takes_kwave(rows, d, d) && gemm_takes_kwave(rows, 4 * d, d) &&
+           gemm_takes_kwave(rows, d, 4 * d);
+}
 
 static GemmPlan gemm_plan_tiled(const GemmArgs& g) {
     GemmPlan p;
@@ -811,8 +877,18 @@
     if (g.K % 4 != 0 || g.lda % 4 != 0) return refuse("gemm: K and lda must be multiples of 4");
     if ((((long)g.M - 1) * g.lda + g.K) * 4 >= (1L << 31) || (long)g.N * g.K * 4 >= (1L << 31))
         return refuse("gemm: operand larger than 2 GiB");
-    if (g.ln_gamma) return refuse("gemm: only the GEMV kernels (rows <= 8) take the LayerNorm; launch it separately");
+    if (g.ln_gamma && !g.ln_stats)
+        return refuse("gemm: only the GEMV kernels (rows <= 8) take the LayerNorm; launch it separately");
     if (g.batch > kMaxBatch) return refuse("gemm: batch too large");
+    if (g.ln_stats || g.stats_out) {
+        if (g.batch > 0 || g.K < 256 || g.force_kernel != 0) return refuse("gemm: row statistics are only available on the 16 x 16 k-wave path");
+        if (g.stats_out && (!(g.flags & kGemmResidual) || g.N % 16 != 0))
+            return refuse("gemm: stats_out needs the residual epilogue and N % 16 == 0");
+        if (g.ln_stats && (!g.ln_gamma || !g.ln_beta || g.K % 16 != 0 || g.K > kLnStatsMaxK))
+            return refuse("gemm: LayerNorm on load needs gamma, beta and K % 16 == 0, K <= 1536");
+        p.kernel = GemmPlan::kKwave16;
+        return p;
+    }
     const bool want_kwave = g.force_kwave || g.force_kernel == 2;
     const KSplitTile kt = (want_kwave || g.kcache || g.force_kernel == 3) ? KSplitTile{0, 0} : ksplit_tile(g.M, g.N, g.K, g.force_kernel == 4);
     if (g.force_kernel == 4 && !kt.tm) return refuse("gemm: the k-pipe kernel does not take this shape");
@@ -847,7 +923,8 @@
         if (!dispatch_kpipe(ctx, g, p.tm, p.tn)) throw std::logic_error("gemm: k-pipe tile without an instantiation");
         break;
     case GemmPlan::kKwave16:
-        hipLaunchKernelGGL(gemm_nt_f32_kwave16_kernel<>, dim3((unsigned)tiles16), dim3(256), 0, ctx.stream, g);
+        if (g.ln_stats) hipLaunchKernelGGL((gemm_nt_f32_kwave16_kernel<false, true>), dim3((unsigned)tiles16), dim3(256), 0, ctx.stream, g);
+        else hipLaunchKernelGGL(gemm_nt_f32_kwave16_kernel<>, dim3((unsigned)tiles16), dim3(256), 0, ctx.stream, g);
         break;
     case GemmPlan::kKwave:
         hipLaunchKernelGGL(gemm_nt_f32_kwave_kernel<false>, dim3((unsigned)tiles32), dim3(256), 0, ctx.stream, g);
@@ -923,7 +1000,7 @@
     };
     if (g.K % 4 != 0 || g.lda % 4 != 0) return refuse("gemm: K and lda must be multiples of 4");
     if (g.batch > 0 || g.kcache) return refuse("gemm (kp family): plain projections only");
-    if (g.ln_gamma) return refuse("gemm (kp family): the LayerNorm is a launch of its own");
+    if (g.ln_gamma || g.ln_stats || g.stats_out) return refuse("gemm (kp family): the LayerNorm is a launch of its own");
     const bool short_k_kwave = g.K % 32 == 0 && g.K >= 128 && g.K < 256;
     if (!short_k_kwave && (g.K % 128 != 0 || g.K < 256)) {
         GemmArgs t = g;
@@ -1445,6 +1522,7 @@
     if (!gemv_applicable(g.M, g.K) || g.lda % 4 != 0) return refuse("gemv: unsupported shape");
     if (g.scale_period > 0) return refuse("gemv: scale_period is a GEMM operand (the GEMV kernels scale columns below scale_cols only)");
     if (g.batch > 0) return refuse("gemv: batched operand tables are a GEMM operand");
+    if (g.ln_stats || g.stats_out) return refuse("gemv: row statistics are a GEMM operand (every wave here holds the whole row)");
     p.rpw = g.N >= 16384 ? 4 : (g.N >= 2048 ? 2 : 1);
     p.ln = g.ln_gamma != nullptr;
     p.mg = g.mg_pm != nullptr;
diff --git a/whisperlivekit_amd/csrc/internal.h b/whisperlivekit_amd/csrc/internal.h
--- a/whisperlivekit_amd/csrc/internal.h
+++ b/whisperlivekit_amd/csrc/internal.h
@@ -127,6 +127,7 @@
     int cap_session_rows = 0;
     float *dx = nullptr, *dh = nullptr, *dqkv = nullptr, *datt = nullptr, *dq = nullptr, *dmlp = nullptr, *hsel = nullptr,
           *logits = nullptr, *part = nullptr;
+    float2* ln_part = nullptr;
     wlk::StepRow *rows_dev = nullptr, *tiles_dev = nullptr;
     int *ring_row_dev = nullptr, *zeros_dev = nullptr;
     char* pinned = nullptr;
@@ -211,6 +212,7 @@
     int max_rows = 0;
     int* tokens_dev = nullptr;
     float *dx = nullptr, *dh = nullptr, *dqkv = nullptr, *datt = nullptr, *dq = nullptr, *dmlp = nullptr;
+    float2* ln_part = nullptr;
     float* kcache[2] = {nullptr, nullptr};
     float* vcache[2] = {nullptr, nullptr};
     int kv_cur = 0;
diff --git a/whisperlivekit_amd/csrc/wave_ops.h b/whisperlivekit_amd/csrc/wave_ops.h
--- a/whisperlivekit_amd/csrc/wave_ops.h
+++ b/whisperlivekit_amd/csrc/wave_ops.h
@@ -95,6 +95,37 @@
     return v;
 }
 
+__device__ __forceinline__ float2 row16_stats(float v) {
+    const float mean = row16_sum_1248(v) * 0.0625f;
+    const float dev = v - mean;
+    return make_float2(mean, row16_sum_1248(__fmul_rn(dev, dev)));
+}
+
+__device__ __forceinline__ float half32_sum(float v) {
+    v += dpp_f32<0xB1>(v);
+    v += dpp_f32<0x4E>(v);
+    v += dpp_f32<0x1B>(dpp_f32<0x141>(v));
+    v += dpp_f32<0x128>(v);
+    float a, b;
+    swap16(v, a, b);
+    return a + b;
+}
+__device__ __forceinline__ float2 ln_stats_combine(const float2 (&p)[3], int n, int P) {
+    float s = 0.f;
+#pragma unroll
+    for (int j = 0; j < 3; ++j)
+        if (j < n) s += p[j].x;
+    const float mean = half32_sum(s) / (float)P;
+    float m2 = 0.f;
+#pragma unroll
+    for (int j = 0; j < 3; ++j) {
+        const float dm = p[j].x - mean;
+        if (j < n) m2 += p[j].y + 16.f * __fmul_rn(dm, dm);
+    }
+    m2 = half32_sum(m2);
+    return make_float2(mean, 1.0f / sqrtf(m2 / (float)(16 * P) + 1e-5f));
+}
+
 __device__ __forceinline__ void wave_argmax(float& bv, int& bi) {
 #define WLK_ARGMAX_LEVEL(OFF)                                              \
     {                                                                      \
```
